# Xiaohao-Liu/EliMRec

Measured on AMD Instinct MI355X. Metric: BPR triplets/sec (Tiktok-shape, d=128x3), higher is better.
Workload: dtype f32; 1 GPU; tiktok-shape-synthetic; num_items=76085, train_interactions=571503, recdim=64, layer_num=3, batch_per_gpu=2048, global_batch=2048, parallelism=colshard1, graph_table=column-sharded (64 of 64 columns per rank): hops need no communication, feature_tables=replicated S_m / c, feature_dtype=f32, columns_per_gpu=64, propagation=folded, head_rows=batch, step_issue=one host call per step (csrc/program.hip): 1243 of the 1243 timed steps

## Files before the change

### elimrec_amd/_lib.py

```python
import ctypes
import os

_HERE = os.path.dirname(os.path.abspath(__file__))
LIB_PATH = os.path.join(_HERE, "lib", "libelimrec_hip.so")

c_i32, c_i64, c_f32, c_u32, c_u64 = ctypes.c_int, ctypes.c_int64, ctypes.c_float, ctypes.c_uint32, ctypes.c_uint64
c_ptr, c_size = ctypes.c_void_p, ctypes.c_size_t

class CsrSplit(ctypes.Structure):
    _fields_ = [("long_threshold", ctypes.c_int32), ("n_long", ctypes.c_int32), ("n_seg", ctypes.c_int32),
                ("d_long_rows", ctypes.c_void_p), ("d_long_seg_ptr", ctypes.c_void_p),
                ("d_seg_bounds", ctypes.c_void_p), ("d_partials", ctypes.c_void_p), ("d_seg_row", ctypes.c_void_p),
                ("d_row_order", ctypes.c_void_p), ("d_tickets", ctypes.c_void_p), ("d_row_items", ctypes.c_void_p),
                ("n_row_items", ctypes.c_int32)]


class CsrDesc(ctypes.Structure):
    _fields_ = [("n_rows", ctypes.c_int64), ("d_rowptr", ctypes.c_void_p), ("d_col", ctypes.c_void_p),
                ("d_val", ctypes.c_void_p), ("split", CsrSplit)]


class LinearDesc(ctypes.Structure):
    _fields_ = [("d_A", ctypes.c_void_p), ("lda", ctypes.c_int64), ("d_W", ctypes.c_void_p), ("ldw", ctypes.c_int64),
                ("d_bias", ctypes.c_void_p), ("d_C", ctypes.c_void_p), ("ldc", ctypes.c_int64), ("M", ctypes.c_int64),
# ... 53 lines not shown
                ("d_Wf_user", ctypes.c_void_p), ("d_bf_user", ctypes.c_void_p), ("d_Wf_item", ctypes.c_void_p),
                ("d_bf_item", ctypes.c_void_p), ("d_pack", ctypes.c_void_p), ("pack_floats", ctypes.c_size_t)]


class HeadFwdIn(ctypes.Structure):
    _fields_ = [("d_out0", ctypes.c_void_p), ("ld_out0", ctypes.c_int64), ("d_narrow", ctypes.c_void_p), ("ld_nar", ctypes.c_int64),
                ("d_c", ctypes.c_void_p), ("d_S", ctypes.c_void_p * HEAD_MAX_TABLES), ("ldS", ctypes.c_int64 * HEAD_MAX_TABLES),
                ("d_recv", ctypes.c_void_p), ("world", ctypes.c_int32), ("dl", ctypes.c_int64), ("src16", HeadSrc16),
                ("rows", HeadRows)]


class HeadBwdSinks(ctypes.Structure):
    _fields_ = [("d_SrcA", ctypes.c_void_p), ("d_SrcB", ctypes.c_void_p), ("N", ctypes.c_int64), ("ns", ctypes.c_int32),
                ("w", ctypes.c_int32), ("d_split", ctypes.c_void_p), ("n_max", ctypes.c_int64), ("world", ctypes.c_int32)]


class ProgramOp(ctypes.Structure):
    _fields_ = [("kind", ctypes.c_int32), ("fn", ctypes.c_int32), ("args", ctypes.c_uint64 * PROGRAM_MAX_ARGS)]


class ProgramPatch(ctypes.Structure):
    _fields_ = [("op", ctypes.c_int32), ("arg", ctypes.c_int32), ("value", ctypes.c_uint64)]


c_sell = ctypes.POINTER(SellDesc)
c_split = ctypes.POINTER(CsrSplit)
c_csr = ctypes.POINTER(CsrDesc)

SIGNATURES = {
    "elimrec_abi_version": (c_i32, []),
    "elimrec_last_error": (ctypes.c_char_p, []),
    "elimrec_linear_fwd": (c_i32, [c_ptr, c_i64, c_ptr, c_i64, c_ptr, c_ptr, c_i64, c_i64, c_i32, c_i32, c_ptr]),
    "elimrec_linear_fwd_batched": (c_i32, [ctypes.POINTER(LinearDesc), c_i32, c_ptr]),
    "elimrec_linear_bwd_w_batched_workspace": (c_size, [ctypes.POINTER(LinearBwdDesc), c_i32]),
    "elimrec_linear_bwd_w_batched": (c_i32, [ctypes.POINTER(LinearBwdDesc), c_i32, c_ptr, c_size, c_ptr]),
    "elimrec_linear_bwd_w_batched_merge": (c_i32, [ctypes.POINTER(LinearBwdDesc), c_i32, c_ptr, c_size, c_ptr, c_ptr, c_i32, c_i64,
                                                   c_i64, c_i64, c_i32, c_i32, c_i32, c_ptr, c_ptr, c_ptr, c_i32, c_ptr]),
    "elimrec_linear_bwd_w_reduce": (c_i32, [ctypes.POINTER(LinearBwdDesc), c_i32, c_ptr, c_size, c_ptr]),
    "elimrec_linear_bwd_w_workspace": (c_size, [c_i64, c_i32, c_i32]),
    "elimrec_linear_bwd_w": (c_i32, [c_ptr, c_i64, c_ptr, c_i64, c_ptr, c_ptr, c_i64, c_i32, c_i32, c_ptr, c_i64,
                                     c_ptr, c_i32, c_ptr, c_size, c_ptr]),
    "elimrec_assemble_x0": (c_i32, [c_ptr, c_ptr, c_ptr, c_i64, c_i64, c_i32, c_i32, c_ptr]),
    "elimrec_spmm_hop": (c_i32, [c_ptr, c_ptr, c_ptr, c_i64, c_i32, c_split, c_ptr, c_ptr, c_ptr, c_ptr, c_f32, c_ptr]),
    "elimrec_propagate": (c_i32, [c_ptr, c_ptr, c_ptr, c_i64, c_i32, c_split, c_i32, c_ptr, c_ptr, c_ptr, c_ptr, c_ptr]),
    "elimrec_bipartite_workspace": (c_size, [c_i64, c_i64, c_i32, c_i32]),
    "elimrec_propagate_bipartite": (c_i32, [c_csr, c_csr, c_i64, c_i64, c_i32, c_i32, c_i32, c_ptr, c_ptr, c_ptr, c_ptr,
                                            c_ptr, c_size, c_ptr]),
    "elimrec_propagate_bipartite_bwd": (c_i32, [c_csr, c_csr, c_i64, c_i64, c_i32, c_i32, c_i32, c_ptr, c_ptr, c_ptr,
                                                c_ptr, c_i64, c_ptr, c_ptr, c_ptr, c_size, c_ptr]),
    "elimrec_ticket_fixup": (c_i32, []),
    "elimrec_set_ticket_fixup": (None, [c_i32]),
    "elimrec_concurrency": (c_i32, []),
    "elimrec_set_concurrency": (None, [c_i32]),
    "elimrec_folded_workspace": (c_size, [c_i64, c_i32]),
    "elimrec_propagate_folded": (c_i32, [c_csr, c_i64, c_i64, c_i32, c_i32, c_ptr, c_ptr, c_i64, c_ptr, c_ptr, c_size, c_ptr]),
    "elimrec_source_rows_split": (c_i32, [c_ptr, c_ptr, c_i64, c_i32, c_i32, c_i32, c_ptr, c_ptr]),
    "elimrec_propagate_folded_bwd": (c_i32, [c_csr, c_i64, c_i64, c_i32, c_i32, c_i32, c_ptr, c_ptr, c_ptr, c_i64, c_ptr,
                                             c_ptr, c_ptr, c_ptr, c_ptr, c_size, c_ptr]),
    "elimrec_block_spmm": (c_i32, [c_csr, c_i32, c_i64, c_ptr, c_ptr, c_ptr, c_ptr, c_f32, c_ptr]),
    "elimrec_blocksum_rows": (c_i32, [c_ptr, c_ptr, c_ptr, c_i64, c_i32, c_i32, c_i32, c_ptr, c_ptr]),
    "elimrec_triplet_rows": (c_i32, [c_ptr, c_ptr, c_ptr, c_i64, c_i64, c_ptr, c_ptr, c_i64, c_i32, c_ptr, c_i64, c_ptr]),
    "elimrec_triplet_rows_checked": (c_i32, [c_ptr, c_ptr, c_ptr, c_i64, c_i64, c_i64, c_ptr, c_ptr, c_ptr]),
    "elimrec_batch_plan": (c_i32, [c_ptr, c_ptr, c_ptr, c_i64, c_i64, c_i64, c_ptr, c_ptr, c_ptr, c_ptr, c_ptr, c_i32, c_ptr, c_ptr,
                                   c_size, c_ptr]),
    "elimrec_gather_rows": (c_i32, [c_ptr, c_i64, c_ptr, c_ptr, c_i64, c_i32, c_ptr, c_i64, c_ptr]),
    "elimrec_copy_cols": (c_i32, [c_ptr, c_i64, c_ptr, c_i64, c_i64, c_i32, c_ptr]),
    "elimrec_bpr_head": (c_i32, [c_ptr, c_i64, c_i64, c_i64, c_ptr, c_ptr, c_ptr, c_i32, c_i32, c_i32,
                                 ctypes.POINTER(c_f32), c_ptr, c_ptr, c_ptr, c_ptr]),
    "elimrec_bpr_head_rows": (c_i32, [c_ptr, c_i64, c_ptr, c_i32, c_i32, c_i32, ctypes.POINTER(c_f32), c_ptr, c_ptr, c_ptr, c_ptr,
                                      c_ptr, c_ptr]),
    "elimrec_loss_pub_create": (c_i32, [c_i32, ctypes.POINTER(c_ptr)]),
    "elimrec_loss_pub_destroy": (c_i32, [c_ptr]),
    "elimrec_loss_pub_issued": (c_u32, [c_ptr]),
    "elimrec_loss_pub_wait": (c_i32, [c_ptr, c_u32, ctypes.c_double, ctypes.POINTER(c_f32)]),
    "elimrec_sum": (c_i32, [c_ptr, c_i64, c_ptr, c_ptr]),
    "elimrec_segment_reduce_workspace": (c_size, [c_i64]),
    "elimrec_segment_plan_workspace": (c_size, [c_i64]),
    "elimrec_segment_plan": (c_i32, [c_ptr, c_i64, c_i32, c_i64, c_ptr, c_ptr, c_ptr, c_ptr, c_ptr, c_size, c_ptr]),
    "elimrec_segment_apply_head_bwd": (c_i32, [c_ptr, c_i64, c_i32, c_ptr, c_ptr, c_ptr, c_ptr, c_ptr, c_size, c_i64, c_i32,
                                               c_i32, c_i32, ctypes.POINTER(c_i32), c_ptr, c_ptr, ctypes.POINTER(c_ptr), c_ptr,
                                               c_ptr, ctypes.POINTER(HeadBwdSinks), c_ptr]),
    "elimrec_segment_apply": (c_i32, [c_ptr, c_i64, c_i32, c_ptr, c_ptr, c_ptr, c_ptr, c_size, c_ptr]),
    "elimrec_segment_reduce_rows": (c_i32, [c_ptr, c_ptr, c_i64, c_i32, c_i32, c_ptr, c_ptr, c_ptr, c_ptr, c_ptr, c_size, c_ptr]),
    "elimrec_head_bwd_input": (c_i32, [c_ptr, c_i64, c_ptr, c_ptr, c_i64, c_i64, c_i32, c_i32, c_i32,
                                       ctypes.POINTER(c_i32), c_ptr, c_ptr, ctypes.POINTER(c_ptr), c_f32, c_ptr, c_i64,
                                       c_i32, c_ptr, c_ptr]),
    "elimrec_embed_grad": (c_i32, [c_ptr, c_i64, c_i64, c_i32, c_i32, c_ptr, c_ptr, c_ptr]),
    "elimrec_adam_step": (c_i32, [c_ptr, c_ptr, c_ptr, c_ptr, c_i64, c_f32, c_f32, c_f32, c_f32, c_f32, c_i64, c_ptr]),
    "elimrec_score_workspace": (c_size, [c_i32, c_i64, c_i32]),
    "elimrec_score_workspace2": (c_size, [c_i32, c_i64, c_i64, c_i32, c_i32]),
    "elimrec_score_workspace_topk": (c_size, [c_i32, c_i64, c_i64, c_i32, c_i32]),
    "elimrec_score_workspace_for": (c_size, [c_i32, c_i64, c_i64, c_i32, c_i32, c_i32, c_i32]),
    "elimrec_row_sqnorms": (c_i32, [c_ptr, c_i64, c_i64, c_i32, c_i32, c_ptr, c_ptr]),
    "elimrec_score_topk": (c_i32, [c_ptr, c_i64, c_i64, c_i64, c_ptr, c_i32, c_i32, c_i32, c_u32, c_i32, c_i32,
                                   c_ptr, c_ptr, c_ptr, c_ptr, c_i64, c_i32, c_ptr, c_ptr, c_ptr, c_size, c_ptr]),
    "elimrec_score_topk_shard": (c_i32, [c_ptr, c_i64, c_i64, c_i64, c_ptr, c_i32, c_i32, c_i32, c_u32, c_i32, c_i32,
                                         c_ptr, c_ptr, c_ptr, c_ptr, c_i64, c_i32, c_ptr, c_ptr, c_ptr, c_size, c_i32, c_ptr, c_i64,
                                         c_i64, c_ptr]),
    "elimrec_topk_merge": (c_i32, [c_ptr, c_ptr, c_i32, c_i32, c_i32, c_ptr, c_ptr, c_ptr]),
    "elimrec_rank_metrics": (c_i32, [c_ptr, c_i32, c_i32, c_ptr, c_ptr, ctypes.POINTER(c_i32), c_i32, c_ptr, c_ptr]),
    "elimrec_group_metric_means": (c_i32, [c_ptr, c_i64, c_i32, c_i64, c_ptr, c_ptr, c_i64, c_i32, c_ptr, c_ptr, c_size, c_ptr]),
    "elimrec_group_metric_means_workspace": (c_size, [c_i64, c_i32, c_i32]),
    "elimrec_group_metric_means_chunk": (c_i32, []),
    "elimrec_rank_targets": (c_i32, [c_ptr, c_i64, c_i64, c_i64, c_ptr, c_ptr, c_i64, c_ptr, c_ptr]),
    "elimrec_rank_segment": (c_i32, []),
    "elimrec_rank_targets_per_pass": (c_i32, []),
    "elimrec_rank_pair_rows": (c_i32, [c_ptr, c_ptr, c_i64, ctypes.POINTER(ctypes.c_int), c_i32, c_ptr, c_ptr]),
    "elimrec_rank_user_rows": (c_i32, [c_ptr, c_ptr, c_i64, c_ptr, c_i64, c_ptr, c_ptr]),
    "elimrec_cosine_topk": (c_i32, [c_ptr, c_i64, c_i64, c_i32, c_ptr, c_i64, c_ptr, c_i64, c_i32, c_ptr, c_ptr, c_i32, c_ptr, c_ptr,
                                    c_ptr, c_size, c_ptr]),
    "elimrec_cosine_topk_workspace": (c_size, [c_i64, c_i64, c_i32]),
    "elimrec_cosine_topk_chunk": (c_i32, []),
    "elimrec_cosine_topk_tile": (c_i32, []),
    "elimrec_list_overlap": (c_i32, [c_ptr, c_ptr, c_i64, c_i32, c_ptr, c_ptr]),
    "elimrec_list_pair_cosine": (c_i32, [c_ptr, c_i64, c_i64, c_i32, c_i32, c_ptr, c_i64, c_ptr, c_i64, c_i32, c_ptr, c_ptr]),
    "elimrec_list_max_k": (c_i32, []),
    "elimrec_list_pair_cosine_small_k": (c_i32, []),
    "elimrec_list_pair_cosine_chunk_cols": (c_i32, [c_i32, c_i32]),
    "elimrec_list_exposure": (c_i32, [c_ptr, c_i64, c_i32, c_i64, c_ptr, c_ptr]),
    "elimrec_mmr_rerank": (c_i32, [c_ptr, c_i64, c_i64, c_i32, c_ptr, c_i64, c_ptr, c_ptr, c_i64, c_i32, c_i32, c_f32, c_ptr, c_ptr,
                                   c_ptr, c_ptr]),
    "elimrec_mmr_max_pool": (c_i32, []),
    "elimrec_mmr_rows_in_lds": (c_i32, [c_i32, c_i32]),
    "elimrec_pick_hard_negatives": (c_i32, [c_ptr, c_i64, c_i64, c_ptr, c_i64, c_ptr, c_i64, c_i64, c_ptr, c_i64, c_i32, c_i32,
                                            ctypes.POINTER(c_f32), c_ptr, c_ptr, c_i64, c_i32, c_ptr, c_ptr, c_ptr, c_ptr]),
    "elimrec_history_support": (c_i32, [c_ptr, c_i64, c_i64, c_i32, c_i32, c_ptr, c_i64, ctypes.POINTER(c_f32), c_ptr, c_ptr, c_i64,
                                        c_i32, c_ptr, c_ptr, c_i64, c_i32, c_i32, c_ptr, c_ptr, c_ptr, c_ptr, c_ptr]),
    "elimrec_history_max_top": (c_i32, []),
    "elimrec_slab_partials_bytes": (c_size, [c_sell, c_i32, c_i32]),
    "elimrec_slab_hop": (c_i32, [c_sell, c_i32, c_i32, c_i32, c_ptr, c_ptr, c_ptr, c_ptr, c_ptr, c_f32, c_ptr, c_size, c_i32,
                                 c_ptr]),
    "elimrec_topk_reference_order": (c_i32, [c_ptr, c_i64, c_i64, c_i64, c_i32, c_ptr]),
    "elimrec_topk_reference_order_device": (c_i32, [c_ptr, c_i64, c_i64, c_i64, c_i32, c_ptr, c_ptr, c_ptr]),
    "elimrec_score_topk_ordered": (c_i32, [c_ptr, c_i64, c_i64, c_i64, c_ptr, c_i32, c_i32, c_i32, c_u32, c_i32, c_i32,
                                           c_ptr, c_ptr, c_ptr, c_ptr, c_i64, c_i32, c_ptr, c_ptr, c_ptr, c_size, c_i32, c_ptr]),
    "elimrec_plan_workspace": (c_size, [c_i64, c_i64, c_i64]),
    "elimrec_plan_tile_count": (c_i64, [c_i64, c_i64, c_i64, c_i64, c_i32]),
    "elimrec_plan_rows": (c_i32, [c_ptr, c_i64, c_i32, c_i32, c_i32, c_i32, c_i32, c_i64, c_i64, c_ptr, c_ptr, c_ptr, c_ptr, c_ptr, c_ptr, c_size, c_ptr]),
    "elimrec_plan_tiles": (c_i32, [c_ptr, c_i64, c_i32, c_i32, c_i32, c_i32, c_i32, c_i64, c_i64, c_ptr, c_ptr, c_ptr, c_i64, c_i64, c_i64, c_i64, c_i64,
                                   c_i64, c_ptr, c_ptr, c_ptr, c_ptr, c_ptr, c_ptr, c_ptr, c_ptr, c_size, c_ptr]),
    "elimrec_plan_scatter": (c_i32, [c_i64, c_i32, c_ptr, c_ptr, c_ptr, c_ptr, c_ptr, c_ptr, c_ptr, c_ptr, c_ptr]),
    "elimrec_slab_sweep_lds_rows": (c_size, [c_i32]),
    "elimrec_slab_sweep_hop": (c_i32, [c_ptr, c_ptr, c_i64, c_i64, c_ptr, c_i32, c_i32, c_i32, c_i32, c_i32, c_i32,
                                       c_ptr, c_ptr, c_ptr, c_ptr, c_f32, c_ptr]),
    "elimrec_slab_sweep_hop_adam": (c_i32, [c_ptr, c_ptr, c_i64, c_i64, c_ptr, c_i32, c_i32, c_i32, c_i32, c_i32, c_i32,
                                            c_ptr, c_ptr, c_ptr, c_ptr, c_f32, c_ptr, c_ptr, c_ptr, c_ptr, c_f32, c_f32, c_f32, c_f32, c_f32,
                                            c_i64, c_ptr]),
    "elimrec_slab_hop_bwd_w": (c_i32, [c_sell, c_i32, c_i32, c_i32, c_ptr, c_ptr, c_ptr, c_ptr, c_ptr, c_f32, c_ptr, c_size, c_i32,
                                       ctypes.POINTER(LinearBwdDesc), c_i32, c_ptr, c_size, c_i32, c_ptr]),
    "elimrec_slab_source_bits": (c_i32, [c_sell, c_i32, c_i32, c_i32, c_ptr, c_ptr, c_size, c_ptr]),
    "elimrec_slab_hop_adam": (c_i32, [c_sell, c_i32, c_i32, c_i32, c_ptr, c_ptr, c_ptr, c_ptr, c_f32, c_ptr, c_size, c_ptr, c_ptr,
                                      c_ptr, c_ptr, c_f32, c_f32, c_f32, c_f32, c_f32, c_i64, ctypes.POINTER(AdamJob), c_i32, c_ptr, c_i64,
                                      c_ptr, c_ptr]),
    "elimrec_slab_rows": (c_i32, [c_sell, c_i32, c_i32, c_i32, c_i64, ctypes.POINTER(c_ptr), c_ptr, c_ptr, c_ptr, c_i64, c_i32,
                                  c_ptr, c_i64, c_ptr, c_i64, c_i32, c_ptr]),
    "elimrec_slab_from_rows": (c_i32, [c_ptr, c_i64, c_i64, c_i64, c_i32, c_i32, c_ptr, c_ptr]),
    "elimrec_slab_to_rows": (c_i32, [c_ptr, c_i64, c_i32, c_i32, c_ptr, c_i64, c_i64, c_ptr]),
    "elimrec_slab_merge_rows": (c_i32, [c_ptr, c_ptr, c_i32, c_i64, c_i64, c_i64, c_i32, c_i32, c_i32, c_ptr, c_ptr, c_ptr, c_ptr]),
    "elimrec_adam_step_out": (c_i32, [c_ptr, c_ptr, c_ptr, c_ptr, c_ptr, c_i64, c_f32, c_f32, c_f32, c_f32, c_f32, c_i64,
                                      c_ptr]),
    "elimrec_head_pack_floats": (c_size, [c_i32, ctypes.POINTER(c_i32)]),
    "elimrec_head_pack_bwd_offset": (c_size, [c_i32, ctypes.POINTER(c_i32)]),
    "elimrec_head_fwd_fused": (c_i32, [ctypes.POINTER(HeadFwdIn), ctypes.POINTER(HeadWeights), c_ptr, c_ptr, c_i64, c_ptr, c_i64,
                                       c_ptr, c_i64, c_i32, c_ptr]),
    "elimrec_score_range_violations": (c_i32, [ctypes.POINTER(c_i64), c_i32, c_ptr]),
    "elimrec_score_range_check": (c_i32, [c_ptr, c_ptr, c_i32, c_i32, c_i32, c_i32, c_ptr, c_ptr]),
    "elimrec_score_set_math": (None, [c_i32]),
    "elimrec_score_get_math": (c_i32, []),
    "elimrec_score_set_bf16x3": (None, [c_i32]),
    "elimrec_score_get_bf16x3": (c_i32, []),
    "elimrec_build_adj_workspace": (c_size, [c_i64, c_i64, c_i32]),
    "elimrec_build_adj": (c_i32, [c_ptr, c_ptr, c_i64, c_i64, c_i64, c_i32, c_ptr, c_i32, c_ptr, c_ptr, c_ptr, c_ptr, c_ptr, c_size,
                                  c_ptr]),
    "elimrec_adam_multi": (c_i32, [ctypes.POINTER(AdamJob), c_i32, c_f32, c_f32, c_f32, c_f32, c_f32, c_ptr]),
    "elimrec_lookup_counts": (c_i32, [c_ptr, c_i32, c_i64, c_i64, c_i64, ctypes.POINTER(c_i64), ctypes.POINTER(c_i64), c_ptr, c_ptr]),
    "elimrec_lookup_pack": (c_i32, [c_ptr, c_i32, c_i64, c_i64, c_i64, ctypes.POINTER(c_i64), ctypes.POINTER(c_i64), c_i32, c_ptr, c_i64,
                                    c_ptr, c_ptr, c_ptr]),
    "elimrec_lookup_unpack": (c_i32, [c_ptr, c_i32, c_i64, c_i64, c_i64, ctypes.POINTER(c_i64), ctypes.POINTER(c_i64), c_i32, c_ptr, c_i64,
                                      c_i32, c_i32, c_i32, c_ptr, c_i64, c_ptr, c_ptr]),
    "elimrec_wide_from_master": (c_i32, [c_ptr, c_i64, c_i64, c_i32, c_i32, c_ptr, c_ptr]),
    "elimrec_wide_rows": (c_i32, [ctypes.POINTER(c_ptr), c_i32, c_i64, c_i32, c_i32, c_ptr, c_i64, c_ptr, c_i64, c_ptr, c_i64, c_ptr]),
    "elimrec_wide_grad": (c_i32, [c_ptr, c_i64, c_i64, c_i32, c_i32, c_f32, c_ptr, c_ptr]),
    "elimrec_rows_bitmap": (c_i32, [c_ptr, c_i32, c_i64, c_i64, c_ptr, c_ptr]),
    "elimrec_peer_cols_to_rows": (c_i32, [c_ptr, c_i32, c_i64, c_i32, c_ptr, c_i64, c_ptr, c_i64, c_ptr]),
    "elimrec_program_fn_count": (c_i32, []),
    "elimrec_program_fn_name": (ctypes.c_char_p, [c_i32]),
    "elimrec_program_fn_args": (c_i32, [c_i32]),
    "elimrec_program_create": (c_i32, [ctypes.POINTER(ProgramOp), c_i32, ctypes.POINTER(c_ptr)]),
    "elimrec_program_create_scoped": (c_i32, [ctypes.POINTER(ProgramOp), c_i32, c_i32, ctypes.POINTER(c_ptr)]),
    "elimrec_program_run": (c_i32, [c_ptr, ctypes.POINTER(ProgramPatch), c_i32]),
    "elimrec_program_destroy": (c_i32, [c_ptr]),
    "elimrec_comm_unique_id": (c_i32, [c_ptr]),
    "elimrec_comm_create": (c_i32, [c_ptr, c_i32, c_i32, ctypes.POINTER(c_ptr)]),
    "elimrec_comm_nranks": (c_i32, [c_ptr, ctypes.POINTER(c_i32)]),
    "elimrec_comm_destroy": (c_i32, [c_ptr]),
    "elimrec_comm_all_gather": (c_i32, [c_ptr, c_ptr, c_ptr, c_i64, c_ptr]),
    "elimrec_comm_all_reduce_f32": (c_i32, [c_ptr, c_ptr, c_i64, c_ptr]),
    "elimrec_comm_all_to_all": (c_i32, [c_ptr, c_ptr, c_ptr, c_i64, c_ptr]),
    "elimrec_comm_all_to_all_v": (c_i32, [c_ptr, c_ptr, c_ptr, ctypes.POINTER(c_i64), c_ptr]),
    "elimrec_sample_triplets": (c_i32, [c_ptr, c_ptr, c_ptr, c_i64, c_i64, c_i64, c_u64, c_u64, c_ptr, c_ptr, c_ptr, c_ptr]),
    "elimrec_sample_triplet_candidates": (c_i32, [c_ptr, c_ptr, c_ptr, c_i64, c_i64, c_i64, c_u64, c_u64, c_i32, c_ptr, c_ptr, c_ptr,
                                                  c_ptr]),
    "elimrec_sample_negatives": (c_i32, [c_ptr, c_ptr, c_i64, c_i64, c_i32, c_u64, c_ptr, c_ptr]),
    "elimrec_score_candidates": (c_i32, [c_ptr, c_i64, c_i64, c_i64, c_ptr, c_i32, c_i32, c_i32, c_u32, c_i32, c_i32,
                                         c_ptr, c_ptr, c_ptr, c_ptr, c_i64, c_ptr, c_i64, c_i64, c_ptr]),
    "elimrec_score_effects": (c_i32, [c_ptr, c_i64, c_i64, c_i64, c_ptr, c_i32, c_i32, c_i32, c_u32, c_i32,
                                      c_ptr, c_ptr, c_ptr, c_ptr, c_i64, c_ptr, c_i64, c_ptr]),
}

_lib = None


class HipLibraryError(RuntimeError):
    pass


def load():
    global _lib
    if _lib is not None:
        return _lib
    if not os.path.exists(LIB_PATH):
        raise HipLibraryError(
            "elimrec_amd: %s is missing. Build it with `python -c 'import __graft_entry__ as g; g.build()'` "
            "(or `make -C elimrec_amd/csrc`). There is no CPU fallback for the hot path." % LIB_PATH)
    try:
        lib = ctypes.CDLL(LIB_PATH)
    except OSError as e:
        raise HipLibraryError("elimrec_amd: cannot load %s: %s" % (LIB_PATH, e))
    for name, (res, args) in SIGNATURES.items():
        try:
            fn = getattr(lib, name)
        except AttributeError:
            raise HipLibraryError("elimrec_amd: %s does not export %s (stale build?)" % (LIB_PATH, name))
        fn.restype = res
        fn.argtypes = args
    if lib.elimrec_abi_version() != 2:
        raise HipLibraryError("elimrec_amd: ABI version mismatch")
    _lib = _Recording(lib)
    return _lib


class _Recording(object):

    def __init__(self, lib):
        self._cdll = lib
        self._rec = None
        self._trace = None
        for name, (res, _) in SIGNATURES.items():
            fn = getattr(lib, name)
            plain = name in ("elimrec_abi_version", "elimrec_program_fn_count", "elimrec_program_fn_args", "elimrec_comm_unique_id",
                             "elimrec_score_get_math", "elimrec_score_get_bf16x3", "elimrec_group_metric_means_chunk",
                             "elimrec_rank_segment", "elimrec_rank_targets_per_pass",
                             "elimrec_cosine_topk_chunk", "elimrec_cosine_topk_tile",
                             "elimrec_list_max_k", "elimrec_list_pair_cosine_small_k", "elimrec_list_pair_cosine_chunk_cols",
                             "elimrec_mmr_max_pool", "elimrec_mmr_rows_in_lds",
                             "elimrec_comm_create", "elimrec_comm_destroy", "elimrec_comm_nranks") or name.startswith("elimrec_program_")
            setattr(self, name, self._wrap(fn, name) if res is c_i32 and not plain else fn)

    def _wrap(self, fn, name):
        def call(*args):
            if self._rec is not None:
                self._rec.append((fn, args))
            if self._trace is not None:
                self._trace.append(("call", name, fn, args))
            return fn(*args)
        return call


def record(calls):
    load()._rec = calls


def replay(calls, what):
    for fn, args in calls:
        rc = fn(*args)
        if rc:
            check(rc, what)


def check(rc, what):
    if rc != 0:
        msg = load().elimrec_last_error()
        raise RuntimeError("%s failed (rc=%d): %s" % (what, rc, msg.decode() if msg else "?"))
```

### elimrec_amd/csrc/bwd_w.h

```cpp
#pragma once
#include "common.h"
#include <cstdlib>

namespace elimrec {

constexpr int kMaxBatch = 8;
typedef float v16f __attribute__((ext_vector_type(16)));
#ifndef ELIMREC_BWDW_TN2
#define ELIMREC_BWDW_TN2 64
#endif
constexpr int TN1 = 64, TN2 = ELIMREC_BWDW_TN2, TRB = 32;
constexpr int BNJ = TN2 / 64, BC4 = TN2 / 4, BRP = 256 / BC4, BPS = TRB / BRP;

struct BwdProblem {
    elimrec_linear_bwd_desc d;
    int chunk_rows, chunks, t1, t2;
    int first_block;
    float *slabs, *cslabs;
};
struct BwdBatch { BwdProblem p[kMaxBatch]; int n; };

__device__ __forceinline__ void bwd_w_partial_body(const BwdBatch &batch, int block, float (*As)[TRB * TN1], float (*Bs)[TRB * TN2]) {
    const int tid = threadIdx.x, lane = tid & 63, wave = tid >> 6;
    int pi = 0;
    while (pi + 1 < batch.n && block >= batch.p[pi + 1].first_block) ++pi;
    const BwdProblem &pb = batch.p[pi];
    const int local = block - pb.first_block;
    const int n1_tiles = pb.t1, n2_tiles = pb.t2;
    const int chunk = local / (n1_tiles * n2_tiles);
    const int tile = local - chunk * (n1_tiles * n2_tiles);
    const int tile_y = tile / n2_tiles, tile_z = tile - tile_y * n2_tiles;
    const float *__restrict__ A = pb.d.d_A;
    const float *__restrict__ B = pb.d.d_B;
    const int32_t *__restrict__ row_index = pb.d.d_row_index;
    const int32_t *__restrict__ range = pb.d.d_range;
    const int64_t lda = pb.d.lda, ldb = pb.d.ldb, R = pb.d.R;
    const int n1 = pb.d.n1, n2 = pb.d.n2, chunk_rows = pb.chunk_rows;
    float *__restrict__ slabs = pb.slabs;
    float *__restrict__ colsum_slabs = pb.d.d_colsum ? pb.cslabs : nullptr;
    const float *__restrict__ cw = pb.d.d_colsum ? pb.d.d_colsum_weight : nullptr;
    int64_t rb = 0, re = R;
    if (range) { rb = range[0]; re = range[1]; }
    const int64_t r0 = rb + (int64_t)chunk * chunk_rows;
    const int64_t r1 = (r0 + chunk_rows < re) ? r0 + chunk_rows : re;
    const int i_base = tile_y * TN1, j_base = tile_z * TN2;

    const int a_row = tid >> 4, a_c4 = tid & 15;
    const int b_row = tid / BC4, b_c4 = tid % BC4;
    const bool a_col_ok = (i_base + a_c4 * 4) < n1;
    const bool b_col_ok = (j_base + b_c4 * 4) < n2;
    float4 ra[2], rbv[BPS];
    float rw = 1.f, rw_cur = 1.f;
    auto load_block = [&](int64_t row0) {
        if (cw && tid < TRB) {
            const int64_t r = row0 + tid;
            rw = r < r1 ? cw[row_index ? (int64_t)row_index[r] : r] : 0.f;
        }
#pragma unroll
        for (int p = 0; p < 2; ++p) {
            const int64_t r = row0 + a_row + 16 * p;
            ra[p] = (a_col_ok && r < r1) ? *reinterpret_cast<const float4 *>(A + r * lda + i_base + a_c4 * 4)
                                         : make_float4(0.f, 0.f, 0.f, 0.f);
        }
#pragma unroll
        for (int p = 0; p < BPS; ++p) {
            const int64_t r = row0 + b_row + BRP * p;
            float4 v = make_float4(0.f, 0.f, 0.f, 0.f);
            if (b_col_ok && r < r1) {
                const int64_t br = row_index ? (int64_t)row_index[r] : r;
                v = *reinterpret_cast<const float4 *>(B + br * ldb + j_base + b_c4 * 4);
            }
            rbv[p] = v;
        }
    };
    auto store_block = [&](int buf) {
        rw_cur = rw;
#pragma unroll
        for (int p = 0; p < 2; ++p)
            *reinterpret_cast<float4 *>(&As[buf][(a_row + 16 * p) * TN1 + a_c4 * 4]) = ra[p];
#pragma unroll
        for (int p = 0; p < BPS; ++p)
            *reinterpret_cast<float4 *>(&Bs[buf][(b_row + BRP * p) * TN2 + b_c4 * 4]) = rbv[p];
    };

    const int wi = (wave & 1) * 32, wj = (wave >> 1) * (TN2 / 2);
    const int li = lane & 31, lk = lane >> 5;
    const bool wave_on = (j_base + wj) < n2;
    const bool half1_on = BNJ > 1 && (j_base + wj + 32) < n2;
    v16f acc0 = {0}, acc1 = {0};
    float csum = 0.f;
    int buf = 0;
    if (r0 < r1) {
        load_block(r0);
        store_block(0);
    }
    __syncthreads();
    for (int64_t row0 = r0; row0 < r1; row0 += TRB) {
        const bool more = (row0 + TRB) < r1;
        if (more) load_block(row0 + TRB);
        const float *as = As[buf], *bs = Bs[buf];
        if (wave_on) {
#pragma unroll
            for (int kk = 0; kk < TRB; kk += 2) {
                const float a = as[(kk + lk) * TN1 + wi + li];
                const float b0 = bs[(kk + lk) * TN2 + wj + li];
                acc0 = __builtin_amdgcn_mfma_f32_32x32x2f32(a, b0, acc0, 0, 0, 0);
                if (BNJ > 1) {
                    const float b1 = bs[(kk + lk) * TN2 + wj + (BNJ > 1 ? 32 : 0) + li];
                    acc1 = __builtin_amdgcn_mfma_f32_32x32x2f32(a, b1, acc1, 0, 0, 0);
                }
            }
        }
        if (colsum_slabs && tid < TN1) {
            if (cw) {
#pragma unroll
                for (int k = 0; k < TRB; ++k)
                    csum += as[k * TN1 + tid] * __builtin_bit_cast(float, __builtin_amdgcn_readlane(__builtin_bit_cast(int, rw_cur), k));
            } else {
#pragma unroll 8
                for (int k = 0; k < TRB; ++k) csum += as[k * TN1 + tid];
            }
        }
        if (more) store_block(buf ^ 1);
        __syncthreads();
        buf ^= 1;
    }
    const int n1_pad = n1_tiles * TN1, n2_pad = n2_tiles * TN2;
    float *slab = slabs + (size_t)chunk * n1_pad * n2_pad;
    if (wave_on) {
#pragma unroll
        for (int r = 0; r < 16; ++r) {
            const int row = i_base + wi + (r & 3) + 8 * (r >> 2) + 4 * (lane >> 5);
            slab[(size_t)row * n2_pad + j_base + wj + li] = acc0[r];
            if (half1_on) slab[(size_t)row * n2_pad + j_base + wj + 32 + li] = acc1[r];
        }
    }
    if (colsum_slabs && tile_z == 0 && tid < TN1) colsum_slabs[(size_t)chunk * n1_pad + i_base + tid] = csum;
}

__device__ __forceinline__ void reduce_slabs_body(const BwdBatch &batch, int bx, int by) {
    const BwdProblem &pb = batch.p[by];
    const int n1 = pb.d.n1, n2 = pb.d.n2;
    const int n1_pad = pb.t1 * TN1, n2_pad = pb.t2 * TN2;
    const int gid = bx * 256 + (int)threadIdx.x;
    const int idx = gid >> 2, q = gid & 3;
    const int total = n1 * n2;
    int64_t rows = pb.d.d_range ? (int64_t)pb.d.d_range[1] - pb.d.d_range[0] : pb.d.R;
    if (rows < 0) rows = 0;
    const int chunks = (int)((rows + pb.chunk_rows - 1) / pb.chunk_rows);
    const float *src = nullptr;
    size_t stride = 0;
    float *dst = nullptr;
    if (idx < total) {
        const int i = idx / n2, j = idx - i * n2;
        src = pb.slabs + (size_t)i * n2_pad + j;
        stride = (size_t)n1_pad * n2_pad;
        dst = pb.d.d_out + (int64_t)i * pb.d.ldo + j;
    } else if (pb.d.d_colsum && idx < total + n1) {
        src = pb.cslabs + (idx - total);
        stride = (size_t)n1_pad;
        dst = pb.d.d_colsum + (idx - total);
    }
    float s = 0.f;
    if (src) {
        int c = q;
        for (; c + 12 < chunks; c += 16) {
            const float v0 = src[(size_t)c * stride], v1 = src[(size_t)(c + 4) * stride];
            const float v2 = src[(size_t)(c + 8) * stride], v3 = src[(size_t)(c + 12) * stride];
            s += v0; s += v1; s += v2; s += v3;
        }
        for (; c < chunks; c += 4) s += src[(size_t)c * stride];
    }
    s += __shfl_xor(s, 1, 64);
    s += __shfl_xor(s, 2, 64);
    if (src && q == 0) *dst = pb.d.accumulate ? (*dst + s) : s;
}


static inline void bwd_w_dims(int64_t R, int n1, int n2, int &chunk_rows, int &chunks, int &t1, int &t2) {
    const int tiles = ((n1 + TN1 - 1) / TN1) * ((n2 + TN2 - 1) / TN2);
    static int target = 0;
    if (!target) target = 480;
    int64_t want = (R * tiles + target - 1) / target;
    want = (want + TRB - 1) / TRB * TRB;
    chunk_rows = (int)(want < 64 ? 64 : (want > 512 ? 512 : want));
    chunks = (int)((R + chunk_rows - 1) / chunk_rows);
    if (chunks < 1) chunks = 1;
    t1 = (n1 + TN1 - 1) / TN1;
    t2 = (n2 + TN2 - 1) / TN2;
}

static inline size_t bwd_w_bytes(int64_t R, int n1, int n2) {
    int cr, chunks, t1, t2;
    bwd_w_dims(R, n1, n2, cr, chunks, t1, t2);
    return align_up(((size_t)chunks * t1 * TN1 * t2 * TN2 + (size_t)chunks * t1 * TN1) * sizeof(float), 256);
}


static inline int bwd_w_build_batch(const elimrec_linear_bwd_desc *descs, int n, void *d_workspace, BwdBatch &batch, int &blocks,
                                    int &max_out) {
    batch.n = n;
    char *ws = (char *)d_workspace;
    blocks = 0; max_out = 0;
    for (int i = 0; i < n; ++i) {
        const elimrec_linear_bwd_desc &d = descs[i];
        ELIMREC_REQUIRE(d.d_A && d.d_B && d.d_out, "linear_bwd_w: null pointer");
        ELIMREC_REQUIRE(d.R >= 0 && d.n1 > 0 && d.n2 > 0, "linear_bwd_w: bad shape");
        ELIMREC_REQUIRE(d.n1 % 4 == 0 && d.n2 % 4 == 0 && d.lda % 4 == 0 && d.ldb % 4 == 0,
                        "linear_bwd_w: n1, n2, lda, ldb must be multiples of 4");
        ELIMREC_REQUIRE(((uintptr_t)d.d_A % 16) == 0 && ((uintptr_t)d.d_B % 16) == 0,
                        "linear_bwd_w: A and B must be 16-byte aligned");
        BwdProblem &pb = batch.p[i];
        pb.d = d;
        bwd_w_dims(d.R, d.n1, d.n2, pb.chunk_rows, pb.chunks, pb.t1, pb.t2);
        pb.first_block = blocks;
        blocks += pb.chunks * pb.t1 * pb.t2;
        pb.slabs = (float *)ws;
        pb.cslabs = pb.slabs + (size_t)pb.chunks * pb.t1 * TN1 * pb.t2 * TN2;
        ws += bwd_w_bytes(d.R, d.n1, d.n2);
        const int out_elems = d.n1 * d.n2 + (d.d_colsum ? d.n1 : 0);
        if (out_elems > max_out) max_out = out_elems;
    }
    return 0;
}

static inline size_t bwd_w_batched_bytes(const elimrec_linear_bwd_desc *descs, int n) {
    size_t total = 0;
    for (int i = 0; i < n; ++i) total += bwd_w_bytes(descs[i].R, descs[i].n1, descs[i].n2);
    return total;
}

}
```

### elimrec_amd/csrc/program.hip

```cpp
#include "common.h"
#include <dlfcn.h>
#include <cstring>
#include <string>
#include <utility>
#include <vector>

namespace elimrec {

template <typename T> struct Unpack {
    static T get(uint64_t v) {
        if constexpr (std::is_pointer<T>::value) return reinterpret_cast<T>(static_cast<uintptr_t>(v));
        else if constexpr (std::is_same<T, float>::value) { uint32_t b = (uint32_t)v; float f; memcpy(&f, &b, 4); return f; }
        else return static_cast<T>(v);
    }
};
template <typename R, typename... A, size_t... I>
static R call_packed_impl(R (*f)(A...), const uint64_t *a, std::index_sequence<I...>) { return f(Unpack<A>::get(a[I])...); }
template <typename R, typename... A> static R call_packed(R (*f)(A...), const uint64_t *a) {
    static_assert(sizeof...(A) <= ELIMREC_PROGRAM_MAX_ARGS, "too many arguments for a program op");
    return call_packed_impl(f, a, std::index_sequence_for<A...>{});
}
template <typename R, typename... A> constexpr int arg_count(R (*)(A...)) { return (int)sizeof...(A); }

static unsigned event_flags(bool has_collectives) {
    return has_collectives ? hipEventDisableTiming : (hipEventDisableTiming | hipEventDisableSystemFence);
}

struct FnEntry { const char *name; int (*thunk)(const uint64_t *); int n_args; };
#define ELIMREC_FN(fn) {#fn, [](const uint64_t *a) -> int { return call_packed(fn, a); }, arg_count(fn)}
static const FnEntry kFns[] = {
    ELIMREC_FN(elimrec_batch_plan), ELIMREC_FN(elimrec_slab_hop), ELIMREC_FN(elimrec_slab_sweep_hop), ELIMREC_FN(elimrec_slab_sweep_hop_adam), ELIMREC_FN(elimrec_slab_source_bits), ELIMREC_FN(elimrec_slab_hop_bwd_w),
    ELIMREC_FN(elimrec_slab_hop_adam), ELIMREC_FN(elimrec_slab_rows), ELIMREC_FN(elimrec_slab_merge_rows),
    ELIMREC_FN(elimrec_head_fwd_fused), ELIMREC_FN(elimrec_bpr_head_rows), ELIMREC_FN(elimrec_sum), ELIMREC_FN(elimrec_segment_apply_head_bwd),
    ELIMREC_FN(elimrec_linear_fwd_batched), ELIMREC_FN(elimrec_linear_bwd_w_batched),
    ELIMREC_FN(elimrec_linear_bwd_w_batched_merge), ELIMREC_FN(elimrec_linear_bwd_w_reduce), ELIMREC_FN(elimrec_adam_multi),
    ELIMREC_FN(elimrec_source_rows_split), ELIMREC_FN(elimrec_copy_cols), ELIMREC_FN(elimrec_lookup_pack), ELIMREC_FN(elimrec_lookup_unpack),
    ELIMREC_FN(elimrec_lookup_counts), ELIMREC_FN(elimrec_adam_step_out),
    ELIMREC_FN(elimrec_peer_cols_to_rows), ELIMREC_FN(elimrec_rows_bitmap), ELIMREC_FN(elimrec_comm_all_gather), ELIMREC_FN(elimrec_comm_all_reduce_f32),
    ELIMREC_FN(elimrec_comm_all_to_all), ELIMREC_FN(elimrec_comm_all_to_all_v), ELIMREC_FN(elimrec_wide_from_master),
    ELIMREC_FN(elimrec_wide_rows), ELIMREC_FN(elimrec_wide_grad),
};
constexpr int kNumFns = (int)(sizeof(kFns) / sizeof(kFns[0]));

typedef struct ncclComm *ncclComm_t;
struct NcclId { char internal[128]; };
struct Rccl {
    void *h = nullptr;
    int (*GetUniqueId)(NcclId *) = nullptr;
    int (*CommInitRank)(ncclComm_t *, int, NcclId, int) = nullptr;
    int (*CommDestroy)(ncclComm_t) = nullptr;
    int (*CommCount)(ncclComm_t, int *) = nullptr;
    int (*AllGather)(const void *, void *, size_t, int, ncclComm_t, hipStream_t) = nullptr;
    int (*AllReduce)(const void *, void *, size_t, int, int, ncclComm_t, hipStream_t) = nullptr;
    int (*Send)(const void *, size_t, int, int, ncclComm_t, hipStream_t) = nullptr;
    int (*Recv)(void *, size_t, int, int, ncclComm_t, hipStream_t) = nullptr;
    int (*GroupStart)() = nullptr;
    int (*GroupEnd)() = nullptr;
    const char *(*GetErrorString)(int) = nullptr;
};
static Rccl g_rccl;
static int rccl_load() {
    if (g_rccl.h) return 0;
    void *h = dlopen("librccl.so", RTLD_NOW | RTLD_NOLOAD);
    if (!h) h = dlopen("librccl.so.1", RTLD_NOW | RTLD_NOLOAD);
    if (!h) h = dlopen("librccl.so", RTLD_NOW | RTLD_GLOBAL);
    if (!h) h = dlopen("/opt/rocm/lib/librccl.so", RTLD_NOW | RTLD_GLOBAL);
    if (!h) { set_error("program: librccl.so not found (%s)", dlerror()); return ELIMREC_E_UNSUPPORTED; }
#define ELIMREC_SYM(field, name)                                                         \
    *(void **)(&g_rccl.field) = dlsym(h, name);                                          \
    if (!g_rccl.field) { set_error("program: %s missing in librccl", name); return ELIMREC_E_UNSUPPORTED; }
    ELIMREC_SYM(GetUniqueId, "ncclGetUniqueId") ELIMREC_SYM(CommInitRank, "ncclCommInitRank") ELIMREC_SYM(CommDestroy, "ncclCommDestroy")
    ELIMREC_SYM(CommCount, "ncclCommCount")
    ELIMREC_SYM(AllGather, "ncclAllGather") ELIMREC_SYM(AllReduce, "ncclAllReduce") ELIMREC_SYM(Send, "ncclSend") ELIMREC_SYM(Recv, "ncclRecv")
    ELIMREC_SYM(GroupStart, "ncclGroupStart") ELIMREC_SYM(GroupEnd, "ncclGroupEnd") ELIMREC_SYM(GetErrorString, "ncclGetErrorString")
#undef ELIMREC_SYM
    g_rccl.h = h;
    return 0;
}
static int rccl_check(int rc, const char *what) {
    if (rc == 0) return 0;
    set_error("%s: %s", what, g_rccl.GetErrorString ? g_rccl.GetErrorString(rc) : "RCCL error");
    return 20000 + rc;
}
constexpr int kNcclFloat32 = 7, kNcclUint8 = 1, kNcclSum = 0;

struct Comm { ncclComm_t comm; int world, rank; };

struct Program {
    std::vector<elimrec_op> ops;
    std::vector<hipEvent_t> events;
};

}

using namespace elimrec;

extern "C" int elimrec_program_fn_count(void) { return kNumFns; }
extern "C" const char *elimrec_program_fn_name(int i) { return (i >= 0 && i < kNumFns) ? kFns[i].name : nullptr; }
extern "C" int elimrec_program_fn_args(int i) { return (i >= 0 && i < kNumFns) ? kFns[i].n_args : -1; }

extern "C" int elimrec_comm_unique_id(void *id128) {
    int rc = rccl_load();
    if (rc) return rc;
    return rccl_check(g_rccl.GetUniqueId((NcclId *)id128), "ncclGetUniqueId");
}

extern "C" int elimrec_comm_create(const void *id128, int world, int rank, void **comm_out) {
    ELIMREC_REQUIRE(id128 && comm_out && world >= 1 && rank >= 0 && rank < world, "comm_create: bad arguments");
    int rc = rccl_load();
    if (rc) return rc;
    NcclId id;
    memcpy(&id, id128, sizeof(id));
    Comm *c = new Comm{nullptr, world, rank};
    rc = rccl_check(g_rccl.CommInitRank(&c->comm, world, id, rank), "ncclCommInitRank");
    if (rc) { delete c; return rc; }
    *comm_out = c;
    return 0;
}

extern "C" int elimrec_comm_nranks(void *comm, int *n_out) {
    ELIMREC_REQUIRE(comm && n_out, "comm_nranks: bad arguments");
    return rccl_check(g_rccl.CommCount(((Comm *)comm)->comm, n_out), "ncclCommCount");
}

extern "C" int elimrec_comm_destroy(void *comm) {
    if (!comm) return 0;
    Comm *c = (Comm *)comm;
    int rc = g_rccl.CommDestroy ? rccl_check(g_rccl.CommDestroy(c->comm), "ncclCommDestroy") : 0;
    delete c;
    return rc;
}

extern "C" int elimrec_comm_all_gather(void *comm, const void *d_send, void *d_recv, int64_t bytes_per_rank, void *stream) {
    ELIMREC_REQUIRE(comm && d_send && d_recv && bytes_per_rank >= 0, "comm_all_gather: bad arguments");
    Comm *c = (Comm *)comm;
    return rccl_check(g_rccl.AllGather(d_send, d_recv, (size_t)bytes_per_rank, kNcclUint8, c->comm, (hipStream_t)stream), "ncclAllGather");
}

extern "C" int elimrec_comm_all_reduce_f32(void *comm, float *d_buf, int64_t n, void *stream) {
    ELIMREC_REQUIRE(comm && d_buf && n >= 0, "comm_all_reduce: bad arguments");
    Comm *c = (Comm *)comm;
    return rccl_check(g_rccl.AllReduce(d_buf, d_buf, (size_t)n, kNcclFloat32, kNcclSum, c->comm, (hipStream_t)stream), "ncclAllReduce");
}

extern "C" int elimrec_comm_all_to_all(void *comm, const void *d_send, void *d_recv, int64_t bytes_per_peer, void *stream) {
    ELIMREC_REQUIRE(comm && d_send && d_recv && bytes_per_peer >= 0, "comm_all_to_all: bad arguments");
    Comm *c = (Comm *)comm;
    const char *s = (const char *)d_send;
    char *r = (char *)d_recv;
    const size_t nb = (size_t)bytes_per_peer;
    int rc = rccl_check(g_rccl.GroupStart(), "ncclGroupStart");
    for (int q = 0; q < c->world && !rc; ++q) {
        rc = rccl_check(g_rccl.Send(s + (size_t)q * nb, nb, kNcclUint8, q, c->comm, (hipStream_t)stream), "ncclSend");
        if (!rc) rc = rccl_check(g_rccl.Recv(r + (size_t)q * nb, nb, kNcclUint8, q, c->comm, (hipStream_t)stream), "ncclRecv");
    }
    const int rc2 = rccl_check(g_rccl.GroupEnd(), "ncclGroupEnd");
    return rc ? rc : rc2;
}

extern "C" int elimrec_comm_all_to_all_v(void *comm, const void *d_send, void *d_recv, const int64_t *sizes, void *stream) {
    ELIMREC_REQUIRE(comm && d_send && d_recv && sizes, "comm_all_to_all_v: bad arguments");
    Comm *c = (Comm *)comm;
    const char *s = (const char *)d_send;
    char *r = (char *)d_recv;
    int rc = rccl_check(g_rccl.GroupStart(), "ncclGroupStart");
    size_t so = 0, ro = 0;
    for (int q = 0; q < c->world && !rc; ++q) {
        const size_t sb = (size_t)sizes[q], rb = (size_t)sizes[c->world + q];
        if (sb) rc = rccl_check(g_rccl.Send(s + so, sb, kNcclUint8, q, c->comm, (hipStream_t)stream), "ncclSend");
        if (!rc && rb) rc = rccl_check(g_rccl.Recv(r + ro, rb, kNcclUint8, q, c->comm, (hipStream_t)stream), "ncclRecv");
        so += sb; ro += rb;
    }
    const int rc2 = rccl_check(g_rccl.GroupEnd(), "ncclGroupEnd");
    return rc ? rc : rc2;
}

extern "C" int elimrec_program_create_scoped(const elimrec_op *ops, int n_ops, int system_scope_events, void **prog_out) {
    ELIMREC_REQUIRE(ops && n_ops > 0 && prog_out, "program_create: bad arguments");
    Program *p = new Program();
    p->ops.assign(ops, ops + n_ops);
    int n_events = 0;
    bool has_collectives = system_scope_events != 0;
    for (const elimrec_op &o : p->ops) {
        if (o.kind == ELIMREC_OP_CALL) {
            if (o.fn < 0 || o.fn >= kNumFns) { delete p; set_error("program_create: unknown function index %d", o.fn); return ELIMREC_E_BADARG; }
// ... 52 lines not shown
```

### elimrec_amd/csrc/slab.hip

```cpp
#include "common.h"
#include "merge_rows.h"
#include "rows_args.h"
#include "bwd_w.h"
#include <cstdlib>

namespace elimrec {


struct SellArgs {
    const int32_t *item_dst, *item_len, *blk_off, *col;
    const float *val;
    int64_t n_rows, n_src;
    int n_seg, n_long;
    int item_begin, item_end;
    int seg_limit;
    int w4, w4_shift, gs, spg;
    const float4 *Xin;
    const uint32_t *src_mask;
    float4 *Xout;
    const float4 *Add;
    const uint32_t *add_mask;
    float scale;
    float4 *partials;
    const int32_t *long_rows, *long_seg_ptr;
// ... 498 lines not shown
#pragma unroll
            for (int q = 0; q < KL; ++q) bal[q] = (MASKED && k + q < nk) ? t.ballots[(int64_t)ti * t.kmax + k + q] : 0ull;
            int cj[UB];
            float vj[UB];
            bool in[UB];
#pragma unroll
            for (int u = 0; u < UB; ++u) {
                const int q = u / LPR, srcl = (u % LPR) * G + sub;
                cj[u] = G == 64 ? cc[q] : __shfl(cc[q], srcl, 64);
                vj[u] = G == 64 ? vc[q] : __shfl(vc[q], srcl, 64);
                in[u] = (jbase + u) < glen;
                if (MASKED) in[u] = in[u] && ((bal[q] >> srcl) & 1ull);
            }
            tile_batch<VPL, IN_BF16, UB>(a, in_base, cj, vj, in, acc);
#pragma unroll
            for (int q = 0; q < KL; ++q) { cc[q] = cn[q]; vc[q] = vn[q]; }
        }
    }
}

template <int LPR, int VPL>
__device__ __forceinline__ void tier_wave_sum(const float (&acc)[VPL], int cl, int n_long_guard, float (&tot)[VPL]) {
    constexpr int NQ = 64 / LPR;
#pragma unroll
    for (int i = 0; i < VPL; ++i) tot[i] = NQ > 1 ? __shfl(acc[i], cl, 64) : acc[i];
    const int nq = NQ + (n_long_guard < 0 ? 1 : 0);
#pragma unroll 2
    for (int g = 1; g < nq; ++g) {
#pragma unroll
        for (int i = 0; i < VPL; ++i) tot[i] += __shfl(acc[i], g * LPR + cl, 64);
    }
}

template <int LPR, int VPL, bool IN_BF16, bool OUT_BF16, bool MASKED, bool ADAM, bool EXT_LDS = false>
__device__ __forceinline__ void tier_body(const TierArgs &t, float *lds = nullptr, unsigned front = 0) {
    constexpr int G = 64 / LPR;
    const StreamArgs &a = t.s;
    const int lane = threadIdx.x & 63, wave = threadIdx.x >> 6;
    const unsigned bx = blockIdx.x - front;
    const int grp = (int)(bx % (unsigned)a.gs);
    const int bidx = (int)(bx / (unsigned)a.gs);
    const int sub = lane / LPR, cl = lane % LPR;
    const int slab = grp * a.spg + (cl >> a.wl_shift);
    const int c = cl & (a.wl - 1);
    const int64_t in_base = (int64_t)slab * a.n_src * a.wl + c;
    __shared__ float s_own[EXT_LDS ? 1 : 4 * 64 * 8];
    float *s_part = EXT_LDS ? lds : s_own;
    const int ti = __builtin_amdgcn_readfirstlane(bidx * 4 + wave);
    const bool wg_row = bidx < t.n_w4;
    int64_t off = 0;
    int steps = 0, glen = 0, dst = -1;
    if (ti < t.n_tiles_run) {
        off = t.tile_off[ti];
        steps = (int)((t.tile_off[ti + 1] - off) / G);
        glen = t.tile_len[(int64_t)ti * G + sub];
        dst = t.tile_dst[(int64_t)ti * G + sub];
    }
    if (a.compact_long && a.add_mask && ti < t.n_tiles_run) {
        if (wg_row || ti < t.tseg_base) {
            const int row = __shfl(dst, 0, 64);
            if (row >= 0 && !bit_of(a.add_mask, row)) return;
        } else if (dst >= 0) {
            const int li0 = t.tile_long[(int64_t)(ti - t.tseg_base) * G + sub];
            if (!bit_of(a.add_mask, a.long_rows[li0])) { dst = -1; glen = 0; }
        }
    }
    float acc[VPL];
    tile_gather<LPR, VPL, IN_BF16, MASKED>(t, ti, in_base, off, steps, glen, lane, sub, acc);
    if (wg_row) {
        float tot[VPL];
        tier_wave_sum<LPR, VPL>(acc, cl, a.n_long, tot);
        if (sub == 0) {
#pragma unroll
            for (int i = 0; i < VPL; ++i) s_part[(wave * LPR + cl) * VPL + i] = tot[i];
        }
        __syncthreads();
        if (wave == 0 && sub == 0) {
#pragma unroll
            for (int i = 0; i < VPL; ++i) tot[i] = ((s_part[cl * VPL + i] + s_part[(LPR + cl) * VPL + i]) + s_part[(2 * LPR + cl) * VPL + i]) +
                                                   s_part[(3 * LPR + cl) * VPL + i];
            if (a.compact_long) lane_store<VPL, false>(a.Xout, ((int64_t)slab * a.n_long + t.long_index[dst]) * a.wl + c, tot);
            else stream_epilogue<VPL, OUT_BF16, ADAM>(a, slab, dst, c, tot);
        }
        return;
    }
    if (ti >= t.n_tiles_run) return;
    if (ti < t.tseg_base) {
        const int row = __shfl(dst, 0, 64);
        if (row < 0) return;
        float tot[VPL];
        tier_wave_sum<LPR, VPL>(acc, cl, a.n_long, tot);
        if (sub == 0) {
            if (a.compact_long) lane_store<VPL, false>(a.Xout, ((int64_t)slab * a.n_long + t.long_index[row]) * a.wl + c, tot);
            else stream_epilogue<VPL, OUT_BF16, ADAM>(a, slab, row, c, tot);
        }
        return;
    }
    if (ti >= t.tfin_base) {
        if (dst >= 0) stream_epilogue<VPL, OUT_BF16, ADAM>(a, slab, dst, c, acc);
        return;
    }
    __amdgpu_buffer_rsrc_t prsrc = __builtin_amdgcn_make_buffer_rsrc(
        (void *)a.partials, 0, (int)min((size_t)0x7FFFFFF0, (size_t)a.n_seg * a.gs * a.spg * a.wl * VPL * 4), 0x00020000);
    if (dst >= 0) {
        const int64_t pidx = ((int64_t)slab * a.n_seg + dst) * a.wl + c;
#pragma unroll
        for (int h = 0; h < VPL / 4; ++h) {
            u32x4s bits = {__float_as_uint(acc[4 * h]), __float_as_uint(acc[4 * h + 1]), __float_as_uint(acc[4 * h + 2]),
                           __float_as_uint(acc[4 * h + 3])};
            __builtin_amdgcn_raw_buffer_store_b128(bits, prsrc, (unsigned)((pidx * (VPL / 4) + h) * 16), 0, 16 );
        }
    }
    asm volatile("s_waitcnt vmcnt(0)" ::: "memory");
    int li = -1, ticket = -1, nseg = 0;
    if (dst >= 0) {
        li = t.tile_long[(int64_t)(ti - t.tseg_base) * G + sub];
        nseg = a.long_seg_ptr[li + 1] - a.long_seg_ptr[li];
        if (cl == 0) ticket = __hip_atomic_fetch_add(&a.tickets[(int64_t)grp * a.n_long + li], 1, __ATOMIC_RELAXED, __HIP_MEMORY_SCOPE_AGENT);
    }
    ticket = __shfl(ticket, sub * LPR, 64);
    const bool last = dst >= 0 && ticket == nseg - 1;
    if (__ballot(last) == 0ull) return;
    __builtin_amdgcn_fence(__ATOMIC_ACQUIRE, "agent");
    asm volatile("s_waitcnt vmcnt(0)" ::: "memory");
#pragma unroll 1
    for (int g = 0; g < G; ++g) {
        if (!__shfl(last ? 1 : 0, g * LPR, 64)) continue;
        const int g_li = __shfl(li, g * LPR, 64);
        stream_combine<LPR, VPL, OUT_BF16, ADAM>(a, grp, g_li);
        if (lane == 0) __hip_atomic_store(&a.tickets[(int64_t)grp * a.n_long + g_li], 0, __ATOMIC_RELAXED, __HIP_MEMORY_SCOPE_AGENT);
    }
}

#ifndef ELIMREC_TILE_WAVES
#define ELIMREC_TILE_WAVES 5
#endif
template <int LPR, int VPL, bool IN_BF16, bool OUT_BF16, bool MASKED>
__global__ __launch_bounds__(256, ELIMREC_TILE_WAVES) void sell_tier_kernel(TierArgs t) {
    tier_body<LPR, VPL, IN_BF16, OUT_BF16, MASKED, false>(t);
}

template <int LPR>
__global__ __launch_bounds__(256) void sell_tier_adam_kernel(TierArgs t, AdamJobs tail, int tail_block0) {
    __shared__ float scratch[4 * 64 * 8];
    if ((int)blockIdx.x >= tail_block0) {
        const int b = (int)blockIdx.x - tail_block0;
        if (b < tail.blocks) adam_jobs_body(tail, b, t.s.ad_beta1, t.s.ad_beta2, t.s.ad_eps, t.s.ad_wd);
        else fixed_order_sum_body(tail.sum_src, tail.sum_n, tail.sum_dst, scratch);
        return;
    }
    tier_body<LPR, 4, false, false, false, true, true>(t, scratch);
}

template <int LPR, bool MASKED>
__global__ __launch_bounds__(256, (LPR <= 8 ? 5 : 1)) void sell_tier_bwdw_kernel(TierArgs t, BwdBatch batch, int tail_block0, int tail_mode, int gx) {
    __shared__ float As[2][TRB * TN1];
    __shared__ float Bs[2][TRB * TN2];
    static_assert(2 * TRB * TN1 >= 4 * 64 * 8, "the hop's LDS scratch must fit the A stages");
    const int front = tail_block0 < 0 ? (-tail_block0 + 7) & ~7 : 0;
    if (tail_block0 < 0 ? (int)blockIdx.x < front : (int)blockIdx.x >= tail_block0) {
        const int b = tail_block0 < 0 ? (int)blockIdx.x : (int)blockIdx.x - tail_block0;
        if (tail_block0 < 0 && b >= -tail_block0) return;
        if (tail_mode == 1) { reduce_slabs_body(batch, b % gx, b / gx); return; }
        bwd_w_partial_body(batch, b, As, Bs);
        return;
    }
    tier_body<LPR, 4, false, false, MASKED, false, true>(t, &As[0][0], (unsigned)front);
}

static int log2_pow2(int x) {
    int s = 0;
    while ((1 << s) < x) ++s;
    return (1 << s) == x ? s : -1;
}

}

using namespace elimrec;

static size_t slab_partial_floats_bytes(const elimrec_sell *A, int ns, int w) {
    return align_up((size_t)(A->n_seg > 0 ? A->n_seg : 1) * ns * w * sizeof(float), 256);
}
static size_t slab_ticket_bytes(const elimrec_sell *A) { return align_up((size_t)8 * (A->n_long > 0 ? A->n_long : 1) * sizeof(int32_t), 256); }
static size_t slab_ballot_bytes(const elimrec_sell *A) {
    if (!A->tiered) return 0;
    const size_t tiles = (size_t)A->n_t4 + A->n_t1 + A->n_tseg + A->n_tfin;
    return align_up(tiles * (size_t)(A->tile_kmax > 0 ? A->tile_kmax : 1) * sizeof(uint64_t), 256);
}

extern "C" size_t elimrec_slab_partials_bytes(const elimrec_sell *A, int ns, int w) {
    if (!A || ns <= 0 || w <= 0) return 0;
    return slab_partial_floats_bytes(A, ns, w) + slab_ticket_bytes(A) + slab_ballot_bytes(A);
}

struct AdamEpilogue {
    const float *p_in; float *p_out, *m, *v;
    float step_size, inv_sqrt_bc2, beta1, beta2, eps, wd;
    int keep_grad;
    const AdamJobs *tail;
};

static int launch_tier(const elimrec_sell *A, int ns, int wl, int wl_shift, int gs, int spg, int lpr, const void *Xin,
                       const uint32_t *src_mask, void *Xout, const float *add,
                       const uint32_t *add_mask, float scale, float *partials, int flags, hipStream_t s,
                       const AdamEpilogue *adam = nullptr, const BwdBatch *bwdw = nullptr, int tail_mode = 0, int tail_blocks = 0,
                       int reduce_gx = 1) {
    const int seg_only = flags & 1;
    const bool bits_ready = (flags & 2) != 0;
    if (A->tile_groups != 64 / lpr) {
        set_error("slab_hop: the plan's wave tiles were laid out for %d lane groups per wave, this table geometry has %d",
                  A->tile_groups, 64 / lpr);
        return ELIMREC_E_BADARG;
    }
    ELIMREC_REQUIRE(A->d_tile_off && A->d_tile_len && A->d_tile_dst && A->d_tile_col && A->d_tile_val && A->n_t4 == 4 * A->n_w4 &&
                        A->n_t1 % 4 == 0 && A->n_tseg % 4 == 0 && A->n_tfin % 4 == 0 && (A->n_tseg == 0 || A->d_tile_long),
                    "slab_hop: bad tile plan");
    TierArgs t = {};
    StreamArgs &a = t.s;
    a.n_rows = A->n_rows; a.n_src = A->n_src; a.n_seg = A->n_seg; a.n_long = A->n_long;
    a.wl = wl; a.wl_shift = wl_shift; a.gs = gs; a.spg = spg;
    a.Xin = Xin; a.src_mask = src_mask; a.Xout = Xout;
    a.Add = seg_only ? nullptr : (const float4 *)add; a.add_mask = add_mask; a.scale = seg_only ? 1.0f : scale;
    a.partials = partials; a.long_rows = A->d_long_rows; a.long_seg_ptr = A->d_long_seg_ptr;
    a.tickets = (int32_t *)((char *)partials + slab_partial_floats_bytes(A, ns, wl * 4));
    a.compact_long = seg_only ? 1 : 0;
    if (adam) {
        a.ad_p_in = adam->p_in; a.ad_p_out = adam->p_out; a.ad_m = adam->m; a.ad_v = adam->v;
        a.ad_step_size = adam->step_size; a.ad_inv_sqrt_bc2 = adam->inv_sqrt_bc2; a.ad_beta1 = adam->beta1; a.ad_beta2 = adam->beta2;
        a.ad_eps = adam->eps; a.ad_wd = adam->wd; a.ad_keep_grad = adam->keep_grad;
    }
    t.tile_off = A->d_tile_off; t.tile_len = A->d_tile_len; t.tile_dst = A->d_tile_dst; t.tile_long = A->d_tile_long;
    t.tcol = A->d_tile_col; t.tval = A->d_tile_val; t.long_index = A->d_long_index;
    t.n_w4 = A->n_w4;
    t.t1_base = A->n_t4; t.tseg_base = t.t1_base + A->n_t1; t.tfin_base = t.tseg_base + A->n_tseg;
    t.n_tiles = t.tfin_base + A->n_tfin;
    t.n_tiles_run = seg_only ? t.tfin_base : t.n_tiles;
    const int64_t per_group = t.n_tiles_run / 4;
    if (per_group <= 0) return 0;
    int tail_block0 = (int)(per_group * gs);
    {
        if (bwdw && tail_blocks > 0 && !adam && tail_mode == 2) {
            tail_block0 = -tail_blocks;
            tail_blocks = (tail_blocks + 7) & ~7;
        }
    }
    AdamJobs tail = {};
    if (adam && adam->tail && (adam->tail->n > 0 || adam->tail->sum_src)) tail = *adam->tail;
    if (tail.n <= 0) tail.blocks = 0;
    const dim3 grid((unsigned)(per_group * gs)), grid_adam((unsigned)(per_group * gs) + (unsigned)tail.blocks + (tail.sum_src ? 1u : 0u));
    const bool masked = src_mask != nullptr;
    if (masked) {
        ELIMREC_REQUIRE(A->tile_kmax > 0, "slab_hop: bad tile plan (tile_kmax)");
        t.kmax = A->tile_kmax;
        uint64_t *ballots = (uint64_t *)((char *)a.tickets + slab_ticket_bytes(A));
        t.ballots = ballots;
        if (!bits_ready)
        hipLaunchKernelGGL(tile_ballot_kernel, dim3((unsigned)per_group, (unsigned)t.kmax), dim3(256), 0, s, t.tile_off, t.tcol, src_mask, 64 / lpr,
                           t.n_tiles_run, t.kmax, ballots);
    }
#define ELIMREC_TIER(LPR)                                                                                                     \
    do {                                                                                                                      \
        if (adam) hipLaunchKernelGGL((sell_tier_adam_kernel<LPR>), grid_adam, dim3(256), 0, s, t, tail, tail_block0);         \
        else if (bwdw && masked)                                                                                              \
            hipLaunchKernelGGL((sell_tier_bwdw_kernel<LPR, true>), dim3(grid.x + (unsigned)tail_blocks), dim3(256), 0, s, t,  \
                               *bwdw, tail_block0, tail_mode, reduce_gx);                                                     \
        else if (bwdw)                                                                                                        \
            hipLaunchKernelGGL((sell_tier_bwdw_kernel<LPR, false>), dim3(grid.x + (unsigned)tail_blocks), dim3(256), 0, s, t, \
                               *bwdw, tail_block0, tail_mode, reduce_gx);                                                     \
        else if (masked) hipLaunchKernelGGL((sell_tier_kernel<LPR, 4, false, false, true>), grid, dim3(256), 0, s, t);        \
        else hipLaunchKernelGGL((sell_tier_kernel<LPR, 4, false, false, false>), grid, dim3(256), 0, s, t);                   \
    } while (0)
    switch (lpr) {
        case 1: ELIMREC_TIER(1); break;
        case 2: ELIMREC_TIER(2); break;
        case 4: ELIMREC_TIER(4); break;
        case 8: ELIMREC_TIER(8); break;
        case 16: ELIMREC_TIER(16); break;
        case 32: ELIMREC_TIER(32); break;
        default: ELIMREC_TIER(64); break;
    }
#undef ELIMREC_TIER
    return check_hip(hipGetLastError(), "slab_hop(tiered)");
}

static int slab_geometry(const char *who, int ns, int w, int gs, int &w4_shift, int &spg, int &lpr) {
    const int w4 = w / 4;
    w4_shift = (w > 0 && w % 4 == 0) ? log2_pow2(w4) : -1;
    if (ns < 1 || w4_shift < 0) { set_error("%s: slab width must be 4 * 2^k (got w=%d, ns=%d)", who, w, ns); return ELIMREC_E_BADARG; }
    if (gs < 1 || ns % gs != 0) { set_error("%s: %d slab groups do not divide %d slabs", who, gs, ns); return ELIMREC_E_BADARG; }
    spg = ns / gs;
    if (log2_pow2(spg) < 0 || spg * w4 > 64) {
        set_error("%s: slabs per group (%d) must be a power of two with spg*w/4 <= 64", who, spg);
        return ELIMREC_E_BADARG;
    }
    lpr = spg * w4;
    return 0;
}

static int slab_simple_geometry(const char *who, int64_t n, int ns, int w, int &w4_shift) {
    w4_shift = (w > 0 && w % 4 == 0) ? log2_pow2(w / 4) : -1;
    if (n < 0 || ns < 1 || w4_shift < 0) { set_error("%s: bad slab geometry (n=%lld, ns=%d, w=%d)", who, (long long)n, ns, w); return ELIMREC_E_BADARG; }
    return 0;
}

extern "C" int elimrec_slab_hop(const elimrec_sell *A, int ns, int w, int gs, const float *d_Xin,
                                const uint32_t *d_src_mask, float *d_Xout, const float *d_add,
                                const uint32_t *d_add_mask, float scale, float *d_partials, size_t partials_bytes,
                                int flags, void *stream) {
    const int seg_only = flags & 1;
    ELIMREC_REQUIRE(A && d_Xin && d_Xout, "slab_hop: null pointer");
    ELIMREC_REQUIRE(d_Xin != d_Xout, "slab_hop: Xout must not alias Xin");
    ELIMREC_REQUIRE(A->n_items % 64 == 0 && A->n_seg_items % 64 == 0 && A->n_seg_items <= A->n_items, "slab_hop: bad plan");
    int w4_shift, spg, lpr, rc;
    if ((rc = slab_geometry("slab_hop", ns, w, gs, w4_shift, spg, lpr))) return rc;
    if ((A->n_long > 0 || A->tiered) && (!d_partials || partials_bytes < elimrec_slab_partials_bytes(A, ns, w))) {
        set_error("slab_hop: partial-row scratch too small");
        return ELIMREC_E_WORKSPACE;
    }
    SellArgs a = {};
    a.item_dst = A->d_item_dst; a.item_len = A->d_item_len; a.blk_off = A->d_blk_off; a.col = A->d_col; a.val = A->d_val;
    a.n_rows = A->n_rows; a.n_src = A->n_src; a.n_seg = A->n_seg; a.n_long = A->n_long;
    a.item_begin = 0; a.item_end = seg_only ? A->n_seg_items : A->n_items; a.seg_limit = A->n_seg_items;
    a.w4 = w / 4; a.w4_shift = w4_shift; a.gs = gs; a.spg = spg;
    a.Xin = (const float4 *)d_Xin; a.src_mask = d_src_mask; a.Xout = (float4 *)d_Xout;
    a.Add = seg_only ? nullptr : (const float4 *)d_add; a.add_mask = d_add_mask; a.scale = seg_only ? 1.0f : scale;
    a.partials = (float4 *)d_partials; a.long_rows = A->d_long_rows; a.long_seg_ptr = A->d_long_seg_ptr;
    a.compact_long = seg_only ? 1 : 0;
    hipStream_t s = (hipStream_t)stream;
    if (A->tiered)
        return launch_tier(A, ns, w / 4, w4_shift, gs, spg, lpr, d_Xin, d_src_mask, d_Xout, d_add, d_add_mask, scale,
                           d_partials, flags, s);
    const int n_it = a.item_end - a.item_begin;
    if (n_it > 0) {
        const int ipw = 64 / lpr;
        const unsigned blocks = (unsigned)(((int64_t)n_it / ipw + 3) / 4) * (unsigned)gs;
#define ELIMREC_SELL_LAUNCH(LPR)                                                                          \
    do {                                                                                                  \
        if (d_src_mask) hipLaunchKernelGGL((sell_hop_kernel<LPR, true, 8, false>), dim3(blocks), dim3(256), 0, s, a); \
        else hipLaunchKernelGGL((sell_hop_kernel<LPR, false, 4, true>), dim3(blocks), dim3(256), 0, s, a);            \
    } while (0)
        switch (lpr) {
            case 1: ELIMREC_SELL_LAUNCH(1); break;
            case 2: ELIMREC_SELL_LAUNCH(2); break;
            case 4: ELIMREC_SELL_LAUNCH(4); break;
            case 8: ELIMREC_SELL_LAUNCH(8); break;
            case 16: ELIMREC_SELL_LAUNCH(16); break;
            case 32: ELIMREC_SELL_LAUNCH(32); break;
            default: ELIMREC_SELL_LAUNCH(64); break;
        }
#undef ELIMREC_SELL_LAUNCH
        ELIMREC_LAUNCH_CHECK("slab_hop");
    }
    if (A->n_long > 0) {
        const unsigned blocks = (unsigned)((A->n_long + 3) / 4) * (unsigned)gs;
        switch (lpr) {
            case 1: hipLaunchKernelGGL((sell_fixup_kernel<1>), dim3(blocks), dim3(256), 0, s, a); break;
            case 2: hipLaunchKernelGGL((sell_fixup_kernel<2>), dim3(blocks), dim3(256), 0, s, a); break;
            case 4: hipLaunchKernelGGL((sell_fixup_kernel<4>), dim3(blocks), dim3(256), 0, s, a); break;
            case 8: hipLaunchKernelGGL((sell_fixup_kernel<8>), dim3(blocks), dim3(256), 0, s, a); break;
            case 16: hipLaunchKernelGGL((sell_fixup_kernel<16>), dim3(blocks), dim3(256), 0, s, a); break;
            case 32: hipLaunchKernelGGL((sell_fixup_kernel<32>), dim3(blocks), dim3(256), 0, s, a); break;
            default: hipLaunchKernelGGL((sell_fixup_kernel<64>), dim3(blocks), dim3(256), 0, s, a); break;
        }
        ELIMREC_LAUNCH_CHECK("slab_hop(fixup)");
    }
    return 0;
}

static int build_adam_jobs(const char *who, const elimrec_adam_job *jobs, int n_jobs, float lr, float beta1, float beta2, AdamJobs &a) {
    a.n = 0;
    int blocks = 0;
    for (int k = 0; k < n_jobs; ++k) {
        const elimrec_adam_job &j = jobs[k];
        if (j.n <= 0) continue;
        ELIMREC_REQUIRE(j.d_p_in, "%s: job %d has no parameters", who, k);
        ELIMREC_REQUIRE(!j.d_g || (j.d_p_out && j.d_m && j.d_v && j.step >= 1), "%s: job %d: an update needs p_out, m, v and a 1-based step", who, k);
        ELIMREC_REQUIRE(j.d_g || j.d_copy_dst, "%s: job %d does nothing", who, k);
        AdamJob &o = a.j[a.n++];
        o.p_in = j.d_p_in; o.p_out = j.d_p_out; o.g = j.d_g; o.m = j.d_m; o.v = j.d_v;
        o.copy_dst = j.d_copy_dst; o.n = j.n;
        if (j.d_g) {
            const double bc1 = 1.0 - pow((double)beta1, (double)j.step);
            const double bc2 = 1.0 - pow((double)beta2, (double)j.step);
            o.step_size = (float)((double)lr / bc1);
            o.inv_sqrt_bc2 = (float)(1.0 / sqrt(bc2));
        }
        o.first_block = blocks;
        int64_t nb = (j.n + 255) / 256;
        if (nb > 4096) nb = 4096;
        blocks += (int)nb;
    }
    a.blocks = blocks;
    return 0;
}

extern "C" int elimrec_slab_source_bits(const elimrec_sell *A, int ns, int w, int gs, const uint32_t *d_src_mask,
                                        float *d_partials, size_t partials_bytes, void *stream) {
    ELIMREC_REQUIRE(A && d_src_mask && d_partials, "slab_source_bits: null pointer");
    ELIMREC_REQUIRE(A->tiered && A->tile_kmax > 0, "slab_source_bits: needs a tiered (wave-tile) plan");
    int w4_shift, spg, lpr, rc;
    if ((rc = slab_geometry("slab_source_bits", ns, w, gs, w4_shift, spg, lpr))) return rc;
    ELIMREC_REQUIRE(A->tile_groups == 64 / lpr, "slab_source_bits: the plan's tiles were laid out for another geometry");
    if (partials_bytes < elimrec_slab_partials_bytes(A, ns, w)) { set_error("slab_source_bits: scratch too small"); return ELIMREC_E_WORKSPACE; }
    const int n_tiles = A->n_t4 + A->n_t1 + A->n_tseg + A->n_tfin;
    if (n_tiles <= 0) return 0;
    uint64_t *ballots = (uint64_t *)((char *)d_partials + slab_partial_floats_bytes(A, ns, w) + slab_ticket_bytes(A));
    hipLaunchKernelGGL(tile_ballot_kernel, dim3((unsigned)(n_tiles / 4), (unsigned)A->tile_kmax), dim3(256), 0, (hipStream_t)stream,
                       A->d_tile_off, A->d_tile_col, d_src_mask, 64 / lpr, n_tiles, A->tile_kmax, ballots);
    ELIMREC_LAUNCH_CHECK("slab_source_bits");
    return 0;
}

extern "C" int elimrec_slab_hop_bwd_w(const elimrec_sell *A, int ns, int w, int gs, const float *d_Xin, const uint32_t *d_src_mask,
                                      float *d_Xout, const float *d_add, const uint32_t *d_add_mask, float scale, float *d_partials,
                                      size_t partials_bytes, int flags, const elimrec_linear_bwd_desc *descs, int n,
                                      void *d_workspace, size_t workspace_bytes, int phase, void *stream) {
    ELIMREC_REQUIRE(A && d_Xin && d_Xout && d_Xin != d_Xout, "slab_hop_bwd_w: null pointer / alias");
    ELIMREC_REQUIRE(A->tiered && !(flags & 1), "slab_hop_bwd_w: needs a tiered (wave-tile) plan and a full hop");
    ELIMREC_REQUIRE(phase == 0 || phase == 1, "slab_hop_bwd_w: phase 0 (partial launch) or 1 (slab reduce)");
    ELIMREC_REQUIRE(descs && n >= 1 && n <= kMaxBatch, "slab_hop_bwd_w: 1..%d problems", kMaxBatch);
    ELIMREC_REQUIRE(d_workspace && workspace_bytes >= bwd_w_batched_bytes(descs, n), "slab_hop_bwd_w: weight-gradient workspace");
    int w4_shift, spg, lpr, rc;
    if ((rc = slab_geometry("slab_hop_bwd_w", ns, w, gs, w4_shift, spg, lpr))) return rc;
    if (!d_partials || partials_bytes < elimrec_slab_partials_bytes(A, ns, w)) {
        set_error("slab_hop_bwd_w: partial-row scratch too small");
        return ELIMREC_E_WORKSPACE;
    }
    BwdBatch batch;
    int blocks = 0, max_out = 0;
    if ((rc = bwd_w_build_batch(descs, n, d_workspace, batch, blocks, max_out))) return rc;
    const int gx = (4 * max_out + 255) / 256;
    return launch_tier(A, ns, w / 4, w4_shift, gs, spg, lpr, d_Xin, d_src_mask, d_Xout, d_add, d_add_mask, scale,
                       d_partials, flags, (hipStream_t)stream, nullptr, &batch, phase == 0 ? 2 : 1, phase == 0 ? blocks : gx * n, gx);
}

extern "C" int elimrec_slab_hop_adam(const elimrec_sell *A, int ns, int w, int gs, const float *d_Xin, float *d_grad_out,
                                     const float *d_add, const uint32_t *d_add_mask, float scale, float *d_partials,
                                     size_t partials_bytes, const float *d_p_in, float *d_p_out, float *d_m, float *d_v, float lr,
                                     float beta1, float beta2, float eps, float weight_decay, int64_t step,
                                     const elimrec_adam_job *tail_jobs, int n_tail_jobs, const float *d_sum_src, int64_t sum_n,
                                     float *d_sum_dst, void *stream) {
    ELIMREC_REQUIRE(A && d_Xin && d_p_in && d_p_out && d_m && d_v, "slab_hop_adam: null pointer");
    ELIMREC_REQUIRE(!d_sum_src || (d_sum_dst && sum_n >= 0 && sum_n < INT32_MAX), "slab_hop_adam: the sum needs a destination");
    ELIMREC_REQUIRE(A->tiered, "slab_hop_adam: needs a tiered (wave-tile) plan");
    ELIMREC_REQUIRE(step >= 1, "slab_hop_adam: 1-based step");
    ELIMREC_REQUIRE((const void *)d_Xin != (const void *)d_p_out && (const void *)d_Xin != (const void *)d_m &&
                        (const void *)d_Xin != (const void *)d_v, "slab_hop_adam: the gathered table must not be written");
    int w4_shift, spg, lpr, rc;
    if ((rc = slab_geometry("slab_hop_adam", ns, w, gs, w4_shift, spg, lpr))) return rc;
    if (!d_partials || partials_bytes < elimrec_slab_partials_bytes(A, ns, w)) {
        set_error("slab_hop_adam: partial-row scratch too small");
        return ELIMREC_E_WORKSPACE;
    }
    AdamEpilogue ad;
    ad.p_in = d_p_in; ad.p_out = d_p_out; ad.m = d_m; ad.v = d_v;
    const double bc1 = 1.0 - pow((double)beta1, (double)step), bc2 = 1.0 - pow((double)beta2, (double)step);
    ad.step_size = (float)((double)lr / bc1);
    ad.inv_sqrt_bc2 = (float)(1.0 / sqrt(bc2));
    ad.beta1 = beta1; ad.beta2 = beta2; ad.eps = eps; ad.wd = weight_decay; ad.keep_grad = d_grad_out ? 1 : 0;
    AdamJobs tail = {};
    ad.tail = nullptr;
    if (tail_jobs && n_tail_jobs > 0) {
        ELIMREC_REQUIRE(n_tail_jobs <= 8, "slab_hop_adam: at most 8 tail jobs");
        if ((rc = build_adam_jobs("slab_hop_adam", tail_jobs, n_tail_jobs, lr, beta1, beta2, tail))) return rc;
        ad.tail = &tail;
    }
    if (d_sum_src) { tail.sum_src = d_sum_src; tail.sum_dst = d_sum_dst; tail.sum_n = (int)sum_n; ad.tail = &tail; }
    return launch_tier(A, ns, w / 4, w4_shift, gs, spg, lpr, d_Xin, nullptr, d_grad_out, d_add, d_add_mask, scale,
                       d_partials, 0, (hipStream_t)stream, &ad);
}

extern "C" int elimrec_slab_rows(const elimrec_sell *A, int ns, int w, int L, int64_t U, const float *const *layers,
                                 const float *d_long, const int32_t *d_rows, const int32_t *d_counts, int64_t R,
                                 int n_lists, float *d_out0, int64_t ld_out0, float *d_narrow, int64_t ld_narrow,
                                 int narrow_by_node, void *stream) {
    ELIMREC_REQUIRE(A && layers && d_out0 && d_narrow, "slab_rows: null pointer");
    ELIMREC_REQUIRE(ld_out0 % 4 == 0 && ld_narrow % 4 == 0, "slab_rows: leading dimensions must be multiples of 4");
    ELIMREC_REQUIRE(n_lists >= 1 && (d_rows || n_lists == 1), "slab_rows: several lists need row ids");
    RowsArgs a = {};
    int rc;
    if ((rc = rows_args_fill("slab_rows", A, ns, w, L, U, layers, d_long, a))) return rc;
    a.rows = d_rows; a.counts = d_counts; a.R = R; a.n_lists = n_lists;
    a.out0 = d_out0; a.ld_out0 = ld_out0; a.narrow = d_narrow; a.ld_narrow = ld_narrow; a.by_node = narrow_by_node;
    const int64_t total = R * n_lists;
    if (total <= 0) return 0;
    int lr = 1;
    while (lr < a.nc4 && lr < 64) lr *= 2;
    hipStream_t s = (hipStream_t)stream;
    const unsigned blocks = (unsigned)((total + (256 / lr) - 1) / (256 / lr));
    switch (lr) {
        case 1: hipLaunchKernelGGL((slab_rows_kernel<1>), dim3(blocks), dim3(256), 0, s, a); break;
        case 2: hipLaunchKernelGGL((slab_rows_kernel<2>), dim3(blocks), dim3(256), 0, s, a); break;
        case 4: hipLaunchKernelGGL((slab_rows_kernel<4>), dim3(blocks), dim3(256), 0, s, a); break;
        case 8: hipLaunchKernelGGL((slab_rows_kernel<8>), dim3(blocks), dim3(256), 0, s, a); break;
        case 16: hipLaunchKernelGGL((slab_rows_kernel<16>), dim3(blocks), dim3(256), 0, s, a); break;
        case 32: hipLaunchKernelGGL((slab_rows_kernel<32>), dim3(blocks), dim3(256), 0, s, a); break;
        default: hipLaunchKernelGGL((slab_rows_kernel<64>), dim3(blocks), dim3(256), 0, s, a); break;
    }
    ELIMREC_LAUNCH_CHECK("slab_rows");
    return 0;
}

extern "C" int elimrec_slab_from_rows(const float *d_src, int64_t ld, int64_t col0, int64_t n, int ns, int w,
                                      float *d_slab, void *stream) {
    ELIMREC_REQUIRE(d_src && d_slab && ld % 4 == 0 && col0 % 4 == 0, "slab_from_rows: bad arguments");
    int sh, rc;
    if ((rc = slab_simple_geometry("slab_from_rows", n, ns, w, sh))) return rc;
    if (n == 0) return 0;
    int64_t blocks = (n * ns * (w / 4) + 255) / 256;
    if (blocks > 4096) blocks = 4096;
    hipLaunchKernelGGL(slab_from_rows_kernel, dim3((unsigned)blocks), dim3(256), 0, (hipStream_t)stream, d_src, ld, col0, n,
                       ns * (w / 4), w / 4, sh, (float4 *)d_slab);
    ELIMREC_LAUNCH_CHECK("slab_from_rows");
    return 0;
}

extern "C" int elimrec_slab_to_rows(const float *d_slab, int64_t n, int ns, int w, float *d_dst, int64_t ld, int64_t col0,
                                    void *stream) {
    ELIMREC_REQUIRE(d_dst && d_slab && ld % 4 == 0 && col0 % 4 == 0, "slab_to_rows: bad arguments");
    int sh, rc;
    if ((rc = slab_simple_geometry("slab_to_rows", n, ns, w, sh))) return rc;
    if (n == 0) return 0;
    int64_t blocks = (n * ns * (w / 4) + 255) / 256;
    if (blocks > 4096) blocks = 4096;
    hipLaunchKernelGGL(slab_to_rows_kernel, dim3((unsigned)blocks), dim3(256), 0, (hipStream_t)stream, (const float4 *)d_slab,
                       n, ns * (w / 4), w / 4, sh, d_dst, ld, col0);
    ELIMREC_LAUNCH_CHECK("slab_to_rows");
    return 0;
}

extern "C" int elimrec_slab_merge_rows(const float *d_rows, const int32_t *d_keys, int world, int64_t R, int64_t U,
                                       int64_t I, int ns, int w, int M, float *d_SrcA, float *d_SrcB, uint32_t *d_mask,
                                       void *stream) {
    ELIMREC_REQUIRE(M >= -1, "slab_merge_rows: M >= 0, or -1 for [H | G] rows without the user / item side swap");
    const int plain = M < 0 ? 1 : 0;
    if (M < 0) M = 0;
    ELIMREC_REQUIRE(d_rows && d_keys && d_SrcA && d_SrcB && d_mask, "slab_merge_rows: null pointer");
    ELIMREC_REQUIRE(world >= 1 && world <= kSlabMaxRanks && R >= 1 && R < INT32_MAX, "slab_merge_rows: 1..%d ranks", kSlabMaxRanks);
    int sh, rc;
    const int64_t N = U + I;
    if ((rc = slab_simple_geometry("slab_merge_rows", N, ns, w, sh))) return rc;
    MergeArgs a = {d_rows, d_keys, world, (int)R, U, N, ns * (w / 4), w / 4, sh, merge_rows_chunk(N), M, d_SrcA, d_SrcB, d_mask, plain};
    const unsigned grid = (unsigned)((N + a.chunk - 1) / a.chunk);
    if (grid == 0) return 0;
    hipLaunchKernelGGL(slab_merge_rows_kernel, dim3(grid), dim3(256), (size_t)(a.chunk / 32) * sizeof(uint32_t), (hipStream_t)stream, a);
    ELIMREC_LAUNCH_CHECK("slab_merge_rows");
    return 0;
}

namespace elimrec {
__global__ __launch_bounds__(256) void rows_bitmap_kernel(const int32_t *__restrict__ keys, int W, int R, int64_t N, int chunk,
                                                          uint32_t *__restrict__ mask) {
    extern __shared__ uint32_t seen[];
    __shared__ int s_beg[kSlabMaxRanks], s_end[kSlabMaxRanks];
    const int tid = threadIdx.x;
    const int64_t lo = (int64_t)blockIdx.x * chunk, hi = min(lo + chunk, N);
    for (int w = tid; w < chunk / 32; w += 256) seen[w] = 0u;
    if (tid < W) {
        const int32_t *kr = keys + (int64_t)tid * R;
        int a0 = 0, a1 = R, b0 = 0, b1 = R;
        while (a0 < a1 || b0 < b1) {
            if (a0 < a1) { const int m = (a0 + a1) >> 1; if (slab_merge_key(kr, m) < lo) a0 = m + 1; else a1 = m; }
            if (b0 < b1) { const int m = (b0 + b1) >> 1; if (slab_merge_key(kr, m) < hi) b0 = m + 1; else b1 = m; }
        }
        s_beg[tid] = a0; s_end[tid] = b0;
    }
    __syncthreads();
    for (int r = 0; r < W; ++r)
        for (int s = s_beg[r] + tid; s < s_end[r]; s += 256) {
            const int bit = (int)((int64_t)keys[(int64_t)r * R + s] - lo);
            atomicOr(&seen[bit >> 5], 1u << (bit & 31));
        }
    __syncthreads();
    for (int w = tid; w < chunk / 32; w += 256)
        if (lo + 32 * (int64_t)w < ((N + 31) / 32) * 32) mask[lo / 32 + w] = seen[w];
}
}

extern "C" int elimrec_rows_bitmap(const int32_t *d_keys, int world, int64_t R, int64_t N, uint32_t *d_mask, void *stream) {
    ELIMREC_REQUIRE(d_keys && d_mask && world >= 1 && world <= kSlabMaxRanks && R >= 1 && R < INT32_MAX && N >= 1, "rows_bitmap: bad arguments");
    const int chunk = merge_rows_chunk(N);
    hipLaunchKernelGGL(rows_bitmap_kernel, dim3((unsigned)((N + chunk - 1) / chunk)), dim3(256), (size_t)(chunk / 32) * sizeof(uint32_t),
                       (hipStream_t)stream, d_keys, world, (int)R, N, chunk, d_mask);
    ELIMREC_LAUNCH_CHECK("rows_bitmap");
    return 0;
}

extern "C" int elimrec_adam_step_out(const float *d_p_in, float *d_p_out, const float *d_g, float *d_m, float *d_v,
                                     int64_t n, float lr, float beta1, float beta2, float eps, float weight_decay,
                                     int64_t step, void *stream) {
    ELIMREC_REQUIRE(d_p_in && d_p_out && d_g && d_m && d_v, "adam_step_out: null pointer");
    ELIMREC_REQUIRE(step >= 1, "adam_step_out: step is 1-based");
    if (n <= 0) return 0;
    const double bc1 = 1.0 - pow((double)beta1, (double)step);
    const double bc2 = 1.0 - pow((double)beta2, (double)step);
    const float step_size = (float)((double)lr / bc1);
    const float inv_sqrt_bc2 = (float)(1.0 / sqrt(bc2));
    int64_t blocks = (n + 255) / 256;
    if (blocks > 4096) blocks = 4096;
    hipLaunchKernelGGL(adam_out_kernel, dim3((unsigned)blocks), dim3(256), 0, (hipStream_t)stream, d_p_in, d_p_out, d_g, d_m,
                       d_v, n, step_size, beta1, beta2, inv_sqrt_bc2, eps, weight_decay);
    ELIMREC_LAUNCH_CHECK("adam_step_out");
    return 0;
}

extern "C" int elimrec_adam_multi(const elimrec_adam_job *jobs, int n_jobs, float lr, float beta1, float beta2, float eps,
                                  float weight_decay, void *stream) {
    ELIMREC_REQUIRE(jobs && n_jobs >= 1 && n_jobs <= 8, "adam_multi: 1..8 jobs");
    AdamJobs a = {};
    int rc = build_adam_jobs("adam_multi", jobs, n_jobs, lr, beta1, beta2, a);
    if (rc) return rc;
    if (a.n == 0) return 0;
    hipLaunchKernelGGL(adam_multi_kernel, dim3((unsigned)a.blocks), dim3(256), 0, (hipStream_t)stream, a, beta1, beta2, eps, weight_decay);
    ELIMREC_LAUNCH_CHECK("adam_multi");
    return 0;
}
```

### elimrec_amd/shard.py

```python
import ctypes

import numpy as np
import torch
import torch.distributed as dist

from . import _lib, ops, program, slab
from .lookup import FeatureShard, RowOwnerMap

PAD_KEY = -(1 << 30)


def _all_gather_parts(loc, world, group):
    if loc.is_cuda and dist.get_backend(group) == "gloo":
        host = loc.cpu()
        parts = [torch.empty_like(host) for _ in range(world)]
        dist.all_gather(parts, host, group=group)
        return [p.to(loc.device) for p in parts]
    parts = [torch.empty_like(loc) for _ in range(world)]
    dist.all_gather(parts, loc, group=group)
    return parts


LOSS_RING = 1 << 16

# ... 648 lines not shown
                fold = ws["fold"]
                self.fshard = FeatureShard(owners, frank, [fold[k] for k in m._mods], fold["c"], dtype=self.feature_dtype, device=dev)
                if self.feature_shard == "row" and world > 1:
                    ws["fold"] = None
            self.lookup_row_bytes = self.fshard.row_bytes
            self._lookup_bufs = {}
        self._direct16 = bool(self.lookup and self.fshard is not None and self.fshard.code != 0 and not self.multi
                              and self.fshard.owners.world == 1 and not self.wide
                              and os.environ.get("ELIMREC_DIRECT16", "1") != "0")
        self.word_train = False
        if hasattr(m, "word_embedding") and m.dataset_name == "tiktok" and "feature_modalities" not in m.config:
            mode = str(m.config["word_embedding"]) if "word_embedding" in m.config else "train"
            if mode not in ("train", "frozen"):
                raise ValueError("word_embedding must be train or frozen (got %r)" % mode)
            if mode == "train" and (world > 1 or self.lean or self.wide or self.multi):
                from .logger import Logger
                Logger.info("word_embedding stays frozen: its gradient (the reference's retained graph) is computed on one rank with "
                            "regular tables only")
            elif mode == "train":
                self._word_setup()
                self.word_train = True
        self.load_from_model()
        m._slab_engine = self
        m._regions = {}
        self._tail = [(n, p) for n, p in m.named_parameters() if not n.startswith(("embedding_user.", "embedding_item."))]
        return ws

    @torch.no_grad()
    def load_from_model(self):
        m = self.model
        ws = m._workspace(m._ws_key[1] if m._ws_key else 1, parity=m._ws_key[3] if m._ws_key else 0)
        if self.lean:
            dev, U = m._device(), m.num_users
            x0 = torch.empty(U + m.num_items, self.dl, dtype=torch.float32, device=dev)
            x0[:U].copy_(m.embedding_user.weight.detach()[:, self.col0:self.col0 + self.dl])
            x0[U:].copy_(m.embedding_item.weight.detach()[:, self.col0:self.col0 + self.dl])
            self.master[self.cur].from_rows(x0, col0=0)
            del x0
        else:
            self.master[self.cur].from_rows(ws["X0d"], col0=self.col0)
        ws["snap"].copy_(ws["flat_param"][ws["tail_off"]:])

    @torch.no_grad()
    def sync_to_model(self):
        ctl = getattr(self.model, "_plugin", None)
        if ctl is not None and ctl.engine is self:
            ctl.master_newer = False
        self._sync_to_model()
        if ctl is not None and ctl.engine is self:
            ctl.synced()

    @torch.no_grad()
    def _sync_to_model(self):
        m = self.model
        if self.lean:
            U = m.num_users
            loc = self.master[self.cur].dense()
            parts = [loc] if self.world == 1 else _all_gather_parts(loc, self.world, self.group)
            eu, ei = m.embedding_user.weight.data, m.embedding_item.weight.data
            for q, part in enumerate(parts):
                host = part.cpu()
                eu[:, q * self.dl:(q + 1) * self.dl] = host[:U]
                ei[:, q * self.dl:(q + 1) * self.dl] = host[U:]
            return
        x0d = m._ws["X0d"]
        if self.world == 1:
            self.master[self.cur].to_rows(x0d, col0=0)
            return
        loc = self.master[self.cur].dense()
        x0d.copy_(torch.cat(_all_gather_parts(loc, self.world, self.group), dim=1))

    def _workspace(self, B):
        m = self.model
        if B not in self._bufs:
            m._workspace(B, 3 * B, parity=1 - self.cur)
        ws = m._workspace(B, 3 * B, parity=self.cur)
        dev, d, R, W = m._device(), m.latent_dim, 3 * B, self.world
        N = m.num_users + m.num_items
        if not self.lookup and (getattr(self, "narrow_x", None) is None or ws["Narrow"].data_ptr() != self.narrow_x.data_ptr()):
            self.narrow_x = torch.zeros(N + 1, d, dtype=torch.float32, device=dev)
            ws["Narrow"] = self.narrow_x[:N]
            m._regions = {}
        bufs = self._bufs.get(B)
        if bufs is None:
            bufs = self._bufs[B] = dict(send_f=torch.empty(W, R, 2 * self.dl, dtype=torch.float32, device=dev) if self.multi else None,
                                        send_b=torch.zeros(W, R, 2 * self.dl, dtype=torch.float32, device=dev) if (self.multi or self.wide) else None)
        self.send_f, self.send_b = bufs["send_f"], bufs["send_b"]
        if "nar_act" not in bufs:
            bufs["nar_act"] = torch.zeros(R, d, dtype=torch.float32, device=dev)
        self.nar_act = bufs["nar_act"]
        if self.lookup:
            if "s_rows" not in bufs:
                sd = self.fshard.sum_d
                bufs["s_rows"] = torch.zeros(R, sd, dtype=torch.float32, device=dev)
                bufs["c_rows"] = torch.zeros(R, dtype=torch.float32, device=dev)
                bufs["iota"] = torch.arange(R, dtype=torch.int32, device=dev)
            self.s_rows, self.c_rows, self.iota = bufs["s_rows"], bufs["c_rows"], bufs["iota"]
            views, off = {}, 0
            for k, D in zip(m._mods, self.fshard.dims):
                views[k] = self.s_rows[:, off:off + D]
                off += D
            m._fold_rows = dict(S=views, c=self.c_rows, narrow=self.nar_act, R=R)
        return ws

    def _fused_head_ok(self):
        m = self.model
        if self._fused is None:
            import os
            dims = [getattr(m, k + "_feat").shape[1] for k in m._mods]
            lds = 4 * (2 * 32 * 65 + sum(32 * (D + 1) for D in dims) + 32 * (m.C + 1) + (1 + m.S) * 32 * 64)
            self._fused = (os.environ.get("ELIMREC_FUSED_HEAD", "1") != "0" and m.latent_dim == 64 and 1 <= m.S <= 3
                           and m.mm_fusion_mode == "concat" and lds <= 158 * 1024)
            self._pack_bwd_off = 0
            if self._fused:
                self._pack = torch.empty(ops.head_pack_floats(dims), dtype=torch.float32, device=m._device())
                self._pack_bwd_off = ops.head_pack_bwd_offset(dims)
        return self._fused

    def _aux_stream(self):
        if self._aux is None:
            import os
            on = (not self.multi or getattr(self, "multi_aux", False)) and os.environ.get("ELIMREC_AUX_STREAM", "1") != "0"
            self._aux = torch.cuda.Stream() if on else False
        return self._aux or None

    @_once
    def _fuse_adam(self):
        import os
        return (not self.wide and self.planT.tiered and self.model.n_layers >= 2
                and os.environ.get("ELIMREC_FUSE_ADAM", "1") != "0")

    @_once
    def _fuse_reduce(self):
        import os
        m = self.model
        hops_in_region = m.n_layers - (1 if self._fuse_adam() else 0)
        return (os.environ.get("ELIMREC_FUSE_REDUCE", "1") != "0" and not self.wide and not self.sweep and self.planT.tiered
                and hops_in_region >= 1 and m.mm_fusion_mode == "concat")

    @_once
    def _long_wanted_only(self):
        import os
        e = os.environ.get("ELIMREC_LONG_WANTED")
        return (not self.wide and self.planT.tiered and self.plan.tiered
                and ((self.sweep or self._split_share >= 0.3) if e is None else e == "1"))

    @_once
    def _fuse_bwd_w(self):
        import os
        hops_in_region = self.model.n_layers - (1 if self._fuse_adam() else 0)
        return os.environ.get("ELIMREC_FUSE_BWDW", "1") != "0" and hops_in_region >= 2

    @_once
    def _sources_in_head(self):
        import os
        return (not self.multi and not self.wide and self._fused_head_ok() and bool(self._pack_bwd_off) and self.model.latent_dim == 64
                and os.environ.get("ELIMREC_HEAD_SOURCES", "1") != "0")

    @_once
    def _loss_sum_late(self):
        import os
        return self._fuse_adam() and os.environ.get("ELIMREC_LOSS_LATE", "1") != "0"

    @_once
    def _split_in_head(self):
        import os
        return (not self.wide and self._fused_head_ok() and bool(self._pack_bwd_off) and self.model.latent_dim == 64
                and os.environ.get("ELIMREC_HEAD_SOURCES", "1") != "0")

    @_once
    def _fuse_merge(self):
        import os
        return (os.environ.get("ELIMREC_FUSE_MERGE", "1") != "0" and not self.wide
                and (self.model.num_users + self.model.num_items) <= (1 << 27))

    def _timed(self, fn, hops):
        ev = self.kernel_events
        if ev is None:
            return fn()
        e0, e1 = torch.cuda.Event(enable_timing=True), torch.cuda.Event(enable_timing=True)
        e0.record()
        fn()
        e1.record()
        ev.append((e0, e1, hops))

    @torch.no_grad()
    def cs_plan(self, users, pos, neg):
        m = self.model
        B = int(users.numel())
        ws = self._workspace(B)
        users, pos, neg = m._index_tensors(users, pos, neg)
        R = 3 * B
        keys = ws["keys"][:R]
        act, seg = ws["active_rows"][:R], ws["seg_info"]
        m._plan_n = R
        m._last_block_weights = m._block_weights()
        self._keys = keys
        err = m._index_err()

        aux = self._aux_stream()
        self._head_split = self._rows_in_head = False
        early_bits = aux is not None and self.planT.tiered and not self.multi
        fresh = aux is not None and getattr(self, "_ws_new_seen", None) != getattr(m, "_ws_new", 0)
        if fresh:
            program.sync(aux, torch.cuda.current_stream())
            self._ws_new_seen = getattr(m, "_ws_new", 0)
        ahead = (aux is not None and self._forked and not fresh and not self.multi and self.prestaged_ok(users, pos, neg)
                 and self.ahead_safe())
        self._last_plan_cur = self.cur


        late_bits = early_bits and R > 8192
        self._late_bits = late_bits

        def plan_only():
            ops.batch_plan(users, pos, neg, m.num_users, m.num_items, keys, act, seg, ws["slot_seg"][:R], ws["plan_ws"], err, PAD_KEY,
                           key_bitmap=self.mask if (early_bits or self._sources_in_head()) else None)

        def bits_only():
            if early_bits and not late_bits:
                slab.source_bits(self.planT, self.hns, self.w, self.hgs, self.mask)

        def plan():
            plan_only()
            bits_only()

        def pack():
            self._head_fused_call(ws, R, phase=1)

        def features():
            self._head_fused_call(ws, R, phase=3)
        self._bits_ready = early_bits
        if aux is None:
            m._region("cs_plan", (m._ws_gen, users.data_ptr(), pos.data_ptr(), neg.data_ptr(), R), plan)
            return act
        if not self._forked:
            program.sync(aux, torch.cuda.current_stream())
        fork_rec = getattr(self, "_fork_rec", None) if self._forked else None
        self._forked, self._fork_rec = False, None
        with torch.cuda.stream(aux):
            if ahead:
                m._region("cs_plan_a", (m._ws_gen, users.data_ptr(), pos.data_ptr(), neg.data_ptr(), R), plan_only)
                program.wait(aux, fork_rec)
                m._region("cs_bits_a", (m._ws_gen, R, early_bits, late_bits), bits_only)
            else:
                if fork_rec is not None:
                    program.wait(aux, fork_rec)
                m._region("cs_plan", (m._ws_gen, users.data_ptr(), pos.data_ptr(), neg.data_ptr(), R), plan)
            if self._fused_head_ok():
                m._region("cs_pack", (m._ws_gen, R), pack)
                self._head_split = (not self.lookup or self._direct16) and self._split_head
                if self._head_split:
                    m._region("cs_head_features", (m._ws_gen, R), features)
                self._rows_in_head = (self._head_split and self._rows_in_head_on and not self.multi and not self.wide
                                      and self.dl == 64 and self.ns * self.w == 64)
        self._aux_pending = True
        self._plan_rec = program.record(aux) if self.multi else None
        self._plan_waited = False
        return act

    def plan_stream(self):
        return self._aux_stream()

    def plan_joined(self):
        if getattr(self, "_plan_rec", None) is not None:
            self._plan_rec = None
            self._plan_waited = True

    def wgrads_deferred(self):
        return bool(getattr(self, "defer_wgrads", False)) and self.multi and self._fuse_reduce() and self._fuse_bwd_w()

    @torch.no_grad()
    def cs_gathered_ids(self, acts, handle):
        aux = self._aux_stream()
        m = self.model
        if aux is None or not self.planT.tiered:
            return
        with torch.cuda.stream(aux):
            handle.wait()

            key = (m._ws_gen, acts.data_ptr(), acts.shape[0], acts.shape[1])
            m._region("cs_row_bits", key, lambda: slab.rows_bitmap(acts, m.num_users + m.num_items, self.mask))
            self._rows_rec = program.record(aux) if self._long_wanted_only() else None
            m._region("cs_bits", key, lambda: slab.source_bits(self.planT, self.hns, self.w, self.hgs, self.mask))
        self._bits_ready = True
        self._bits_join = True

    def cs_fork(self):
        aux = self._aux_stream()
        if aux is None or self.model._ws is None:
            return False
        self._fork_rec = program.record(torch.cuda.current_stream())
        self._forked = True
        return True

    def prestage(self, batches):
        aux = self._aux_stream()
        self._prestaged = {}
        if aux is None or self.multi:
            return
        program.sync(aux, torch.cuda.current_stream())
        self._prestaged = {id(u): (u, p, n) for u, p, n in batches}

    def ahead_safe(self):
        return getattr(self, "_last_plan_cur", None) != self.cur

# ... 196 lines not shown
            if with_rows:
                self._head_fused_rows_call(ws, R)
            else:
                self._head_fused_call(ws, R, phase=4 if split else (2 if packed else 0))
        m._region("cs_head_fused%d" % (self.cur if with_rows else 2), (m._ws_gen, R, B, packed, split, with_rows, self.nar_act.data_ptr(),
                                    0 if self._out0_src is None else self._out0_src.data_ptr(),
                                    0 if self._peer_src is None else self._peer_src.data_ptr()), head)
        loss = self._next_loss_slot()
        if getattr(self, "_step_in_flight", False) and getattr(self, "publish_loss", False):
            ops.bpr_head_rows_sum_pub(YAct, ws["slot_seg"][:3 * B], d, bw, ws["loss_rows"], ws["grad_rows"], loss, self._loss_ticket,
                                      self.loss_publisher().handle)
        elif getattr(self, "_step_in_flight", False) and self._loss_sum_late():
            ops.bpr_head_rows(YAct, ws["slot_seg"][:3 * B], d, bw, ws["loss_rows"], ws["grad_rows"])
            self._loss_late = (ws["loss_rows"][:B], loss)
        else:
            ops.bpr_head_rows_sum(YAct, ws["slot_seg"][:3 * B], d, bw, ws["loss_rows"], ws["grad_rows"], loss, self._loss_ticket)
        m._publish_cache(ws["Y"], dirty=True)
        return loss

    def _pair(self, R, d):
        b = self._pairs.get(R)
        if b is None:
            b = self._pairs[R] = torch.zeros(R, 2, d, dtype=torch.float32, device=self.model._device())
        return b

    def _head_fused_rows_call(self, ws, R):
        m = self.model
        d, fold, W = m.latent_dim, ws["fold"], ws["live_views"]
        OutAct, YAct = ws["OutAct"][:R], ws["YAct"][:R]
        wu, wi = m._fusion_weights(W)
        tabs = self._tabs
        rows = dict(plan=self.plan, ns=self.ns, w=self.w, L=m.n_layers, U=m.num_users, layers=[t.data for t in tabs] + [None],
                    long_tab=self.long_tab, narrow=self.nar_act)
        if self._direct16:
            c_tab, s_tabs = self.c_rows, [m._fold_rows["S"][k] for k in m._mods]
        else:
            c_tab, s_tabs = fold["c"], [fold[k] for k in m._mods]
        ok = ops.head_fwd_fused_rows(rows, ws["active_rows"][:R], ws["seg_info"], c_tab, s_tabs,
                                     [W[k + "_dense.weight"] for k in m._mods], [W[k + "_dense.bias"] for k in m._mods], wu,
                                     W["embedding_user_after_GCN.bias"], wi, W["embedding_item_after_GCN.bias"],
                                     [W["s_dense_%s.weight" % k] for k in m._mods], [W["s_dense_%s.bias" % k] for k in m._mods],
                                     self._pack, OutAct, YAct, d)
        if not ok:
            raise RuntimeError("fused head forward (with rows) refused a shape _fused_head_ok accepted")

    def _head_fused_call(self, ws, R, phase):
        m = self.model
        d, fold, W = m.latent_dim, ws["fold"], ws["live_views"]
        OutAct, YAct = ws["OutAct"][:R], ws["YAct"][:R]
        wu, wi = m._fusion_weights(W)
        out0 = self._out0_src if self._out0_src is not None else OutAct[:, :d]
        nar = self._nar_src if self._nar_src is not None else self.nar_act
        if self._direct16:
            if phase == 1:
                rows_src = (None, None)
            else:
                rows_src = (self.s_rows, self.c_rows) if phase != 4 else (None, None)
            ok = ops.head_fwd_fused_src16(self.fshard, rows_src[0], rows_src[1], ws["active_rows"][:R], ws["seg_info"], out0, nar,
                                          [W[k + "_dense.weight"] for k in m._mods], [W[k + "_dense.bias"] for k in m._mods], wu,
                                          W["embedding_user_after_GCN.bias"], wi, W["embedding_item_after_GCN.bias"],
                                          [W["s_dense_%s.weight" % k] for k in m._mods], [W["s_dense_%s.bias" % k] for k in m._mods],
                                          self._pack, OutAct, YAct, d, phase=phase)
            if not ok:
                raise RuntimeError("fused head forward (16-bit constants) refused a shape _fused_head_ok accepted")
            return
        if self.lookup:
            rows, c_tab, s_tabs = self.iota[:R], self.c_rows, [m._fold_rows["S"][k] for k in m._mods]
        else:
            rows, c_tab, s_tabs = ws["active_rows"][:R], fold["c"], [fold[k] for k in m._mods]
        ok = ops.head_fwd_fused(rows, ws["seg_info"], out0, nar, c_tab,
                                s_tabs, [W[k + "_dense.weight"] for k in m._mods],
                                [W[k + "_dense.bias"] for k in m._mods], wu, W["embedding_user_after_GCN.bias"], wi,
                                W["embedding_item_after_GCN.bias"], [W["s_dense_%s.weight" % k] for k in m._mods],
                                [W["s_dense_%s.bias" % k] for k in m._mods], self._pack, OutAct, YAct, d, phase=phase,
                                peers=self._peer_src if phase in (0, 2, 4) else None)
        if not ok:
            raise RuntimeError("fused head forward refused a shape _fused_head_ok accepted")

    @torch.no_grad()
    def cs_backward_local(self, scale):
        m = self.model
        ws, d = m._ws, m.latent_dim
        R = m._plan_n
        pack_bwd = self._pack[self._pack_bwd_off:] if (self._fused_head_ok() and self._pack_bwd_off) else None
        merge = None
        sources = (self.srcA, self.srcB) if (pack_bwd is not None and self._sources_in_head()) else None
        if self.multi and pack_bwd is not None and self._split_in_head():
            sources = ("split", self.send_b, self.world)
        if sources is not None:
            pass
        elif not self.multi and self._fuse_merge():
            merge = dict(rows=ws["dOutR"][:R].view(R, m.C), keys=self._acts.reshape(-1), world=1, U=m.num_users, I=m.num_items,
                         srcA=self.srcA, srcB=self.srcB, mask=self.mask, M=m.M)
        self._merged = merge is not None or sources is not None
        defer = (not self.multi and self._fuse_reduce())
        if defer and merge is None and self._fuse_bwd_w():
            defer = "all"
        if self.multi and self.wgrads_deferred():
            defer = "all"
        self._grads = m._backward_batch_rows(ws, scale, ws["grad_rows"], R, head_only=True, pack_bwd=pack_bwd,
                                             merge=merge, defer_reduce=defer, sources=sources)
        self._reduce = (m._bwd_w_reduce, 0 if defer == "all" else 1) if defer else None
        if self.word_train:
            self._word_grad(ws, R)
        wg = ws["flat_grad"][ws["tail_off"]:]
        if not self.multi and not self.wide:
            return ws["dOutR"][:R].view(1, R, m.C), wg
        W = self.world
        send = self.send_b
        if sources is not None:
            return send, wg
        m._region("cs_sources", (m._ws_gen, R, send.data_ptr()),
                  lambda: ops.source_rows_split(ws["dOutR"][:R], ws["seg_info"][0:1], d, m.M, W, send))
        return send, wg

    def join_source_bits(self):
        if getattr(self, "_bits_join", False):
            program.sync(torch.cuda.current_stream(), self._aux)
            self._bits_join = False

    @torch.no_grad()
    def cs_backward_hops(self, recv2, acts, grads_ready=None, reduce_wgrads=None):
        m = self.model
        U, I, L = m.num_users, m.num_items, m.n_layers
        W, R = acts.shape
        inv = 1.0 / (L + 1)

        fuse = self._fuse_adam() and not getattr(self, "grads_only", False)
        last = 1 if fuse else 0

        single = not self.multi
        merged = single and getattr(self, "_merged", False)
        self.join_source_bits()
        reduce = getattr(self, "_reduce", None) if (single or reduce_wgrads is not None) else None
        self._reduce = None
        self.wgrads_handle = None

        if self.wide:
            def wide_hops():
                slab.merge_rows(recv2.view(W * R, 2 * self.dl), acts.reshape(-1), W, U, I, self.srcA, self.srcB, self.mask, M=-1)
                t, tmask = self.srcW, self.mask
                for k in range(L - 1, -1, -1):
                    dst = self.tmp[k & 1]
                    slab.hop(self.planT, t, dst, gs=self.hgs, src_mask=tmask, add=self.srcW, add_mask=self.mask, scale=1.0,
                             bits_ready=tmask is not None and self._bits_ready)
                    t, tmask = dst, None
                slab.wide_grad(t, U, inv, self.grad)
            self._timed(lambda: m._region("cs_bwd_hops", (m._ws_gen, recv2.data_ptr(), acts.data_ptr(), R, W, self._bits_ready), wide_hops), L)
            self._adam_in_hop = self._tail_in_hop = False
            if reduce_wgrads is not None and reduce_wgrads is not True:
                self.wgrads_handle = reduce_wgrads()
            return

        def hops():
            phase = None if reduce is None else reduce[1]
            if merged:
                pass
            elif single:
                slab.merge_rows(recv2.view(R, m.C), acts.reshape(-1), 1, U, I, self.srcA, self.srcB, self.mask, M=m.M)
            else:
                slab.merge_rows(recv2.view(W * R, 2 * self.dl), acts.reshape(-1), W, U, I, self.srcA, self.srcB, self.mask)
            t, tmask = (self.srcB if (L & 1) else self.srcA), self.mask
            for k in range(L - 1, last - 1, -1):
                dst = self.grad if k == 0 else self.tmp[k & 1]
                slab.hop(self.planT, t, dst, gs=self.gs, src_mask=tmask, add=self.srcB if (k & 1) else self.srcA,
                         add_mask=self.mask, scale=inv if k == 0 else 1.0, bits_ready=tmask is not None and self._bits_ready,
                         bwd_w=reduce[0] if phase is not None and phase <= 1 else None, bwd_w_phase=phase)
                phase = None if phase is None else phase + 1
                t, tmask = dst, None
        self._timed(lambda: m._region("cs_bwd_hops", (m._ws_gen, recv2.data_ptr(), acts.data_ptr(), R, W, fuse, self._bits_ready, merged,
                                                               0 if reduce is None else ctypes.addressof(reduce[0][0]), 0 if reduce is None else reduce[1]), hops), L - last)
        self._adam_in_hop = fuse
        self._tail_in_hop = False
        if fuse:
            g = self.opt.param_groups[0]
            nxt = 1 - self.cur
            in_hop = single or grads_ready is not None
            if reduce_wgrads is True:
                in_hop = True
            elif reduce_wgrads is not None:
                self.wgrads_handle = reduce_wgrads()
                in_hop = False
            if grads_ready is not None:
                grads_ready.wait()
            tail = self._tail_jobs() if in_hop else []
            if len(tail) > 8:
                raise RuntimeError("more than 8 optimizer spans")
            if getattr(self, "_tail_arr", None) is None:
                self._tail_arr = (_lib.AdamJob * 8)()
            for i, job in enumerate(tail):
                self._tail_arr[i] = job
            self._tail_n, self._tail_base = len(tail), 0
            tail = (self._tail_arr, len(tail))
            self._tail_in_hop = in_hop
            late = getattr(self, "_loss_late", None)
            self._loss_late = None
            self._timed(lambda: slab.hop_adam(self.planT, self.tmp[1], self.grad if self.keep_grad else None, self.gs, self.srcA,
                                              self.mask, inv, self.master[self.cur].data, self.master[nxt].data, self.m1, self.m2,
                                              g["lr"], g["betas"][0], g["betas"][1], g["eps"], g["weight_decay"],
                                              self.step_count + 1, tail_jobs=tail, loss_sum=late), 1)

    @torch.no_grad()
    def cs_update(self):
        m = self.model
        g = self.opt.param_groups[0]
        self.step_count += 1
        nxt = 1 - self.cur
        jobs = []
        if not getattr(self, "_adam_in_hop", False):
            jobs.append(_lib.AdamJob(self.master[self.cur].data.data_ptr(), self.master[nxt].data.data_ptr(),
                                     self.grad.data.data_ptr(),
                                     self.m1.data_ptr(), self.m2.data_ptr(), None, self.grad.data.numel(), self.step_count))
        if not getattr(self, "_tail_in_hop", False):
            jobs += self._tail_jobs()
        if len(jobs) > 8:
            raise RuntimeError("more than 8 optimizer spans")
        if jobs:
            if getattr(self, "_tail_arr", None) is None:
                self._tail_arr = (_lib.AdamJob * 8)()
            for i, job in enumerate(jobs):
                self._tail_arr[i] = job
            self._tail_base = 0 if getattr(self, "_adam_in_hop", False) else 1
            self._tail_n = len(jobs) - self._tail_base
            _lib.check(_lib.load().elimrec_adam_multi(self._tail_arr, len(jobs), g["lr"], g["betas"][0], g["betas"][1], g["eps"],
                                                      g["weight_decay"], ops._stream()), "adam_multi")
        self.cur = nxt
        self._updated()

    def _updated(self):
        ctl = getattr(self.model, "_plugin", None)
        if ctl is not None and ctl.engine is self:
            ctl.master_newer = True

    def native_prologue(self):
        base = getattr(self, "_tail_base", 0)
        if base:
            nxt = 1 - self.cur
            self._tail_arr[0] = _lib.AdamJob(self.master[self.cur].data.data_ptr(), self.master[nxt].data.data_ptr(),
                                             self.grad.data.data_ptr(),
                                             self.m1.data_ptr(), self.m2.data_ptr(), None, self.grad.data.numel(), self.step_count + 1)
        if self._tail_plan is not None and getattr(self, "_tail_n", 0):
            _, spans, states = self._tail_plan[:3]
            for st in states:
                st["step"] += 1
            i = base
            for sp in spans:
                if sp["upd"]:
                    sp["step"] += 1
                    self._tail_arr[i].step = sp["step"]
                i += 1

    def native_epilogue(self, R):
        m = self.model
        x0 = self.master[self.cur]
        self._x0_fwd = x0
        self._tabs = [x0] + self.layers[1:]
        self._srcs = [x0] + self.layers[1:]
        m._plan_n = R
        m._slab_fwd = True
        m._publish_cache(m._ws["Y"], dirty=True)
        self.step_count += 1
        self.cur = 1 - self.cur
        self._updated()

    def _tail_jobs(self):
        m, ws = self.model, self.model._ws
        have = tuple(name for name, _ in self._tail if self._grads.get(name) is not None)
        if self._tail_plan is None or self._tail_plan[0] != have:
            base_p, base_g, snap = ws["flat_param"].data_ptr(), ws["flat_grad"].data_ptr(), ws["snap"].data_ptr()
            tail_off = ws["tail_off"]
            spans, states = [], []
            for name, p in self._tail:
                off, numel = ws["param_off"][name]
                upd = name in have
                st = self.opt._state_for(p) if upd else None
                if upd:
                    states.append(st)
                if spans and spans[-1]["upd"] == upd and spans[-1]["end"] + 3 >= off and (not upd or (
                        st["step"] == spans[-1]["step"] and st["exp_avg"].data_ptr() == spans[-1]["m"] + 4 * (off - spans[-1]["off"]))):
                    spans[-1]["end"] = off + numel
                else:
                    spans.append(dict(off=off, end=off + numel, upd=upd, step=st["step"] if upd else 0,
                                      m=st["exp_avg"].data_ptr() if upd else 0, v=st["exp_avg_sq"].data_ptr() if upd else 0))
            self._tail_plan = (have, spans, states, base_p, base_g, snap, tail_off)
        _, spans, states, base_p, base_g, snap, tail_off = self._tail_plan
        for st in states:
            st["step"] += 1
        jobs = []
        for sp in spans:
            n, o = sp["end"] - sp["off"], sp["off"]
            if sp["upd"]:
                sp["step"] += 1
                jobs.append(_lib.AdamJob(base_p + 4 * o, base_p + 4 * o, base_g + 4 * o, sp["m"], sp["v"],
                                         snap + 4 * (o - tail_off), n, sp["step"]))
            else:
                jobs.append(_lib.AdamJob(base_p + 4 * o, None, None, None, None, snap + 4 * (o - tail_off), n, 0))
        return jobs

    @torch.no_grad()
    def _horner_mean(self, x0_rows, plan=None):
        m, N, L = self.model, x0_rows.shape[0], self.model.n_layers
        per_group = (self.hns // self.hgs) * self.w
        cols = x0_rows.shape[1]
        padded = (cols + per_group - 1) // per_group * per_group
        if padded != cols:
            x0_rows = torch.cat([x0_rows, torch.zeros(N, padded - cols, dtype=torch.float32, device=x0_rows.device)], dim=1)
        ns, gs = padded // self.w, padded // per_group
        mk = lambda: slab.SlabTable(N, ns, self.w, x0_rows.device)
        x0, a, b = mk().from_rows(x0_rows.contiguous()), mk(), mk()
        t = x0
        for k in range(L):
            dst = a if t is not a else b
            slab.hop(self.plan if plan is None else plan, t, dst, gs=gs, add=x0, scale=1.0 / (L + 1) if k == L - 1 else 1.0)
            t = dst
        return t.dense()[:, :cols]

    def _word_setup(self):
        import scipy.sparse as sp
        m = self.model
        words = m.dataset.words_tensor
        it, wd = words[0].numpy().astype(np.int64), words[1].numpy().astype(np.int64)
        cnt = np.bincount(it, minlength=m.num_items).astype(np.float64)
        vals = (1.0 / cnt[it]).astype(np.float32)
        V = m.word_embedding.weight.shape[0]
        mat = sp.csr_matrix((vals, (wd, it)), shape=(V, m.num_items))
        dev = m._device()
        self._word_csr = ops.Csr.from_scipy(mat, dev, C=m.word_embedding.weight.shape[1])
        N, d = m.num_users + m.num_items, m.latent_dim
        self._word_full = torch.zeros(N + 1, d, dtype=torch.float32, device=dev)
        self._word_dF = torch.empty(m.num_items, m.word_embedding.weight.shape[1], dtype=torch.float32, device=dev)

    @torch.no_grad()
    def _word_grad(self, ws, R):
        m = self.model
        d, U = m.latent_dim, m.num_users
        N = U + m.num_items
        k = m._mods.index("t")
        blk = ws["dOutR"][:R, (k + 1) * d:(k + 2) * d]
        act = ws["active_rows"][:R].long()
        full = self._word_full
        full.zero_()
        full.index_copy_(0, torch.where(act >= 0, act, torch.full_like(act, N)), blk)
        g_items = self._horner_mean(full[:N], plan=self.planT)[U:].contiguous()
        wt = ws["live_views"]["t_dense.weight"]
        ops.linear_fwd_batched([(g_items, wt.t().contiguous(), None, self._word_dF)])
        gview = ws["grad_views"]["word_embedding.weight"]
        ops.block_spmm(self._word_csr, self._word_dF, Xout=gview)
        self._grads["word_embedding.weight"] = gview

    @torch.no_grad()
    def _fold_sharded(self, owners, frank):
        from .shard_eval import collectives_for
        m, W = self.model, owners.world
# ... 191 lines not shown
```

### elimrec_amd/slab.py

```python
import ctypes
import os

import numpy as np
import torch

from . import _lib
from .ops import _dev, _stream

LONG_ROW_THRESHOLD = 32
SLAB_W_CAP = 32
SLAB_GROUPS = 0


def choose_slabs(dl, n_rows=None):
    if dl % 4 != 0:
        raise ValueError("column count must be a multiple of 4 (got %d)" % dl)
    cap = SLAB_W_CAP
    w = 4
    while w * 2 <= cap and dl % (w * 2) == 0:
        w *= 2
    return dl // w, w


def choose_groups(ns):
# ... 301 lines not shown
            win = (self._col.astype(np.int64) - n) // self.window(w)
            n_win = int(win.max()) + 1 if len(win) else 1
            lpr = w // 4
            G, NW = 64 // lpr, lpr
            blk_of_row = np.searchsorted(ptr, np.arange(n), side="right") - 1
            by_len = np.lexsort((-self.row_nnz, blk_of_row))
            pos = np.arange(n) - ptr[blk_of_row[by_len]]
            snake = np.where((pos // NW) % 2 == 0, pos % NW, NW - 1 - pos % NW)
            wave_of_row = np.empty(n, np.int64)
            wave_of_row[by_len] = snake
            cell = (blk * NW + wave_of_row[rows]) * n_win + win
            order = np.argsort(cell, kind="stable")
            n_cells = nb * NW * n_win
            cell_ptr = np.concatenate([[0], np.cumsum(np.bincount(cell, minlength=n_cells))]).astype(np.int64)
            srow, scell = rows[order], cell[order]
            first = np.concatenate([[True], (srow[1:] != srow[:-1]) | (scell[1:] != scell[:-1])]) if len(srow) else np.zeros(0, bool)
            starts = np.nonzero(first)[0]
            k = np.arange(G + 1, dtype=np.int64)[None, :]
            ideal = (cell_ptr[:-1, None] + ((cell_ptr[1:] - cell_ptr[:-1])[:, None] * k) // G).reshape(-1)
            cut = starts[np.minimum(np.searchsorted(starts, ideal), len(starts) - 1)] if len(starts) else ideal
            cut = np.minimum(np.maximum(cut.reshape(-1, G + 1), cell_ptr[:-1, None]), cell_ptr[1:, None])
            cut[:, 0], cut[:, -1] = cell_ptr[:-1], cell_ptr[1:]
            cut = np.maximum.accumulate(cut, axis=1)
            csz = cut[:, 1:] - cut[:, :-1]
            cell_steps = ((csz + 7) // 8).max(axis=1)
            step_ptr = np.concatenate([[0], np.cumsum(cell_steps)]).astype(np.int64)
            n_steps = int(step_ptr[-1])
            dummy = int(np.diff(ptr).max())
            rec = np.zeros(((n_steps + 8) * G, 20), np.int32)
            rows16 = np.full(((n_steps + 8) * G, 8), dummy, np.uint16)
            chunk_of = np.repeat(np.arange(csz.size, dtype=np.int64), csz.reshape(-1))
            p_in = np.arange(len(chunk_of), dtype=np.int64) - np.repeat(cut[:, :-1].reshape(-1), csz.reshape(-1))
            ri = (step_ptr[chunk_of // G] + p_in // 8) * G + chunk_of % G
            si = p_in % 8
            rec[ri, si] = (self._col[order].astype(np.int64) * lpr).astype(np.uint32).view(np.int32)
            rec[ri, 8 + si] = self._val[order].view(np.int32)
            rows16[ri, si] = rloc[order].astype(np.uint16)
            rec[:, 16:20] = rows16.view(np.int32)
            slot_ptr = step_ptr[::n_win]
            t = lambda a, dt: torch.from_numpy(np.ascontiguousarray(a.astype(dt))).to(self.device)
            self._geo[key] = dict(block_ptr=t(ptr, np.int32), slot_ptr=t(slot_ptr, np.int64), rec=t(rec.reshape(-1), np.int32),
                                  parts=parts, passes=passes, bpx=bpx, rows=int(np.diff(ptr).max()), n_win=n_win, n_rec=n_steps * G,
                                  fill=float(len(order)) / max(8 * n_steps * G, 1))
        return self._geo[key]

    def index_bytes(self, ns, w):
        return 80 * int(self.geometry(ns, w)["n_rec"]) + self.items.index_bytes()

    def device_bytes(self):
        own = sum(v.numel() * v.element_size() for k, v in self.items.t.items() if k not in self.items.shared)
        own += sum(v.numel() * v.element_size() for v in self.items._partials.values())
        return own + sum(v.numel() * v.element_size() for g in self._geo.values() for v in g.values() if hasattr(v, "numel"))

    def hop(self, xin, xout, add=None, add_mask=None, scale=1.0):
        ns, w = xin.ns, xin.w
        g = self.geometry(ns, w)
        _lib.check(_lib.load().elimrec_slab_sweep_hop(_dev(g["slot_ptr"], "slot_ptr", torch.int64), _dev(g["rec"], "records", torch.int32), self.n, self.n,
                                                      _dev(g["block_ptr"], "block_ptr", torch.int32), g["parts"], g["passes"], g["bpx"],
                                                      g["rows"], ns, w, _dev(xin.data, "xin"), _dev(xout.data, "xout"),
                                                      _dev(None if add is None else add.data, "add"),
                                                      _dev(add_mask, "add_mask", torch.int32), float(scale), _stream()), "slab_sweep_hop")

    def hop_adam(self, xin, grad_out, add, add_mask, scale, p_in, p_out, m, v, lr, beta1, beta2, eps, weight_decay, step):
        ns, w = xin.ns, xin.w
        g = self.geometry(ns, w)
        _lib.check(_lib.load().elimrec_slab_sweep_hop_adam(
            _dev(g["slot_ptr"], "slot_ptr", torch.int64), _dev(g["rec"], "records", torch.int32), self.n, self.n,
            _dev(g["block_ptr"], "block_ptr", torch.int32), g["parts"], g["passes"], g["bpx"], g["rows"], ns, w, _dev(xin.data, "xin"),
            _dev(None if grad_out is None else grad_out.data, "grad"), _dev(None if add is None else add.data, "add"),
            _dev(add_mask, "add_mask", torch.int32), float(scale), _dev(p_in, "p_in"), _dev(p_out, "p_out"), _dev(m, "m"), _dev(v, "v"),
            float(lr), float(beta1), float(beta2), float(eps), float(weight_decay), int(step), _stream()), "slab_sweep_hop_adam")


SWEEP_AUTO_MAX_NNZ = 1 << 27


def sweep_wanted(n_rows, dl, nnz=None):
    env = os.environ.get("ELIMREC_SWEEP", "")
    if env in ("0", "1"):
        return env == "1"
    return n_rows * dl * 4 > (256 << 20) and (nnz is None or nnz <= SWEEP_AUTO_MAX_NNZ)


def sweep_tiles_xcds(ns):
    return (8 % ns == 0) if ns <= 8 else (ns % 8 == 0)


class SlabTable(object):

    def __init__(self, n, ns, w, device, data=None):
        self.n, self.ns, self.w = int(n), int(ns), int(w)
        self.data = torch.empty(self.ns * self.n * self.w, dtype=torch.float32, device=device) if data is None else data
        assert self.data.numel() == self.ns * self.n * self.w and self.data.is_contiguous() and self.data.dtype == torch.float32

    @property
    def cols(self):
        return self.ns * self.w

    def like(self):
        return SlabTable(self.n, self.ns, self.w, self.data.device)

    def from_rows(self, src, col0=0):
        assert src.dim() == 2 and src.stride(1) == 1 and src.shape[0] == self.n and col0 + self.cols <= src.shape[1]
        _lib.check(_lib.load().elimrec_slab_from_rows(_dev(src, "src"), src.stride(0), int(col0), self.n, self.ns, self.w,
                                                      _dev(self.data, "slab"), _stream()), "slab_from_rows")
        return self

    def to_rows(self, dst, col0=0):
        assert dst.dim() == 2 and dst.stride(1) == 1 and dst.shape[0] == self.n and col0 + self.cols <= dst.shape[1]
        _lib.check(_lib.load().elimrec_slab_to_rows(_dev(self.data, "slab"), self.n, self.ns, self.w, _dev(dst, "dst"),
                                                    dst.stride(0), int(col0), _stream()), "slab_to_rows")
        return dst

    def dense(self):
        return self.to_rows(torch.empty(self.n, self.cols, dtype=torch.float32, device=self.data.device))


def source_bits(plan, ns, w, gs, src_mask):
    part = plan.partials(ns, w)
    _lib.check(_lib.load().elimrec_slab_source_bits(plan.ref(), ns, w, int(gs), _dev(src_mask, "src_mask", torch.int32),
                                                    _dev(part, "partials"), part.numel() * 4, _stream()), "slab_source_bits")


def _swept(plan, xin):
    return plan.sweep is not None and xin.w in (16, 32) and sweep_tiles_xcds(xin.ns)


def hop(plan, xin, xout, gs=None, src_mask=None, add=None, add_mask=None, scale=1.0, seg_only=False, bits_ready=False, bwd_w=None, bwd_w_phase=1):
    ns, w = xin.ns, xin.w
    gs = choose_groups(ns) if gs is None else gs
    if _swept(plan, xin) and src_mask is None and not seg_only and isinstance(xout, SlabTable):
        hop(plan.sweep.items, xin, xout, gs=gs, add=add, add_mask=add_mask, scale=scale, bwd_w=bwd_w, bwd_w_phase=bwd_w_phase)
        plan.sweep.hop(xin, xout, add=add, add_mask=add_mask, scale=scale)
        return
    part = plan.partials(ns, w)
    out = xout if isinstance(xout, torch.Tensor) else xout.data
    lib = _lib.load()
    if bwd_w is not None:
        arr, n, wsp = bwd_w
        _lib.check(lib.elimrec_slab_hop_bwd_w(plan.ref(), ns, w, int(gs), _dev(xin.data, "xin"), _dev(src_mask, "src_mask", torch.int32),
                                               _dev(out, "xout"), _dev(None if add is None else add.data, "add"),
                                               _dev(add_mask, "add_mask", torch.int32), float(scale), _dev(part, "partials"),
                                               part.numel() * 4, 2 if bits_ready else 0, arr, n, _dev(wsp, "workspace", torch.uint8),
                                               wsp.numel(), int(bwd_w_phase), _stream()), "slab_hop_bwd_w")
        return
    _lib.check(lib.elimrec_slab_hop(plan.ref(), ns, w, int(gs), _dev(xin.data, "xin"),
                                    _dev(src_mask, "src_mask", torch.int32), _dev(out, "xout"),
                                    _dev(None if add is None else add.data, "add"),
                                    _dev(add_mask, "add_mask", torch.int32), float(scale), _dev(part, "partials"),
                                    part.numel() * 4, (1 if seg_only else 0) | (2 if bits_ready else 0), _stream()), "slab_hop")


def hop_adam(plan, xin, grad_out, gs, add, add_mask, scale, p_in, p_out, m, v, lr, beta1, beta2, eps, weight_decay, step, tail_jobs=(),
             loss_sum=None):
    if isinstance(tail_jobs, tuple) and len(tail_jobs) == 2 and not isinstance(tail_jobs[0], _lib.AdamJob):
        arr, n_tail = tail_jobs
    else:
        arr, n_tail = ((_lib.AdamJob * len(tail_jobs))(*tail_jobs) if tail_jobs else None), len(tail_jobs)
    ns, w = xin.ns, xin.w
    if _swept(plan, xin):
        hop_adam(plan.sweep.items, xin, grad_out, gs, add, add_mask, scale, p_in, p_out, m, v, lr, beta1, beta2, eps, weight_decay, step,
                 tail_jobs=(arr, n_tail), loss_sum=loss_sum)
        plan.sweep.hop_adam(xin, grad_out, add, add_mask, scale, p_in, p_out, m, v, lr, beta1, beta2, eps, weight_decay, step)
        return
    part = plan.partials(ns, w)
    _lib.check(_lib.load().elimrec_slab_hop_adam(
        plan.ref(), ns, w, int(gs), _dev(xin.data, "xin"), _dev(None if grad_out is None else grad_out.data, "grad"),
        _dev(None if add is None else add.data, "add"), _dev(add_mask, "add_mask", torch.int32), float(scale), _dev(part, "partials"),
        part.numel() * 4, _dev(p_in, "p_in"), _dev(p_out, "p_out"), _dev(m, "m"), _dev(v, "v"), float(lr), float(beta1), float(beta2),
        float(eps), float(weight_decay), int(step), arr, n_tail, _dev(None if loss_sum is None else loss_sum[0], "loss_rows"),
        0 if loss_sum is None else loss_sum[0].numel(), _dev(None if loss_sum is None else loss_sum[1], "loss_out"), _stream()),
        "slab_hop_adam")



def rows(plan, ns, w, L, U, layers, long_tab, row_ids, counts, R, n_lists, out0, narrow, narrow_by_node):
    ptrs = (ctypes.c_void_p * (L + 1))(*[None if t is None else _dev(t, "layer") for t in layers])
    assert out0.stride(1) == 1 and narrow.stride(1) == 1
    _lib.check(_lib.load().elimrec_slab_rows(plan.ref(), ns, w, L, int(U), ptrs, _dev(long_tab, "long_tab"),
                                             _dev(row_ids, "rows", torch.int32), _dev(counts, "counts", torch.int32),
                                             int(R), int(n_lists), _dev(out0, "out0"), out0.stride(0),
                                             _dev(narrow, "narrow"), narrow.stride(0), 1 if narrow_by_node else 0,
                                             _stream()), "slab_rows")


def merge_rows(all_rows, all_keys, world, U, I, srcA, srcB, mask, M=0):
    R = all_keys.numel() // world
    assert all_rows.is_contiguous() and all_rows.shape == (world * R, (M if M > 0 else 2) * srcA.cols) and mask.numel() * 32 >= U + I
    _lib.check(_lib.load().elimrec_slab_merge_rows(_dev(all_rows, "rows"), _dev(all_keys, "keys", torch.int32), int(world), R,
                                                   int(U), int(I), srcA.ns, srcA.w, int(M), _dev(srcA.data, "srcA"),
                                                   _dev(srcB.data, "srcB"), _dev(mask, "mask", torch.int32), _stream()),
               "slab_merge_rows")


def adam_step_out(p_in, p_out, g, m, v, lr, beta1, beta2, eps, weight_decay, step):
    n = p_in.numel()
    for t in (p_in, p_out, g, m, v):
        assert t.is_contiguous() and t.numel() == n
    _lib.check(_lib.load().elimrec_adam_step_out(_dev(p_in, "p_in"), _dev(p_out, "p_out"), _dev(g, "g"), _dev(m, "m"),
                                                 _dev(v, "v"), n, float(lr), float(beta1), float(beta2), float(eps),
                                                 float(weight_decay), int(step), _stream()), "adam_step_out")


def rows_bitmap(keys, N, mask):
    W, R = keys.shape
    assert keys.is_contiguous() and mask.numel() * 32 >= N
    _lib.check(_lib.load().elimrec_rows_bitmap(_dev(keys, "keys", torch.int32), int(W), int(R), int(N), _dev(mask, "mask", torch.int32),
                                               _stream()), "rows_bitmap")


def wide_from_master(master, U, wide):
    assert wide.ns == 2 * master.ns and wide.w == master.w and wide.n == master.n
    _lib.check(_lib.load().elimrec_wide_from_master(_dev(master.data, "master"), int(U), master.n, master.ns, master.w, _dev(wide.data, "wide"),
                                                    _stream()), "wide_from_master")


def wide_rows(layers, n, ns, w, rows, total, out0, narrow):
    L = len(layers) - 1
    ptrs = (ctypes.c_void_p * (L + 1))(*[_dev(t, "layer") for t in layers])
    assert out0.stride(1) == 1 and narrow.stride(1) == 1
    _lib.check(_lib.load().elimrec_wide_rows(ptrs, L, int(n), int(ns), int(w), _dev(rows, "rows", torch.int32), int(total), _dev(out0, "out0"),
                                             out0.stride(0), _dev(narrow, "narrow"), narrow.stride(0), _stream()), "wide_rows")


def wide_grad(wide, U, scale, grad):
    assert wide.ns == 2 * grad.ns and wide.w == grad.w and wide.n == grad.n
    _lib.check(_lib.load().elimrec_wide_grad(_dev(wide.data, "wide"), int(U), grad.n, grad.ns, grad.w, float(scale), _dev(grad.data, "grad"),
                                             _stream()), "wide_grad")
```

### include/elimrec_hip.h

```cpp
#ifndef ELIMREC_HIP_H
#define ELIMREC_HIP_H

#include <stddef.h>
#include <stdint.h>

#ifdef __cplusplus
extern "C" {
#endif

#define ELIMREC_ABI_VERSION 2
#define ELIMREC_E_BADARG 10001
#define ELIMREC_E_UNSUPPORTED 10002
#define ELIMREC_E_WORKSPACE 10003

int elimrec_abi_version(void);
const char *elimrec_last_error(void);

int elimrec_linear_fwd(const float *d_A, int64_t lda, const float *d_W, int64_t ldw,
                       const float *d_bias, float *d_C, int64_t ldc,
                       int64_t M, int N, int K, void *stream);

typedef struct elimrec_linear_desc {
    const float *d_A; int64_t lda;
    const float *d_W; int64_t ldw;
// ... 216 lines not shown
                               void *d_workspace, size_t workspace_bytes, int tie_order, void *stream);
int elimrec_topk_reference_order_device(const float *d_scores, int64_t n_rows, int64_t I, int64_t ld, int K,
                                        int32_t *d_topk_idx, float *d_topk_val, void *stream);
int elimrec_topk_reference_order(const float *h_scores, int64_t n_rows, int64_t I, int64_t ld, int K, int32_t *h_topk);

int elimrec_score_candidates(const float *d_Y, int64_t ldy, int64_t U, int64_t I, const int64_t *d_users, int B, int d,
                             int S, uint32_t head_mask, int fusion_mode, int predict_type, const float *d_sqnorm,
                             const int64_t *d_cand_ptr, const int32_t *d_cand_items, const float *d_row_sum,
                             int64_t I_total, float *d_scores, int64_t lds, int64_t width, void *stream);

int elimrec_score_effects(const float *d_Y, int64_t ldy, int64_t U, int64_t I, const int64_t *d_users, int B, int d, int S,
                          uint32_t head_mask, int fusion_mode, const float *d_sqnorm, const int64_t *d_cand_ptr,
                          const int32_t *d_cand_items, const float *d_row_sum, int64_t I_total, float *d_out, int64_t width,
                          void *stream);

int elimrec_rank_metrics(const int32_t *d_topk_idx, int B, int K, const int64_t *d_truth_ptr,
                         const int32_t *d_truth_items, const int *metric_ids, int n_metrics,
                         float *d_out, void *stream);

int elimrec_group_metric_means(const float *d_rows, int64_t n_rows, int C, int64_t ld, const int64_t *d_group_ptr,
                               const int32_t *d_group_rows, int64_t n_listed_rows, int G, float *d_means,
                               void *d_workspace, size_t workspace_bytes, void *stream);
size_t elimrec_group_metric_means_workspace(int64_t n_listed_rows, int C, int G);
int elimrec_group_metric_means_chunk(void);

int elimrec_rank_targets(const float *d_scores, int64_t B, int64_t I, int64_t lds, const int64_t *d_tgt_ptr,
                         const int32_t *d_tgt_items, int64_t n_targets, int32_t *d_rank, void *stream);
int elimrec_rank_segment(void);
int elimrec_rank_targets_per_pass(void);
int elimrec_rank_pair_rows(const int32_t *d_rank, const int32_t *d_n_cand, int64_t P, const int *ks, int n_k, float *d_out,
                           void *stream);
int elimrec_rank_user_rows(const int32_t *d_rank, const int64_t *d_tgt_ptr, int64_t n_targets, const int32_t *d_n_cand,
                           int64_t B, float *d_out, void *stream);

int elimrec_cosine_topk(const float *d_T, int64_t ld, int64_t n_rows, int d, const float *d_sqnorm, int64_t ld_sq,
                        const int32_t *d_query_rows, int64_t Q, int exclude_self, const int64_t *d_excl_ptr,
                        const int32_t *d_excl_rows, int K, int32_t *d_idx, float *d_val, void *d_workspace, size_t workspace_bytes,
                        void *stream);
size_t elimrec_cosine_topk_workspace(int64_t Q, int64_t n_rows, int K);
int elimrec_cosine_topk_chunk(void);
int elimrec_cosine_topk_tile(void);
int elimrec_list_overlap(const int32_t *d_a, const int32_t *d_b, int64_t n_rows, int K, int32_t *d_count, void *stream);

int elimrec_list_pair_cosine(const float *d_T, int64_t ld, int64_t n_rows, int blocks, int d, const float *d_sqnorm, int64_t ld_sq,
                             const int32_t *d_lists, int64_t B, int K, float *d_out, void *stream);
int elimrec_list_max_k(void);
int elimrec_list_pair_cosine_small_k(void);
int elimrec_list_pair_cosine_chunk_cols(int K, int d);
int elimrec_list_exposure(const int32_t *d_lists, int64_t B, int K, int64_t n_rows, int32_t *d_counts, void *stream);

int elimrec_mmr_rerank(const float *d_T, int64_t ld, int64_t n_rows, int d, const float *d_sqnorm, int64_t ld_sq,
                       const int32_t *d_pool_idx, const float *d_pool_val, int64_t B, int N, int K, float lambda,
                       int32_t *d_out_idx, int32_t *d_out_pos, float *d_out_val, void *stream);
int elimrec_mmr_max_pool(void);
int elimrec_mmr_rows_in_lds(int N, int d);

int elimrec_pick_hard_negatives(const float *d_U, int64_t ld_u, int64_t n_users, const float *d_sq_u, int64_t ldsq_u,
                                const float *d_T, int64_t ld_i, int64_t n_items, const float *d_sq_i, int64_t ldsq_i,
                                int blocks, int d, const float *h_weights, const int64_t *d_users, const int32_t *d_cands,
                                int64_t n, int M, int64_t *d_out_neg, int32_t *d_out_pos, float *d_out_score, void *stream);

int elimrec_history_support(const float *d_T, int64_t ld, int64_t n_items, int blocks, int d,
                            const float *d_sqnorm, int64_t ld_sq, const float *h_weights,
                            const int64_t *d_users, const int32_t *d_lists, int64_t B, int K,
                            const int64_t *d_hist_ptr, const int32_t *d_hist_items, int64_t n_hist_rows,
                            int top, int exclude_self,
                            int32_t *d_out_idx, float *d_out_val, int32_t *d_out_cnt, float *d_out_mean, void *stream);
int elimrec_history_max_top(void);

int elimrec_sample_triplets(const int32_t *d_user_ids, const int64_t *d_ptr, const int32_t *d_items,
                            int64_t n_train_users, int64_t I, int64_t n, uint64_t seed,
                            uint64_t epoch, int64_t *d_users, int64_t *d_pos, int64_t *d_neg,
                            void *stream);

int elimrec_sample_triplet_candidates(const int32_t *d_user_ids, const int64_t *d_ptr, const int32_t *d_items,
                                      int64_t n_train_users, int64_t I, int64_t n, uint64_t seed, uint64_t epoch, int n_cand,
                                      int64_t *d_users, int64_t *d_pos, int32_t *d_cands, void *stream);

int elimrec_sample_negatives(const int64_t *d_excl_ptr, const int32_t *d_excl_items, int64_t n_users, int64_t I,
                             int n_neg, uint64_t seed, int32_t *d_out, void *stream);

typedef struct elimrec_sell {
    int64_t n_rows;
    int64_t n_src;
    int32_t n_items;
    int32_t n_seg_items;
    int32_t n_seg;
    int32_t n_long;
    const int32_t *d_item_dst;
    const int32_t *d_item_len;
    const int32_t *d_blk_off;
    const int32_t *d_col;
    const float *d_val;
    const int32_t *d_long_rows;
    const int32_t *d_long_seg_ptr;
    const int32_t *d_long_index;
    const int64_t *d_rowptr;
    const int32_t *d_csr_col;
    const float *d_csr_val;
    const int32_t *d_item_long;
    int32_t tiered, n_w1, n_w4;
    int32_t tile_groups, n_t4, n_t1, n_tseg, n_tfin;
    int32_t tile_kmax;
    const int64_t *d_tile_off;
    const int32_t *d_tile_len, *d_tile_dst, *d_tile_long, *d_tile_col;
    const float *d_tile_val;
} elimrec_sell;

size_t elimrec_plan_workspace(int64_t n_rows, int64_t n_seg, int64_t n_tiles);
int64_t elimrec_plan_tile_count(int64_t n_w4, int64_t n_w1, int64_t n_seg, int64_t n_short, int G);
int elimrec_plan_rows(const int64_t *d_rowptr, int64_t n_rows, int T, int T1, int T2, int TS, int G, int64_t side_split,
                      int64_t rows_from, int32_t *d_order, int32_t *d_long_rows, int32_t *d_long_index, int32_t *d_long_seg_ptr,
                      int64_t *d_counts, void *d_workspace, size_t workspace_bytes, void *stream);
int elimrec_plan_tiles(const int64_t *d_rowptr, int64_t n_rows, int T, int T1, int T2, int TS, int G, int64_t side_split,
                       int64_t rows_from, const int32_t *d_order, const int32_t *d_long_rows, const int32_t *d_long_seg_ptr,
                       int64_t n_w4, int64_t n_w1, int64_t n_split, int64_t n_short, int64_t n_long, int64_t n_seg,
                       int64_t *d_tile_off, int32_t *d_tile_len, int32_t *d_tile_dst, int32_t *d_tile_long, int64_t *d_gb,
                       int32_t *d_gs, int64_t *d_totals, void *d_workspace, size_t workspace_bytes, void *stream);
int elimrec_plan_scatter(int64_t n_tiles, int G, const int64_t *d_tile_off, const int64_t *d_gb, const int32_t *d_tile_len,
                         const int32_t *d_gs, const int32_t *d_col, const float *d_val, int32_t *d_tile_col, float *d_tile_val,
                         void *stream);

size_t elimrec_slab_partials_bytes(const elimrec_sell *A, int ns, int w);
int elimrec_slab_hop(const elimrec_sell *A, int ns, int w, int gs, const float *d_Xin,
                     const uint32_t *d_src_mask, float *d_Xout, const float *d_add,
                     const uint32_t *d_add_mask, float scale, float *d_partials, size_t partials_bytes,
                     int seg_only, void *stream);
size_t elimrec_slab_sweep_lds_rows(int w);
int elimrec_slab_sweep_hop(const int64_t *d_slot_ptr, const void *d_records,
                           int64_t n_rows, int64_t n_src, const int32_t *d_block_ptr, int parts, int passes, int bpx,
                           int max_block_rows, int ns, int w, const float *d_Xin, float *d_Xout,
                           const float *d_add, const uint32_t *d_add_mask, float scale, void *stream);
int elimrec_slab_sweep_hop_adam(const int64_t *d_slot_ptr, const void *d_records, int64_t n_rows, int64_t n_src,
                                const int32_t *d_block_ptr, int parts, int passes, int bpx, int max_block_rows, int ns, int w,
                                const float *d_Xin, float *d_grad_out, const float *d_add, const uint32_t *d_add_mask, float scale,
                                const float *d_p_in, float *d_p_out, float *d_m, float *d_v, float lr, float beta1, float beta2,
                                float eps, float weight_decay, int64_t step , void *stream);

int elimrec_slab_source_bits(const elimrec_sell *A, int ns, int w, int gs, const uint32_t *d_src_mask,
                             float *d_partials, size_t partials_bytes, void *stream);

int elimrec_slab_hop_bwd_w(const elimrec_sell *A, int ns, int w, int gs, const float *d_Xin, const uint32_t *d_src_mask,
                           float *d_Xout, const float *d_add, const uint32_t *d_add_mask, float scale, float *d_partials,
                           size_t partials_bytes, int flags, const elimrec_linear_bwd_desc *descs , int n,
                           void *d_workspace, size_t workspace_bytes, int phase, void *stream);

struct elimrec_adam_job;
int elimrec_slab_hop_adam(const elimrec_sell *A, int ns, int w, int gs, const float *d_Xin, float *d_grad_out,
                          const float *d_add, const uint32_t *d_add_mask, float scale, float *d_partials,
                          size_t partials_bytes, const float *d_p_in, float *d_p_out, float *d_m, float *d_v, float lr,
                          float beta1, float beta2, float eps, float weight_decay, int64_t step,
                          const struct elimrec_adam_job *tail_jobs, int n_tail_jobs, const float *d_sum_src, int64_t sum_n,
                          float *d_sum_dst, void *stream);

int elimrec_slab_rows(const elimrec_sell *A, int ns, int w, int L, int64_t U,
                      const float *const *layers, const float *d_long, const int32_t *d_rows,
                      const int32_t *d_counts, int64_t R, int n_lists, float *d_out0, int64_t ld_out0,
                      float *d_narrow, int64_t ld_narrow, int narrow_by_node, void *stream);

int elimrec_slab_from_rows(const float *d_src, int64_t ld, int64_t col0, int64_t n, int ns, int w,
                           float *d_slab, void *stream);
int elimrec_slab_to_rows(const float *d_slab, int64_t n, int ns, int w, float *d_dst, int64_t ld,
                         int64_t col0, void *stream);

int elimrec_slab_merge_rows(const float *d_rows, const int32_t *d_keys, int world, int64_t R, int64_t U,
                            int64_t I, int ns, int w, int M, float *d_SrcA, float *d_SrcB, uint32_t *d_mask,
                            void *stream);

int elimrec_adam_step_out(const float *d_p_in, float *d_p_out, const float *d_g, float *d_m, float *d_v,
                          int64_t n, float lr, float beta1, float beta2, float eps, float weight_decay,
                          int64_t step, void *stream);

size_t elimrec_head_pack_floats(int n_mod, const int *D);
size_t elimrec_head_pack_bwd_offset(int n_mod, const int *D);

#define ELIMREC_HEAD_MAX_TABLES 3
typedef struct elimrec_head_weights {
    int32_t n_mod, recdim;
    int32_t D[ELIMREC_HEAD_MAX_TABLES];
    const float *d_Wm[ELIMREC_HEAD_MAX_TABLES], *d_bm[ELIMREC_HEAD_MAX_TABLES];
    const float *d_Ws[ELIMREC_HEAD_MAX_TABLES], *d_bs[ELIMREC_HEAD_MAX_TABLES];
    const float *d_Wf_user, *d_bf_user, *d_Wf_item, *d_bf_item;
    float *d_pack;
    size_t pack_floats;
} elimrec_head_weights;

typedef struct elimrec_head_src16 {
    const void *d_table;
    int64_t row_elems;
    int32_t dtype;
    float *d_S_out;
    int64_t ld_S_out;
    float *d_c_out;
} elimrec_head_src16;

typedef struct elimrec_head_rows {
    const elimrec_sell *A;
    int32_t ns, w, L;
    int64_t U;
    const float *layers[9];
    const float *d_long;
    float *d_narrow_out;
    int64_t ld_narrow_out;
} elimrec_head_rows;

typedef struct elimrec_head_fwd_in {
    const float *d_out0; int64_t ld_out0;
    const float *d_narrow; int64_t ld_nar;
    const float *d_c;
    const float *d_S[ELIMREC_HEAD_MAX_TABLES]; int64_t ldS[ELIMREC_HEAD_MAX_TABLES];
    const float *d_recv; int32_t world; int64_t dl;
    elimrec_head_src16 src16;
    elimrec_head_rows rows;
} elimrec_head_fwd_in;
int elimrec_head_fwd_fused(const elimrec_head_fwd_in *in, const elimrec_head_weights *w, const int32_t *d_act,
                           const int32_t *d_seg_info, int64_t R, float *d_OutAct, int64_t ld_out, float *d_YAct, int64_t ld_y,
                           int phase, void *stream);

size_t elimrec_build_adj_workspace(int64_t E, int64_t N, int with_diag);
int elimrec_build_adj(const int64_t *d_users, const int64_t *d_items, int64_t E, int64_t U, int64_t I, int adj_type,
                      const float *d_pow_table, int table_len, int32_t *d_rowptr, int32_t *d_col, float *d_val,
                      int32_t *d_err, void *d_workspace, size_t workspace_bytes, void *stream);

typedef struct elimrec_adam_job {
    const float *d_p_in; float *d_p_out;
    const float *d_g; float *d_m; float *d_v;
    float *d_copy_dst;
    int64_t n; int64_t step;
} elimrec_adam_job;
int elimrec_adam_multi(const elimrec_adam_job *jobs , int n_jobs, float lr, float beta1, float beta2,
                       float eps, float weight_decay, void *stream);

#define ELIMREC_MAX_RANKS 16
int elimrec_lookup_counts(const int32_t *d_acts, int world, int64_t R, int64_t U, int64_t I, const int64_t *ub,
                          const int64_t *ib, int32_t *d_counts, void *stream);
int elimrec_lookup_pack(const int32_t *d_acts, int world, int64_t R, int64_t U, int64_t I, const int64_t *ub,
                        const int64_t *ib, int me, const void *d_shard, int64_t row_bytes, void *d_send,
                        int32_t *d_send_off, void *stream);
int elimrec_lookup_unpack(const int32_t *d_act, int world, int64_t R, int64_t U, int64_t I, const int64_t *ub,
                          const int64_t *ib, int me, const void *d_rows, int64_t row_bytes, int dtype, int sum_d,
                          int direct, float *d_S, int64_t ldS, float *d_c, void *stream);

int elimrec_wide_from_master(const float *d_master, int64_t U, int64_t N, int ns, int w, float *d_wide, void *stream);
int elimrec_wide_rows(const float *const *layers , int L, int64_t N, int ns, int w, const int32_t *d_rows,
                      int64_t total, float *d_out0, int64_t ld_out0, float *d_narrow, int64_t ld_narrow, void *stream);
int elimrec_wide_grad(const float *d_wide_grad, int64_t U, int64_t N, int ns, int w, float scale, float *d_grad, void *stream);
int elimrec_rows_bitmap(const int32_t *d_keys, int world, int64_t R, int64_t N, uint32_t *d_mask, void *stream);
int elimrec_peer_cols_to_rows(const float *d_recv, int world, int64_t R, int dl, float *d_out0, int64_t ld0, float *d_out1,
                              int64_t ld1, void *stream);

#define ELIMREC_PROGRAM_MAX_ARGS 32
enum { ELIMREC_OP_CALL = 0,
       ELIMREC_OP_RECORD = 1,
       ELIMREC_OP_WAIT = 2 };
typedef struct elimrec_op { int32_t kind; int32_t fn; uint64_t args[ELIMREC_PROGRAM_MAX_ARGS]; } elimrec_op;
typedef struct elimrec_patch { int32_t op; int32_t arg; uint64_t value; } elimrec_patch;
int elimrec_program_fn_count(void);
const char *elimrec_program_fn_name(int i);
int elimrec_program_fn_args(int i);
int elimrec_program_create(const elimrec_op *ops, int n_ops, void **prog_out);
int elimrec_program_create_scoped(const elimrec_op *ops, int n_ops, int system_scope_events, void **prog_out);
int elimrec_program_run(void *prog, const elimrec_patch *patches, int n_patches);
int elimrec_program_destroy(void *prog);
int elimrec_comm_unique_id(void *id128);
int elimrec_comm_create(const void *id128, int world, int rank, void **comm_out);
int elimrec_comm_nranks(void *comm, int *n_out);
int elimrec_comm_destroy(void *comm);
int elimrec_comm_all_gather(void *comm, const void *d_send, void *d_recv, int64_t bytes_per_rank, void *stream);
int elimrec_comm_all_reduce_f32(void *comm, float *d_buf, int64_t n, void *stream);
int elimrec_comm_all_to_all(void *comm, const void *d_send, void *d_recv, int64_t bytes_per_peer, void *stream);
int elimrec_comm_all_to_all_v(void *comm, const void *d_send, void *d_recv, const int64_t *sizes, void *stream);

#ifdef __cplusplus
}
#endif
#endif
```

Measured before the change: 7.359 million triplets/s.

## Fold weight-gradient slab reduction and its Adam update into the final hop kernel

The weight-gradient slab reduction phase moves out of its own pass and runs as front blocks of the final adam-fused hop kernel. Each of those blocks sums the per-chunk partials and applies Adam to the weight and bias spans directly. The overlapping optimizer tail jobs are split around these spans so nothing is updated twice. This removes a kernel phase and a round trip of the gradient through memory, at the cost of more host-side job splitting and a larger fused grid.

```diff
diff --git a/elimrec_amd/_lib.py b/elimrec_amd/_lib.py
--- a/elimrec_amd/_lib.py
+++ b/elimrec_amd/_lib.py
@@ -229,6 +229,10 @@
     "elimrec_slab_hop_adam": (c_i32, [c_sell, c_i32, c_i32, c_i32, c_ptr, c_ptr, c_ptr, c_ptr, c_f32, c_ptr, c_size, c_ptr, c_ptr,
                                       c_ptr, c_ptr, c_f32, c_f32, c_f32, c_f32, c_f32, c_i64, ctypes.POINTER(AdamJob), c_i32, c_ptr, c_i64,
                                       c_ptr, c_ptr]),
+    "elimrec_slab_hop_adam_wgrad": (c_i32, [c_sell, c_i32, c_i32, c_i32, c_ptr, c_ptr, c_ptr, c_ptr, c_f32, c_ptr, c_size, c_ptr, c_ptr,
+                                            c_ptr, c_ptr, c_f32, c_f32, c_f32, c_f32, c_f32, c_i64, ctypes.POINTER(AdamJob), c_i32, c_ptr,
+                                            c_i64, c_ptr, ctypes.POINTER(LinearBwdDesc), c_i32, c_ptr, c_size, c_ptr]),
+    "elimrec_slab_hop_adam_wgrad_jobs": (c_i32, [ctypes.POINTER(AdamJob), c_i32, ctypes.POINTER(LinearBwdDesc), c_i32]),
     "elimrec_slab_rows": (c_i32, [c_sell, c_i32, c_i32, c_i32, c_i64, ctypes.POINTER(c_ptr), c_ptr, c_ptr, c_ptr, c_i64, c_i32,
                                   c_ptr, c_i64, c_ptr, c_i64, c_i32, c_ptr]),
     "elimrec_slab_from_rows": (c_i32, [c_ptr, c_i64, c_i64, c_i64, c_i32, c_i32, c_ptr, c_ptr]),
@@ -327,7 +331,7 @@
             fn = getattr(lib, name)
             plain = name in ("elimrec_abi_version", "elimrec_program_fn_count", "elimrec_program_fn_args", "elimrec_comm_unique_id",
                              "elimrec_score_get_math", "elimrec_score_get_bf16x3", "elimrec_group_metric_means_chunk",
-                             "elimrec_rank_segment", "elimrec_rank_targets_per_pass",
+                             "elimrec_rank_segment", "elimrec_rank_targets_per_pass", "elimrec_slab_hop_adam_wgrad_jobs",
                              "elimrec_cosine_topk_chunk", "elimrec_cosine_topk_tile",
                              "elimrec_list_max_k", "elimrec_list_pair_cosine_small_k", "elimrec_list_pair_cosine_chunk_cols",
                              "elimrec_mmr_max_pool", "elimrec_mmr_rows_in_lds",
diff --git a/elimrec_amd/csrc/bwd_w.h b/elimrec_amd/csrc/bwd_w.h
--- a/elimrec_amd/csrc/bwd_w.h
+++ b/elimrec_amd/csrc/bwd_w.h
@@ -138,6 +138,18 @@
     if (colsum_slabs && tile_z == 0 && tid < TN1) colsum_slabs[(size_t)chunk * n1_pad + i_base + tid] = csum;
 }
 
+__device__ __forceinline__ float slab_lane_sum(const float *src, size_t stride, int chunks, int q) {
+    float s = 0.f;
+    int c = q;
+    for (; c + 12 < chunks; c += 16) {
+        const float v0 = src[(size_t)c * stride], v1 = src[(size_t)(c + 4) * stride];
+        const float v2 = src[(size_t)(c + 8) * stride], v3 = src[(size_t)(c + 12) * stride];
+        s += v0; s += v1; s += v2; s += v3;
+    }
+    for (; c < chunks; c += 4) s += src[(size_t)c * stride];
+    return s;
+}
+
 __device__ __forceinline__ void reduce_slabs_body(const BwdBatch &batch, int bx, int by) {
     const BwdProblem &pb = batch.p[by];
     const int n1 = pb.d.n1, n2 = pb.d.n2;
@@ -161,19 +173,72 @@
         stride = (size_t)n1_pad;
         dst = pb.d.d_colsum + (idx - total);
     }
-    float s = 0.f;
-    if (src) {
-        int c = q;
-        for (; c + 12 < chunks; c += 16) {
-            const float v0 = src[(size_t)c * stride], v1 = src[(size_t)(c + 4) * stride];
-            const float v2 = src[(size_t)(c + 8) * stride], v3 = src[(size_t)(c + 12) * stride];
-            s += v0; s += v1; s += v2; s += v3;
-        }
-        for (; c < chunks; c += 4) s += src[(size_t)c * stride];
-    }
+    float s = src ? slab_lane_sum(src, stride, chunks, q) : 0.f;
     s += __shfl_xor(s, 1, 64);
     s += __shfl_xor(s, 2, 64);
     if (src && q == 0) *dst = pb.d.accumulate ? (*dst + s) : s;
+}
+
+
+struct FoldSpan {
+    const float *p_in;
+    float *p_out, *m, *v, *copy_dst;
+    float step_size, inv_sqrt_bc2;
+};
+struct FoldProblem {
+    const float *slabs, *cslabs;
+    const int32_t *range;
+    float *out, *colsum;
+    int64_t R, ldo;
+    int chunk_rows, n1, n2, n1_pad, n2_pad, accumulate;
+    FoldSpan w, b;
+};
+struct FoldBatch { FoldProblem p[kMaxBatch]; int n, gx; };
+
+__device__ __forceinline__ void reduce_adam_body(const FoldBatch &batch, int bx, int by, float beta1, float beta2, float eps, float wd) {
+    const FoldProblem &pb = batch.p[by];
+    const int gid = bx * 256 + (int)threadIdx.x;
+    const int idx = gid >> 2, q = gid & 3;
+    const int total = pb.n1 * pb.n2;
+    int64_t rows = pb.range ? (int64_t)pb.range[1] - pb.range[0] : pb.R;
+    if (rows < 0) rows = 0;
+    const int chunks = (int)((rows + pb.chunk_rows - 1) / pb.chunk_rows);
+    const bool is_w = idx < total, is_b = !is_w && pb.cslabs && idx < total + pb.n1;
+    const float *src = nullptr;
+    size_t stride = 0;
+    int64_t at = 0;
+    if (is_w) {
+        const int i = idx / pb.n2, j = idx - i * pb.n2;
+        src = pb.slabs + (size_t)i * pb.n2_pad + j;
+        stride = (size_t)pb.n1_pad * pb.n2_pad;
+        at = (int64_t)i * pb.ldo + j;
+    } else if (is_b) {
+        src = pb.cslabs + (idx - total);
+        stride = (size_t)pb.n1_pad;
+        at = idx - total;
+    }
+    float s = src ? slab_lane_sum(src, stride, chunks, q) : 0.f;
+    s += __shfl_xor(s, 1, 64);
+    s += __shfl_xor(s, 2, 64);
+    if (!src || q != 0) return;
+    float *dst = (is_w ? pb.out : pb.colsum) + at;
+    const float g = pb.accumulate ? (*dst + s) : s;
+    *dst = g;
+    const float *p_in = is_w ? pb.w.p_in : pb.b.p_in;
+    if (!p_in) return;
+    float *p_out = is_w ? pb.w.p_out : pb.b.p_out, *m = is_w ? pb.w.m : pb.b.m, *v = is_w ? pb.w.v : pb.b.v;
+    float *copy_dst = is_w ? pb.w.copy_dst : pb.b.copy_dst;
+    const float step_size = is_w ? pb.w.step_size : pb.b.step_size, inv_sqrt_bc2 = is_w ? pb.w.inv_sqrt_bc2 : pb.b.inv_sqrt_bc2;
+    const float pi = p_in[at];
+    if (copy_dst) copy_dst[at] = pi;
+    const float gi = fmaf(wd, pi, g);
+    const float mo = m[at];
+    const float mi = mo + (1.f - beta1) * (gi - mo);
+    const float vi = fmaf(1.f - beta2, gi * gi, beta2 * v[at]);
+    const float denom = sqrtf(vi) * inv_sqrt_bc2 + eps;
+    m[at] = mi;
+    v[at] = vi;
+    p_out[at] = pi - step_size * (mi / denom);
 }
 
 
diff --git a/elimrec_amd/csrc/program.hip b/elimrec_amd/csrc/program.hip
--- a/elimrec_amd/csrc/program.hip
+++ b/elimrec_amd/csrc/program.hip
@@ -30,7 +30,7 @@
 #define ELIMREC_FN(fn) {#fn, [](const uint64_t *a) -> int { return call_packed(fn, a); }, arg_count(fn)}
 static const FnEntry kFns[] = {
     ELIMREC_FN(elimrec_batch_plan), ELIMREC_FN(elimrec_slab_hop), ELIMREC_FN(elimrec_slab_sweep_hop), ELIMREC_FN(elimrec_slab_sweep_hop_adam), ELIMREC_FN(elimrec_slab_source_bits), ELIMREC_FN(elimrec_slab_hop_bwd_w),
-    ELIMREC_FN(elimrec_slab_hop_adam), ELIMREC_FN(elimrec_slab_rows), ELIMREC_FN(elimrec_slab_merge_rows),
+    ELIMREC_FN(elimrec_slab_hop_adam), ELIMREC_FN(elimrec_slab_hop_adam_wgrad), ELIMREC_FN(elimrec_slab_rows), ELIMREC_FN(elimrec_slab_merge_rows),
     ELIMREC_FN(elimrec_head_fwd_fused), ELIMREC_FN(elimrec_bpr_head_rows), ELIMREC_FN(elimrec_sum), ELIMREC_FN(elimrec_segment_apply_head_bwd),
     ELIMREC_FN(elimrec_linear_fwd_batched), ELIMREC_FN(elimrec_linear_bwd_w_batched),
     ELIMREC_FN(elimrec_linear_bwd_w_batched_merge), ELIMREC_FN(elimrec_linear_bwd_w_reduce), ELIMREC_FN(elimrec_adam_multi),
diff --git a/elimrec_amd/csrc/slab.hip b/elimrec_amd/csrc/slab.hip
--- a/elimrec_amd/csrc/slab.hip
+++ b/elimrec_amd/csrc/slab.hip
@@ -674,6 +674,23 @@
     tier_body<LPR, 4, false, false, false, true, true>(t, scratch);
 }
 
+template <int LPR>
+__global__ __launch_bounds__(256) void sell_tier_adam_fold_kernel(TierArgs t, AdamJobs tail, int tail_block0, FoldBatch fold, int front) {
+    __shared__ float scratch[4 * 64 * 8];
+    if ((int)blockIdx.x < front) {
+        const int b = (int)blockIdx.x;
+        if (b < fold.gx * fold.n) reduce_adam_body(fold, b % fold.gx, b / fold.gx, t.s.ad_beta1, t.s.ad_beta2, t.s.ad_eps, t.s.ad_wd);
+        return;
+    }
+    if ((int)blockIdx.x >= tail_block0) {
+        const int b = (int)blockIdx.x - tail_block0;
+        if (b < tail.blocks) adam_jobs_body(tail, b, t.s.ad_beta1, t.s.ad_beta2, t.s.ad_eps, t.s.ad_wd);
+        else fixed_order_sum_body(tail.sum_src, tail.sum_n, tail.sum_dst, scratch);
+        return;
+    }
+    tier_body<LPR, 4, false, false, false, true, true>(t, scratch, (unsigned)front);
+}
+
 template <int LPR, bool MASKED>
 __global__ __launch_bounds__(256, (LPR <= 8 ? 5 : 1)) void sell_tier_bwdw_kernel(TierArgs t, BwdBatch batch, int tail_block0, int tail_mode, int gx) {
     __shared__ float As[2][TRB * TN1];
@@ -720,6 +737,7 @@
     float step_size, inv_sqrt_bc2, beta1, beta2, eps, wd;
     int keep_grad;
     const AdamJobs *tail;
+    const FoldBatch *fold;
 };
 
 static int launch_tier(const elimrec_sell *A, int ns, int wl, int wl_shift, int gs, int spg, int lpr, const void *Xin,
@@ -769,7 +787,11 @@
     AdamJobs tail = {};
     if (adam && adam->tail && (adam->tail->n > 0 || adam->tail->sum_src)) tail = *adam->tail;
     if (tail.n <= 0) tail.blocks = 0;
-    const dim3 grid((unsigned)(per_group * gs)), grid_adam((unsigned)(per_group * gs) + (unsigned)tail.blocks + (tail.sum_src ? 1u : 0u));
+    const FoldBatch *fold = (adam && adam->fold && adam->fold->n > 0) ? adam->fold : nullptr;
+    const int fold_front = fold ? (fold->gx * fold->n + 7) & ~7 : 0;
+    if (fold) tail_block0 += fold_front;
+    const dim3 grid((unsigned)(per_group * gs)),
+        grid_adam((unsigned)fold_front + (unsigned)(per_group * gs) + (unsigned)tail.blocks + (tail.sum_src ? 1u : 0u));
     const bool masked = src_mask != nullptr;
     if (masked) {
         ELIMREC_REQUIRE(A->tile_kmax > 0, "slab_hop: bad tile plan (tile_kmax)");
@@ -782,7 +804,10 @@
     }
 #define ELIMREC_TIER(LPR)                                                                                                     \
     do {                                                                                                                      \
-        if (adam) hipLaunchKernelGGL((sell_tier_adam_kernel<LPR>), grid_adam, dim3(256), 0, s, t, tail, tail_block0);         \
+        if (fold)                                                                                                             \
+            hipLaunchKernelGGL((sell_tier_adam_fold_kernel<LPR>), grid_adam, dim3(256), 0, s, t, tail, tail_block0, *fold,    \
+                               fold_front);                                                                                   \
+        else if (adam) hipLaunchKernelGGL((sell_tier_adam_kernel<LPR>), grid_adam, dim3(256), 0, s, t, tail, tail_block0);    \
         else if (bwdw && masked)                                                                                              \
             hipLaunchKernelGGL((sell_tier_bwdw_kernel<LPR, true>), dim3(grid.x + (unsigned)tail_blocks), dim3(256), 0, s, t,  \
                                *bwdw, tail_block0, tail_mode, reduce_gx);                                                     \
@@ -956,22 +981,89 @@
                        d_partials, flags, (hipStream_t)stream, nullptr, &batch, phase == 0 ? 2 : 1, phase == 0 ? blocks : gx * n, gx);
 }
 
-extern "C" int elimrec_slab_hop_adam(const elimrec_sell *A, int ns, int w, int gs, const float *d_Xin, float *d_grad_out,
-                                     const float *d_add, const uint32_t *d_add_mask, float scale, float *d_partials,
-                                     size_t partials_bytes, const float *d_p_in, float *d_p_out, float *d_m, float *d_v, float lr,
-                                     float beta1, float beta2, float eps, float weight_decay, int64_t step,
-                                     const elimrec_adam_job *tail_jobs, int n_tail_jobs, const float *d_sum_src, int64_t sum_n,
-                                     float *d_sum_dst, void *stream) {
-    ELIMREC_REQUIRE(A && d_Xin && d_p_in && d_p_out && d_m && d_v, "slab_hop_adam: null pointer");
-    ELIMREC_REQUIRE(!d_sum_src || (d_sum_dst && sum_n >= 0 && sum_n < INT32_MAX), "slab_hop_adam: the sum needs a destination");
-    ELIMREC_REQUIRE(A->tiered, "slab_hop_adam: needs a tiered (wave-tile) plan");
-    ELIMREC_REQUIRE(step >= 1, "slab_hop_adam: 1-based step");
+struct FoldBind { int job; int64_t off, len; };
+static int fold_split(const elimrec_adam_job *jobs, int n_jobs, const elimrec_linear_bwd_desc *descs, int n, elimrec_adam_job *left,
+                      FoldBind (*binds)[2]) {
+    if (!descs || n < 1 || n > kMaxBatch || n_jobs < 0 || n_jobs > 8 || (n_jobs > 0 && !jobs)) return -1;
+    struct Piece { int64_t off, len; };
+    Piece cover[8][2 * kMaxBatch];
+    int n_cover[8] = {0};
+    const float *seen_lo[2 * kMaxBatch], *seen_hi[2 * kMaxBatch];
+    int n_seen = 0;
+    for (int i = 0; i < n; ++i) {
+        const elimrec_linear_bwd_desc &d = descs[i];
+        if (!d.d_out || d.n1 <= 0 || d.n2 <= 0 || d.ldo != d.n2) return -1;
+        for (int h = 0; h < 2; ++h) {
+            FoldBind &b = binds[i][h];
+            b.job = -1; b.off = 0; b.len = 0;
+            const float *lo = h == 0 ? d.d_out : d.d_colsum;
+            if (!lo) continue;
+            const float *hi = lo + (h == 0 ? (int64_t)d.n1 * d.n2 : (int64_t)d.n1);
+            for (int k = 0; k < n_seen; ++k)
+                if (lo < seen_hi[k] && seen_lo[k] < hi) return -1;
+            seen_lo[n_seen] = lo; seen_hi[n_seen] = hi; ++n_seen;
+            for (int k = 0; k < n_jobs; ++k) {
+                const elimrec_adam_job &j = jobs[k];
+                if (j.n <= 0 || !j.d_g) continue;
+                if (hi <= j.d_g || j.d_g + j.n <= lo) continue;
+                if (lo < j.d_g || j.d_g + j.n < hi) return -1;
+                b.job = k; b.off = lo - j.d_g; b.len = hi - lo;
+                cover[k][n_cover[k]++] = Piece{b.off, b.len};
+                break;
+            }
+        }
+    }
+    int n_left = 0;
+    for (int k = 0; k < n_jobs; ++k) {
+        const elimrec_adam_job &j = jobs[k];
+        if (j.n <= 0) continue;
+        if (n_cover[k] == 0) {
+            if (n_left == 8) return -1;
+            left[n_left++] = j;
+            continue;
+        }
+        for (int a = 1; a < n_cover[k]; ++a)
+            for (int b = a; b > 0 && cover[k][b].off < cover[k][b - 1].off; --b) { const Piece t = cover[k][b]; cover[k][b] = cover[k][b - 1]; cover[k][b - 1] = t; }
+        int64_t at = 0;
+        for (int a = 0; a <= n_cover[k]; ++a) {
+            const int64_t end = a < n_cover[k] ? cover[k][a].off : j.n;
+            if (end > at) {
+                if (n_left == 8) return -1;
+                elimrec_adam_job g = j;
+                g.d_p_in = j.d_p_in + at; g.d_p_out = j.d_p_out + at; g.d_g = j.d_g + at; g.d_m = j.d_m + at; g.d_v = j.d_v + at;
+                g.d_copy_dst = j.d_copy_dst ? j.d_copy_dst + at : nullptr;
+                g.n = end - at;
+                left[n_left++] = g;
+            }
+            if (a < n_cover[k]) at = cover[k][a].off + cover[k][a].len;
+        }
+    }
+    return n_left;
+}
+
+extern "C" int elimrec_slab_hop_adam_wgrad_jobs(const elimrec_adam_job *tail_jobs, int n_tail_jobs, const elimrec_linear_bwd_desc *descs,
+                                                int n) {
+    elimrec_adam_job left[8];
+    FoldBind binds[kMaxBatch][2];
+    return fold_split(tail_jobs, n_tail_jobs, descs, n, left, binds);
+}
+
+static int slab_hop_adam(const char *who, const elimrec_sell *A, int ns, int w, int gs, const float *d_Xin, float *d_grad_out,
+                         const float *d_add, const uint32_t *d_add_mask, float scale, float *d_partials, size_t partials_bytes,
+                         const float *d_p_in, float *d_p_out, float *d_m, float *d_v, float lr, float beta1, float beta2, float eps,
+                         float weight_decay, int64_t step, const elimrec_adam_job *tail_jobs, int n_tail_jobs, const float *d_sum_src,
+                         int64_t sum_n, float *d_sum_dst, const elimrec_linear_bwd_desc *descs, int n, void *d_workspace,
+                         size_t workspace_bytes, void *stream) {
+    ELIMREC_REQUIRE(A && d_Xin && d_p_in && d_p_out && d_m && d_v, "%s: null pointer", who);
+    ELIMREC_REQUIRE(!d_sum_src || (d_sum_dst && sum_n >= 0 && sum_n < INT32_MAX), "%s: the sum needs a destination", who);
+    ELIMREC_REQUIRE(A->tiered, "%s: needs a tiered (wave-tile) plan", who);
+    ELIMREC_REQUIRE(step >= 1, "%s: 1-based step", who);
     ELIMREC_REQUIRE((const void *)d_Xin != (const void *)d_p_out && (const void *)d_Xin != (const void *)d_m &&
-                        (const void *)d_Xin != (const void *)d_v, "slab_hop_adam: the gathered table must not be written");
+                        (const void *)d_Xin != (const void *)d_v, "%s: the gathered table must not be written", who);
     int w4_shift, spg, lpr, rc;
-    if ((rc = slab_geometry("slab_hop_adam", ns, w, gs, w4_shift, spg, lpr))) return rc;
+    if ((rc = slab_geometry(who, ns, w, gs, w4_shift, spg, lpr))) return rc;
     if (!d_partials || partials_bytes < elimrec_slab_partials_bytes(A, ns, w)) {
-        set_error("slab_hop_adam: partial-row scratch too small");
+        set_error("%s: partial-row scratch too small", who);
         return ELIMREC_E_WORKSPACE;
     }
     AdamEpilogue ad;
@@ -981,15 +1073,82 @@
     ad.inv_sqrt_bc2 = (float)(1.0 / sqrt(bc2));
     ad.beta1 = beta1; ad.beta2 = beta2; ad.eps = eps; ad.wd = weight_decay; ad.keep_grad = d_grad_out ? 1 : 0;
     AdamJobs tail = {};
+    FoldBatch fold = {};
     ad.tail = nullptr;
+    ad.fold = nullptr;
+    elimrec_adam_job left[8];
+    if (descs) {
+        ELIMREC_REQUIRE(n >= 1 && n <= kMaxBatch, "%s: 1..%d weight-gradient problems", who, kMaxBatch);
+        ELIMREC_REQUIRE(n_tail_jobs >= 0 && n_tail_jobs <= 8, "%s: at most 8 tail jobs", who);
+        ELIMREC_REQUIRE(d_workspace && workspace_bytes >= bwd_w_batched_bytes(descs, n), "%s: weight-gradient workspace", who);
+        FoldBind binds[kMaxBatch][2];
+        const int n_left = fold_split(tail_jobs, n_tail_jobs, descs, n, left, binds);
+        if (n_left < 0) {
+            set_error("%s: the weight gradients do not fold into these optimizer spans (elimrec_slab_hop_adam_wgrad_jobs)", who);
+            return ELIMREC_E_BADARG;
+        }
+        BwdBatch batch;
+        int blocks = 0, max_out = 0;
+        if ((rc = bwd_w_build_batch(descs, n, d_workspace, batch, blocks, max_out))) return rc;
+        fold.n = n;
+        fold.gx = (4 * max_out + 255) / 256;
+        for (int i = 0; i < n; ++i) {
+            const BwdProblem &pb = batch.p[i];
+            FoldProblem &f = fold.p[i];
+            f.slabs = pb.slabs; f.cslabs = pb.d.d_colsum ? pb.cslabs : nullptr; f.range = pb.d.d_range;
+            f.out = pb.d.d_out; f.colsum = pb.d.d_colsum; f.R = pb.d.R; f.ldo = pb.d.ldo;
+            f.chunk_rows = pb.chunk_rows; f.n1 = pb.d.n1; f.n2 = pb.d.n2; f.n1_pad = pb.t1 * TN1; f.n2_pad = pb.t2 * TN2;
+            f.accumulate = pb.d.accumulate;
+            for (int h = 0; h < 2; ++h) {
+                FoldSpan &sp = h == 0 ? f.w : f.b;
+                sp = FoldSpan{};
+                const FoldBind &b = binds[i][h];
+                if (b.job < 0) continue;
+                const elimrec_adam_job &j = tail_jobs[b.job];
+                ELIMREC_REQUIRE(j.d_p_in && j.d_p_out && j.d_m && j.d_v && j.step >= 1, "%s: job %d: an update needs p_out, m, v and a 1-based step",
+                                who, b.job);
+                sp.p_in = j.d_p_in + b.off; sp.p_out = j.d_p_out + b.off; sp.m = j.d_m + b.off; sp.v = j.d_v + b.off;
+                sp.copy_dst = j.d_copy_dst ? j.d_copy_dst + b.off : nullptr;
+                sp.step_size = (float)((double)lr / (1.0 - pow((double)beta1, (double)j.step)));
+                sp.inv_sqrt_bc2 = (float)(1.0 / sqrt(1.0 - pow((double)beta2, (double)j.step)));
+            }
+        }
+        ad.fold = &fold;
+        tail_jobs = left;
+        n_tail_jobs = n_left;
+    }
     if (tail_jobs && n_tail_jobs > 0) {
-        ELIMREC_REQUIRE(n_tail_jobs <= 8, "slab_hop_adam: at most 8 tail jobs");
-        if ((rc = build_adam_jobs("slab_hop_adam", tail_jobs, n_tail_jobs, lr, beta1, beta2, tail))) return rc;
+        ELIMREC_REQUIRE(n_tail_jobs <= 8, "%s: at most 8 tail jobs", who);
+        if ((rc = build_adam_jobs(who, tail_jobs, n_tail_jobs, lr, beta1, beta2, tail))) return rc;
         ad.tail = &tail;
     }
     if (d_sum_src) { tail.sum_src = d_sum_src; tail.sum_dst = d_sum_dst; tail.sum_n = (int)sum_n; ad.tail = &tail; }
     return launch_tier(A, ns, w / 4, w4_shift, gs, spg, lpr, d_Xin, nullptr, d_grad_out, d_add, d_add_mask, scale,
                        d_partials, 0, (hipStream_t)stream, &ad);
+}
+
+extern "C" int elimrec_slab_hop_adam(const elimrec_sell *A, int ns, int w, int gs, const float *d_Xin, float *d_grad_out,
+                                     const float *d_add, const uint32_t *d_add_mask, float scale, float *d_partials,
+                                     size_t partials_bytes, const float *d_p_in, float *d_p_out, float *d_m, float *d_v, float lr,
+                                     float beta1, float beta2, float eps, float weight_decay, int64_t step,
+                                     const elimrec_adam_job *tail_jobs, int n_tail_jobs, const float *d_sum_src, int64_t sum_n,
+                                     float *d_sum_dst, void *stream) {
+    return slab_hop_adam("slab_hop_adam", A, ns, w, gs, d_Xin, d_grad_out, d_add, d_add_mask, scale, d_partials, partials_bytes, d_p_in,
+                         d_p_out, d_m, d_v, lr, beta1, beta2, eps, weight_decay, step, tail_jobs, n_tail_jobs, d_sum_src, sum_n, d_sum_dst,
+                         nullptr, 0, nullptr, 0, stream);
+}
+
+extern "C" int elimrec_slab_hop_adam_wgrad(const elimrec_sell *A, int ns, int w, int gs, const float *d_Xin, float *d_grad_out,
+                                           const float *d_add, const uint32_t *d_add_mask, float scale, float *d_partials,
+                                           size_t partials_bytes, const float *d_p_in, float *d_p_out, float *d_m, float *d_v, float lr,
+                                           float beta1, float beta2, float eps, float weight_decay, int64_t step,
+                                           const elimrec_adam_job *tail_jobs, int n_tail_jobs, const float *d_sum_src, int64_t sum_n,
+                                           float *d_sum_dst, const elimrec_linear_bwd_desc *descs, int n, void *d_workspace,
+                                           size_t workspace_bytes, void *stream) {
+    ELIMREC_REQUIRE(descs, "slab_hop_adam_wgrad: no weight-gradient problems");
+    return slab_hop_adam("slab_hop_adam_wgrad", A, ns, w, gs, d_Xin, d_grad_out, d_add, d_add_mask, scale, d_partials, partials_bytes,
+                         d_p_in, d_p_out, d_m, d_v, lr, beta1, beta2, eps, weight_decay, step, tail_jobs, n_tail_jobs, d_sum_src, sum_n,
+                         d_sum_dst, descs, n, d_workspace, workspace_bytes, stream);
 }
 
 extern "C" int elimrec_slab_rows(const elimrec_sell *A, int ns, int w, int L, int64_t U, const float *const *layers,
diff --git a/elimrec_amd/shard.py b/elimrec_amd/shard.py
--- a/elimrec_amd/shard.py
+++ b/elimrec_amd/shard.py
@@ -824,6 +824,12 @@
         return os.environ.get("ELIMREC_FUSE_BWDW", "1") != "0" and hops_in_region >= 2
 
     @_once
+    def _fuse_wgrad_fold(self):
+        import os
+        return (os.environ.get("ELIMREC_FUSE_WGRAD_FOLD", "1") != "0" and not self.multi and not self.sweep and self._fuse_adam()
+                and self._fuse_reduce() and self._fuse_bwd_w())
+
+    @_once
     def _sources_in_head(self):
         import os
         return (not self.multi and not self.wide and self._fused_head_ok() and bool(self._pack_bwd_off) and self.model.latent_dim == 64
@@ -1326,6 +1332,14 @@
                 self.wgrads_handle = reduce_wgrads()
             return
 
+        fold, tail_early = False, None
+        if single and fuse and reduce is not None and reduce[1] == 0 and self._fuse_wgrad_fold():
+            tail_early = self._tail_jobs()
+            fkey = (self._tail_plan[0], ctypes.addressof(reduce[0][0]), reduce[0][1])
+            if getattr(self, "_fold_ok", (None, False))[0] != fkey:
+                self._fold_ok = (fkey, len(tail_early) <= 8 and slab.wgrad_fold_jobs(tail_early, reduce[0]) >= 0)
+            fold = self._fold_ok[1]
+
         def hops():
             phase = None if reduce is None else reduce[1]
             if merged:
@@ -1339,11 +1353,11 @@
                 dst = self.grad if k == 0 else self.tmp[k & 1]
                 slab.hop(self.planT, t, dst, gs=self.gs, src_mask=tmask, add=self.srcB if (k & 1) else self.srcA,
                          add_mask=self.mask, scale=inv if k == 0 else 1.0, bits_ready=tmask is not None and self._bits_ready,
-                         bwd_w=reduce[0] if phase is not None and phase <= 1 else None, bwd_w_phase=phase)
+                         bwd_w=reduce[0] if phase is not None and phase <= (0 if fold else 1) else None, bwd_w_phase=phase)
                 phase = None if phase is None else phase + 1
                 t, tmask = dst, None
         self._timed(lambda: m._region("cs_bwd_hops", (m._ws_gen, recv2.data_ptr(), acts.data_ptr(), R, W, fuse, self._bits_ready, merged,
-                                                               0 if reduce is None else ctypes.addressof(reduce[0][0]), 0 if reduce is None else reduce[1]), hops), L - last)
+                                                               0 if reduce is None else ctypes.addressof(reduce[0][0]), 0 if reduce is None else reduce[1], fold), hops), L - last)
         self._adam_in_hop = fuse
         self._tail_in_hop = False
         if fuse:
@@ -1357,7 +1371,10 @@
                 in_hop = False
             if grads_ready is not None:
                 grads_ready.wait()
-            tail = self._tail_jobs() if in_hop else []
+            if tail_early is not None:
+                tail = tail_early
+            else:
+                tail = self._tail_jobs() if in_hop else []
             if len(tail) > 8:
                 raise RuntimeError("more than 8 optimizer spans")
             if getattr(self, "_tail_arr", None) is None:
@@ -1372,7 +1389,7 @@
             self._timed(lambda: slab.hop_adam(self.planT, self.tmp[1], self.grad if self.keep_grad else None, self.gs, self.srcA,
                                               self.mask, inv, self.master[self.cur].data, self.master[nxt].data, self.m1, self.m2,
                                               g["lr"], g["betas"][0], g["betas"][1], g["eps"], g["weight_decay"],
-                                              self.step_count + 1, tail_jobs=tail, loss_sum=late), 1)
+                                              self.step_count + 1, tail_jobs=tail, loss_sum=late, wgrad=reduce[0] if fold else None), 1)
 
     @torch.no_grad()
     def cs_update(self):
diff --git a/elimrec_amd/slab.py b/elimrec_amd/slab.py
--- a/elimrec_amd/slab.py
+++ b/elimrec_amd/slab.py
@@ -477,25 +477,38 @@
 
 
 def hop_adam(plan, xin, grad_out, gs, add, add_mask, scale, p_in, p_out, m, v, lr, beta1, beta2, eps, weight_decay, step, tail_jobs=(),
-             loss_sum=None):
+             loss_sum=None, wgrad=None):
     if isinstance(tail_jobs, tuple) and len(tail_jobs) == 2 and not isinstance(tail_jobs[0], _lib.AdamJob):
         arr, n_tail = tail_jobs
     else:
         arr, n_tail = ((_lib.AdamJob * len(tail_jobs))(*tail_jobs) if tail_jobs else None), len(tail_jobs)
     ns, w = xin.ns, xin.w
     if _swept(plan, xin):
+        assert wgrad is None, "hop_adam: the swept form carries no weight-gradient fold"
         hop_adam(plan.sweep.items, xin, grad_out, gs, add, add_mask, scale, p_in, p_out, m, v, lr, beta1, beta2, eps, weight_decay, step,
                  tail_jobs=(arr, n_tail), loss_sum=loss_sum)
         plan.sweep.hop_adam(xin, grad_out, add, add_mask, scale, p_in, p_out, m, v, lr, beta1, beta2, eps, weight_decay, step)
         return
     part = plan.partials(ns, w)
-    _lib.check(_lib.load().elimrec_slab_hop_adam(
-        plan.ref(), ns, w, int(gs), _dev(xin.data, "xin"), _dev(None if grad_out is None else grad_out.data, "grad"),
-        _dev(None if add is None else add.data, "add"), _dev(add_mask, "add_mask", torch.int32), float(scale), _dev(part, "partials"),
-        part.numel() * 4, _dev(p_in, "p_in"), _dev(p_out, "p_out"), _dev(m, "m"), _dev(v, "v"), float(lr), float(beta1), float(beta2),
-        float(eps), float(weight_decay), int(step), arr, n_tail, _dev(None if loss_sum is None else loss_sum[0], "loss_rows"),
-        0 if loss_sum is None else loss_sum[0].numel(), _dev(None if loss_sum is None else loss_sum[1], "loss_out"), _stream()),
-        "slab_hop_adam")
+    args = (plan.ref(), ns, w, int(gs), _dev(xin.data, "xin"), _dev(None if grad_out is None else grad_out.data, "grad"),
+            _dev(None if add is None else add.data, "add"), _dev(add_mask, "add_mask", torch.int32), float(scale), _dev(part, "partials"),
+            part.numel() * 4, _dev(p_in, "p_in"), _dev(p_out, "p_out"), _dev(m, "m"), _dev(v, "v"), float(lr), float(beta1), float(beta2),
+            float(eps), float(weight_decay), int(step), arr, n_tail, _dev(None if loss_sum is None else loss_sum[0], "loss_rows"),
+            0 if loss_sum is None else loss_sum[0].numel(), _dev(None if loss_sum is None else loss_sum[1], "loss_out"))
+    if wgrad is not None:
+        descs, n, wsp = wgrad
+        _lib.check(_lib.load().elimrec_slab_hop_adam_wgrad(*(args + (descs, n, _dev(wsp, "workspace", torch.uint8), wsp.numel(), _stream()))),
+                   "slab_hop_adam_wgrad")
+        return
+    _lib.check(_lib.load().elimrec_slab_hop_adam(*(args + (_stream(),))), "slab_hop_adam")
+
+
+def wgrad_fold_jobs(tail_jobs, wgrad):
+    if isinstance(tail_jobs, tuple) and len(tail_jobs) == 2 and not isinstance(tail_jobs[0], _lib.AdamJob):
+        arr, n_tail = tail_jobs
+    else:
+        arr, n_tail = ((_lib.AdamJob * len(tail_jobs))(*tail_jobs) if tail_jobs else None), len(tail_jobs)
+    return int(_lib.load().elimrec_slab_hop_adam_wgrad_jobs(arr, n_tail, wgrad[0], wgrad[1]))
 
 
 
diff --git a/include/elimrec_hip.h b/include/elimrec_hip.h
--- a/include/elimrec_hip.h
+++ b/include/elimrec_hip.h
@@ -392,6 +392,15 @@
                           float beta1, float beta2, float eps, float weight_decay, int64_t step,
                           const struct elimrec_adam_job *tail_jobs, int n_tail_jobs, const float *d_sum_src, int64_t sum_n,
                           float *d_sum_dst, void *stream);
+int elimrec_slab_hop_adam_wgrad(const elimrec_sell *A, int ns, int w, int gs, const float *d_Xin, float *d_grad_out,
+                                const float *d_add, const uint32_t *d_add_mask, float scale, float *d_partials,
+                                size_t partials_bytes, const float *d_p_in, float *d_p_out, float *d_m, float *d_v, float lr,
+                                float beta1, float beta2, float eps, float weight_decay, int64_t step,
+                                const struct elimrec_adam_job *tail_jobs, int n_tail_jobs, const float *d_sum_src, int64_t sum_n,
+                                float *d_sum_dst, const elimrec_linear_bwd_desc *descs , int n, void *d_workspace,
+                                size_t workspace_bytes, void *stream);
+int elimrec_slab_hop_adam_wgrad_jobs(const struct elimrec_adam_job *tail_jobs , int n_tail_jobs,
+                                     const elimrec_linear_bwd_desc *descs , int n);
 
 int elimrec_slab_rows(const elimrec_sell *A, int ns, int w, int L, int64_t U,
                       const float *const *layers, const float *d_long, const int32_t *d_rows,
```

New measurement: 7.476 million triplets/s (median of 6 runs). 1.6% higher.
